# plai-group/latent-flexible-video-diffusion-modeling

Measured on AMD Instinct MI355X. Metric: denoising steps/sec on 20-frame 4x16x16 latents (sampling; training reported alongside), higher is better.
Workload: dtype f32

## Files before the change

### include/lfvdm_hip.h

```cpp
#ifndef LFVDM_HIP_H
#define LFVDM_HIP_H

#include <stdint.h>

#ifdef __cplusplus
extern "C" {
#endif

#define LFVDM_OK 0
#define LFVDM_E_SHAPE 1
#define LFVDM_E_LAUNCH 2
#define LFVDM_E_UNSUPPORTED 3

#define LFVDM_ACT_NONE 0
#define LFVDM_ACT_SILU 1

#define LFVDM_OUT_ROWS 0
#define LFVDM_OUT_NCHW 1

int lfvdm_abi_version(void);

typedef struct lfvdm_conv_args {
    const float* src0;
    const float* src1;
// ... 186 lines not shown
} lfvdm_rpe_job;

int lfvdm_rpe_nets(const lfvdm_rpe_job* jobs_dev, int njobs, int total_tiles, const int64_t* frame_indices_i64,
                   int B, int T, void* stream);
int lfvdm_rpe_nets_maxc(const lfvdm_rpe_job* jobs_dev, int njobs, int total_tiles, const int64_t* frame_indices_i64,
                        int B, int T, int max_channels, void* stream);

typedef struct lfvdm_rpe_bwd_job {
    const float* tproj;
    const float* Wd;
    const float* bd;
    const float* Wout_t;
    const float* dR;
    float* dtproj;
    float* dWd;
    float* dbd;
    int32_t C;
    int32_t tile0;
    int32_t tproj_ld;
    int32_t dtproj_ld;
} lfvdm_rpe_bwd_job;

int lfvdm_rpe_nets_bwd(const lfvdm_rpe_bwd_job* jobs_dev, int njobs, int total_tiles, const int64_t* frame_indices_i64,
                       int B, int T, void* stream);
int lfvdm_rpe_nets_bwd_det(const lfvdm_rpe_bwd_job* jobs_dev, int njobs, int total_tiles, const int64_t* frame_indices_i64,
                           int B, int T, float* det_ws, int64_t det_ws_floats, void* stream);

int lfvdm_rpe_front(const float* tproj, int tproj_ld, const float* feats, const float* Wd, const float* bd, float* act, int B,
                    int rows_per_b, int C, void* stream);
int lfvdm_rpe_front_bwd(const float* tproj, int tproj_ld, const float* feats, const float* Wd, const float* bd,
                        const float* d_act, float* dtproj, int dtproj_ld, float* dWd, float* dbd, int B, int rows_per_b,
                        int C, void* stream);

int lfvdm_attn_spatial(const float* qkv, float* o, float* attn_out, float* lse_out, int N, int P, int C, int heads,
                       void* stream);

int lfvdm_attn_spatial_fused_ok(int N, int P, int C, int heads);
int lfvdm_attn_spatial_fused(const float* xn, const float* Wqkv, const float* bqkv, float* o, int N, int P, int C, int heads,
                             void* stream);

int lfvdm_attn_spatial_bwd(const float* qkv, const float* o, const float* d_o, const float* lse, float* delta_ws,
                           float* dqkv, int N, int P, int C, int heads, void* stream);

int lfvdm_attn_temporal(const float* qkv, const float* Rq, const float* Rk, const float* Rv,
                        const float* mask , float* o, float* attn_out,
                        int B, int T, int P, int C, int heads, void* stream);
int lfvdm_attn_temporal_sel(const float* qkv, const float* Rq, const float* Rk, const float* Rv, const float* mask,
                            float* o, float* attn_out, int B, int T, int P, int C, int heads, const int64_t* rsel,
                            void* stream);
int lfvdm_attn_temporal_ring(const float* qkv, const float* Rq, const float* Rk, const float* Rv, const float* mask,
                             float* o, float* attn_out, int B, int T, int P, int C, int heads, const int64_t* rsel,
                             int ring, void* stream);

int lfvdm_attn_temporal_bwd(const float* qkv, const float* d_o, const float* Rq, const float* Rk, const float* Rv,
                            const float* mask, float* ws_p, float* ws_ds, float* dqkv, float* dRq, float* dRk,
                            float* dRv, int B, int T, int P, int C, int heads, void* stream);

int lfvdm_q_sample(const float* x0, const float* noise, const int64_t* t, const float* sqrt_acp,
                   const float* sqrt_1macp, float* out, int B, int inner, void* stream);
#define LFVDM_RULE_ANCESTRAL 0
#define LFVDM_RULE_DDIM 1
#define LFVDM_MEAN_EPS 0
#define LFVDM_MEAN_X0 1
int lfvdm_update_x0(const float* x, const float* model_out, const float* noise, const int64_t* t, const float* sqrt_recip_acp,
                    const float* sqrt_recipm1_acp, const float* c1, const float* c2, const float* sg, int rule, int mean_type,
                    int clip, float* sample, float* pred_xstart, float* mean_out, int B, int inner, void* stream);
int lfvdm_update_rng_x0(const float* x, const float* model_out, float* noise_out, const int64_t* t, const float* sqrt_recip_acp,
                        const float* sqrt_recipm1_acp, const float* c1, const float* c2, const float* sg, int rule,
                        int mean_type, int clip, float* sample, float* pred_xstart, float* mean_out, int B, int inner,
                        const int64_t* seed, void* stream);
int lfvdm_conv_out_psample_ok(int N, int H, int W, int C, int Cout);
int lfvdm_conv_out_update_x0(const float* act, const float* Wp, const float* bias, float* out, const float* x,
                             const float* noise_in, float* noise_out, const int64_t* t, const float* sqrt_recip_acp,
                             const float* sqrt_recipm1_acp, const float* c1, const float* c2, const float* sg, int rule,
                             int mean_type, int clip, float* sample, float* pred_xstart, float* mean_out, int B, int T, int H,
                             int W, int C, int Cout, const int64_t* seed, void* stream);
int lfvdm_update_ms_x0(const float* x, const float* model_out, const float* hist, const int64_t* t, const float* sqrt_recip_acp,
                       const float* sqrt_recipm1_acp, const float* k1, const float* k2, const float* k3, int mean_type, int clip,
                       float* sample, float* pred_xstart, int B, int inner, void* stream);
int lfvdm_conv_out_update_ms_x0(const float* act, const float* Wp, const float* bias, float* out, const float* x,
                                const float* hist, const int64_t* t, const float* sqrt_recip_acp, const float* sqrt_recipm1_acp,
                                const float* k1, const float* k2, const float* k3, int mean_type, int clip, float* sample,
                                float* pred_xstart, int B, int T, int H, int W, int C, int Cout, void* stream);
int lfvdm_known_blend(float* x, const float* known, const float* mask, const float* eps, float* noise_out, const int64_t* t,
                      const float* sqrt_acp_prev, const float* sqrt_1macp_prev, const int64_t* seed, int B, int T, int C,
                      int HW, void* stream);
int lfvdm_renoise(float* x, float* noise_out, const int64_t* t, const float* sqrt_1mbeta, const float* sqrt_beta,
                  const int64_t* seed, int B, int inner, void* stream);
int lfvdm_sampler_tick(int64_t* t, const float* model_timestep_table, float* model_t, int B, void* stream);
int lfvdm_sampler_tick_fetch(int64_t* t, const float* model_timestep_table, float* model_t, int B, const float* rows_all,
                             int rows_ld, float* rows, int row_floats, void* stream);
int lfvdm_masked_mse(const float* a, const float* b, const float* mask, float* out, int B, int T,
                     int frame_inner, void* stream);
int lfvdm_masked_mse_bwd(const float* target, const float* pred, const float* mask, const float* g, float* dpred, int B, int T,
                         int frame_inner, void* stream);

int lfvdm_train_loss(const float* target, const float* pred, const float* mask, const float* eval_mask, const int64_t* t,
                     const float* wtab, int n_t, float* mse, float* eval_mse, float* loss, int B, int T, int frame_inner,
                     void* stream);
int lfvdm_train_loss_bwd(const float* target, const float* pred, const float* mask, const int64_t* t, const float* wtab, int n_t,
                         const float* g, float* dpred, int B, int T, int frame_inner, void* stream);

int lfvdm_vb_terms(const float* x_start, const float* x_t, const float* model_out, const float* noise, const int64_t* t,
                   const float* sqrt_recip_acp, const float* sqrt_recipm1_acp, const float* c1, const float* c2,
                   const float* post_log_var, const float* model_log_var, const float* mask, int mean_type, int clip, float* vb,
                   float* xstart_mse, float* eps_mse, float* pred_xstart, int B, int T, int frame_inner, int out_ld,
                   int col_base, void* stream);
int lfvdm_vb_terms_bwd(const float* x_start, const float* x_t, const float* model_out, const int64_t* t,
                       const float* sqrt_recip_acp, const float* sqrt_recipm1_acp, const float* c1, const float* c2,
                       const float* model_log_var, const float* mask, const float* g, int mean_type, int clip, float* d_out,
                       int B, int T, int frame_inner, void* stream);

typedef struct lfvdm_adamw_args {
    float* p;
    const float* g;
    float* m;
    float* v;
    float* ema[4];
    float ema_rate[4];
    int32_t n_ema;
    int64_t n;
    float lr, beta1, beta2, eps, weight_decay;
    float bias_corr1, bias_corr2_sqrt;
    float grad_scale;
    float* grad_sqsum;
    const int32_t* skip_flag;
    const int32_t* skip_flag2;
} lfvdm_adamw_args;

int lfvdm_adamw_ema(const lfvdm_adamw_args* a, void* stream);

#define LFVDM_GRAD_NORM_MAX_PARTS 512
int lfvdm_grad_norm_nparts(int64_t n);
int lfvdm_grad_norm_partials(const float* g, int64_t n, float grad_scale, float* partials, int nparts, void* stream);
int lfvdm_grad_norm_finalize(const float* partials, int nparts, float max_norm, float* stat, void* stream);
int lfvdm_adamw_ema_clip(const lfvdm_adamw_args* a, const float* stat, void* stream);

int lfvdm_prepare_batch(const float* pool, const int32_t* table, float* batch, int64_t* frame_indices, float* obs_mask,
                        float* latent_mask, int B, int F, int Tp, int frame_elems, void* stream);

#define LFVDM_SLOT_PAD 0
#define LFVDM_SLOT_OBS 1
#define LFVDM_SLOT_LATENT 2
int lfvdm_search_assemble(const float* pool, const int32_t* table, const int32_t* role, float* x0, float* x_start,
                          float* obs_mask, float* latent_mask, float* mask, int64_t* frame_indices, int W, int K, int V, int Tv,
                          int frame_elems, void* stream);
int lfvdm_search_noise_qsample(const float* x_start, const int32_t* table, const int64_t* t_list, int32_t* ctl,
                               const int64_t* key, const float* sqrt_acp, const float* sqrt_1macp, float* noise, float* x_t,
                               int64_t* t_buf, int W, int K, int V, int frame_elems, void* stream);
int lfvdm_search_noise_fill(const int32_t* table, uint64_t seed, int step, int j, float* noise, int W, int K, int V,
                            int frame_elems, void* stream);
int lfvdm_search_scores(const float* terms, const int64_t* t_list, float* scores, int G, int V, int n_t, int ld, int col_base,
                        void* stream);

int lfvdm_compose_rows(const float* x, const float* x0, const float* obs, float* rows, int N, int Cx, int H, int W, int ld,
                       void* stream);

#define LFVDM_CHAIN_CONV 0
#define LFVDM_CHAIN_GN 1
#define LFVDM_CHAIN_LOCAL 2
#define LFVDM_CHAIN_MAX_DEPS 64
#define LFVDM_CHAIN_CTL_EPOCH 0
#define LFVDM_CHAIN_CTL_EXIT 32
#define LFVDM_CHAIN_CTL_ABORT 64
#define LFVDM_CHAIN_CTL_INTS 96

// ... 56 lines not shown
```

### latent-flexible-video-diffusion-modeling_amd/csrc/diffusion_ops.hip

```cpp
#include "common_hip.h"
#include "philox_normal.h"

namespace {

__global__ __launch_bounds__(256) void q_sample_kernel(const float* __restrict__ x0, const float* __restrict__ noise,
                                                       const int64_t* __restrict__ t, const float* __restrict__ sa,
                                                       const float* __restrict__ sb, float* __restrict__ out, int inner) {
    const int b = blockIdx.y;
    const float ca = sa[t[b]], cb = sb[t[b]];
    const size_t base = (size_t)b * inner;
    for (int i = (blockIdx.x * blockDim.x + threadIdx.x) * 4; i < inner; i += gridDim.x * blockDim.x * 4) {
        if (i + 3 < inner) {
            st4(out + base + i, ca * ld4(x0 + base + i) + cb * ld4(noise + base + i));
        } else {
            for (int j = i; j < inner; ++j) out[base + j] = ca * x0[base + j] + cb * noise[base + j];
        }
    }
}

enum { RULE_ANCESTRAL = 0, RULE_DDIM = 1, RULE_DDIM_DET = 2, RULE_DPMPP2M = 3 };
constexpr bool rule_draws(int rule) { return rule == RULE_ANCESTRAL || rule == RULE_DDIM; }

enum { MEAN_EPS = 0, MEAN_X0 = 1 };

template <int MEAN>
__device__ __forceinline__ float mean_x0hat(float r, float rm1, float xv, float out) {
    return MEAN == MEAN_X0 ? out : r * xv - rm1 * out;
}

template <int RULE>
__device__ __forceinline__ float rule_sigma(const float* __restrict__ t_logvar, int64_t tb) {
    if (RULE == RULE_ANCESTRAL) return tb != 0 ? expf(0.5f * t_logvar[tb]) : 0.f;
    if (RULE == RULE_DDIM) return tb != 0 ? t_logvar[tb] : 0.f;
    return 0.f;
}

struct StepCoef { float r, rm1, c1, c2, sigma; };

template <int RULE, int MEAN>
__device__ __forceinline__ StepCoef step_coef(int64_t tb, const float* t_recip, const float* t_recipm1, const float* t_c1,
                                              const float* t_c2, const float* t_logvar) {
    return {MEAN == MEAN_EPS ? t_recip[tb] : 0.f, MEAN == MEAN_EPS ? t_recipm1[tb] : 0.f, t_c1[tb], t_c2[tb],
            rule_sigma<RULE>(t_logvar, tb)};
}

template <int MEAN>
__device__ __forceinline__ float step_mean(const StepCoef& k, float xv, float out, int clip, float& p0) {
    p0 = mean_x0hat<MEAN>(k.r, k.rm1, xv, out);
    if (clip) p0 = fminf(fmaxf(p0, -1.f), 1.f);
    return k.c1 * p0 + k.c2 * xv;
}

template <int MEAN>
__device__ __forceinline__ float multistep_mean(const StepCoef& k, float k3, float xv, float out, int clip, const float* hist,
                                                size_t at, float& p0) {
    p0 = MEAN == MEAN_X0 ? out : __fmaf_rn(k.r, xv, -__fmul_rn(k.rm1, out));
    if (clip) p0 = fminf(fmaxf(p0, -1.f), 1.f);
    float mean = __fmaf_rn(k.c2, xv, __fmul_rn(k.c1, p0));
    if (k3 != 0.f) mean = __fmaf_rn(k3, __fsub_rn(p0, hist[at]), mean);
    return mean;
}

template <int RULE> struct PredOut { typedef float* __restrict__ ptr; };
template <> struct PredOut<RULE_DPMPP2M> { typedef float* ptr; };

template <int RULE, int MEAN>
__global__ __launch_bounds__(256) void p_sample_kernel(const float* x, const float* __restrict__ eps,
                                                       const float* __restrict__ noise, const int64_t* __restrict__ t,
                                                       const float* __restrict__ t_recip, const float* __restrict__ t_recipm1,
                                                       const float* __restrict__ t_c1, const float* __restrict__ t_c2,
                                                       const float* __restrict__ t_logvar, int clip,
                                                       float* sample, typename PredOut<RULE>::ptr pred,
                                                       float* __restrict__ mean_out, int inner, const float* hist,
                                                       const float* __restrict__ t_k3) {
    const int b = blockIdx.y;
    const int64_t tb = t[b];
    const StepCoef k = step_coef<RULE, MEAN>(tb, t_recip, t_recipm1, t_c1, t_c2, t_logvar);
    const float k3 = RULE == RULE_DPMPP2M ? t_k3[tb] : 0.f;
    const size_t base = (size_t)b * inner;
    for (int i = blockIdx.x * blockDim.x + threadIdx.x; i < inner; i += gridDim.x * blockDim.x) {
        float p0;
        const float mean = RULE == RULE_DPMPP2M ? multistep_mean<MEAN>(k, k3, x[base + i], eps[base + i], clip, hist, base + i, p0)
                                                : step_mean<MEAN>(k, x[base + i], eps[base + i], clip, p0);
        float sv = mean;
        if (rule_draws(RULE) && tb != 0) sv += k.sigma * noise[base + i];
        sample[base + i] = sv;
        if (pred) pred[base + i] = p0;
        if (mean_out) mean_out[base + i] = mean;
    }
}

template <int RULE, int MEAN>
__global__ __launch_bounds__(256) void p_sample_rng_kernel(const float* x, const float* __restrict__ eps,
                                                           float* __restrict__ noise_out, const int64_t* __restrict__ t,
                                                           const float* __restrict__ t_recip, const float* __restrict__ t_recipm1,
                                                           const float* __restrict__ t_c1, const float* __restrict__ t_c2,
                                                           const float* __restrict__ t_logvar, int clip, float* sample,
                                                           float* __restrict__ pred, float* __restrict__ mean_out, int inner,
                                                           const int64_t* __restrict__ seed) {
    const int b = blockIdx.y;
    const int64_t tb = t[b];
    const StepCoef k = step_coef<RULE, MEAN>(tb, t_recip, t_recipm1, t_c1, t_c2, t_logvar);
    const unsigned long long key = RULE != RULE_DDIM_DET ? (unsigned long long)seed[0] : 0ull;
    const unsigned k0 = (unsigned)key, k1 = (unsigned)(key >> 32);
    const size_t base = (size_t)b * inner;
    const int nq = (inner + 3) >> 2;
    for (int qd = blockIdx.x * blockDim.x + threadIdx.x; qd < nq; qd += gridDim.x * blockDim.x) {
        f32x4 z = (f32x4){0.f, 0.f, 0.f, 0.f};
        if (RULE != RULE_DDIM_DET) z = normal4((unsigned)qd, (unsigned)b, (unsigned)tb, k0, k1);
#pragma unroll
        for (int e = 0; e < 4; ++e) {
            const int i = 4 * qd + e;
            if (i < inner) {
                float p0;
                const float mean = step_mean<MEAN>(k, x[base + i], eps[base + i], clip, p0);
                sample[base + i] = RULE != RULE_DDIM_DET ? mean + k.sigma * z[e] : mean;
                if (RULE != RULE_DDIM_DET && noise_out) noise_out[base + i] = z[e];
                if (pred) pred[base + i] = p0;
                if (mean_out) mean_out[base + i] = mean;
            }
        }
    }
}

struct HeadUpdate {
    const float *act, *Wp, *bias, *x, *noise_in;
    float *eps_out, *noise_out, *sample, *pred, *mean_out;
    const int64_t *t, *seed;
    const float *t_recip, *t_recipm1, *t_c1, *t_c2, *t_logvar;
    int N, T, H, W, C, clip;
    const float *hist, *t_k3;
};

template <int CO, int CPL, int RULE, int MEAN>
__global__ __launch_bounds__(256) void conv_out_psample_kernel(const HeadUpdate p) {
    extern __shared__ __attribute__((aligned(16))) float wl[];
    const int tid = threadIdx.x;
    const int C = p.C;
    {
        constexpr int NW4 = CO * 9 * 16 * CPL, NIT = (NW4 + 255) / 256;
        f32x4 wv[NIT];
#pragma unroll
        for (int u = 0; u < NIT; ++u) {
            const int i = tid + 256 * u;
            wv[u] = i < NW4 ? ld4(p.Wp + 4 * (size_t)i) : (f32x4){0.f, 0.f, 0.f, 0.f};
        }
#pragma unroll
        for (int u = 0; u < NIT; ++u) {
            const int i = tid + 256 * u;
            if (i < NW4) st4(wl + 4 * i, wv[u]);
        }
    }
    __syncthreads();
    const int lane = tid & 63, wave = tid >> 6;
    const int WQ = p.W >> 2;
    const long quad = (long)blockIdx.x * 4 + wave;
    if (quad >= (long)p.N * p.H * WQ) return;
    const int n = (int)(quad / (p.H * WQ));
    const int rem = (int)(quad - (long)n * p.H * WQ);
    const int y = rem / WQ, xq = rem - y * WQ;
    const int j = lane >> 4, cl = lane & 15;
    const int x = 4 * xq + j;
    float acc[CO];
#pragma unroll
    for (int co = 0; co < CO; ++co) acc[co] = 0.f;
#pragma unroll
    for (int tap = 0; tap < 9; ++tap) {
        const int iy = y + tap / 3 - 1, ix = x + tap % 3 - 1;
        const bool inb = iy >= 0 && iy < p.H && ix >= 0 && ix < p.W;
        const float* a = p.act + ((size_t)(n * p.H + (inb ? iy : y)) * p.W + (inb ? ix : x)) * C;
#pragma unroll
        for (int u = 0; u < CPL; ++u) {
            const int c = (cl + 16 * u) * 4;
            f32x4 a4 = ld4(a + c);
            if (!inb) a4 = (f32x4){0.f, 0.f, 0.f, 0.f};
#pragma unroll
            for (int co = 0; co < CO; ++co) {
                const f32x4 w4 = ld4(wl + (co * 9 + tap) * C + c);
                acc[co] += (a4.x * w4.x + a4.y * w4.y) + (a4.z * w4.z + a4.w * w4.w);
            }
        }
    }
#pragma unroll
    for (int co = 0; co < CO; ++co)
#pragma unroll
        for (int o = 1; o < 16; o <<= 1) acc[co] += __shfl_xor(acc[co], o, 64);
    if (cl >= CO) return;
    float e = acc[0];
#pragma unroll
    for (int co = 1; co < CO; ++co) e = cl == co ? acc[co] : e;
    const int co = cl;
    e += p.bias[co];
    const int b = n / p.T, tt = n - b * p.T;
    const int inner = p.T * CO * p.H * p.W;
    const int i = ((tt * CO + co) * p.H + y) * p.W + x;
    const size_t at = (size_t)b * inner + i;
    const int64_t tb = p.t[b];
    const StepCoef k = step_coef<RULE, MEAN>(tb, p.t_recip, p.t_recipm1, p.t_c1, p.t_c2, p.t_logvar);
    float z = 0.f;
    if (!rule_draws(RULE)) {
    } else if (p.noise_in) {
        z = p.noise_in[at];
    } else {
        const unsigned long long key = (unsigned long long)p.seed[0];
        const f32x4 z4 = normal4((unsigned)(i >> 2), (unsigned)b, (unsigned)tb, (unsigned)key, (unsigned)(key >> 32));
        z = j == 0 ? z4.x : j == 1 ? z4.y : j == 2 ? z4.z : z4.w;
    }
    float p0;
    const float mean = RULE == RULE_DPMPP2M ? multistep_mean<MEAN>(k, p.t_k3[tb], p.x[at], e, p.clip, p.hist, at, p0)
                                            : step_mean<MEAN>(k, p.x[at], e, p.clip, p0);
    p.sample[at] = rule_draws(RULE) ? mean + k.sigma * z : mean;
    if (p.eps_out) p.eps_out[at] = e;
    if (rule_draws(RULE) && p.noise_out) p.noise_out[at] = z;
    if (p.pred) p.pred[at] = p0;
    if (p.mean_out) p.mean_out[at] = mean;
}

__global__ __launch_bounds__(1024) void masked_mse_kernel(const float* __restrict__ a, const float* __restrict__ bb,
                                                          const float* __restrict__ mask, float* __restrict__ out, int T,
                                                          int frame_inner) {
    const int b = blockIdx.x;
    const size_t base = (size_t)b * T * frame_inner;
    float acc = 0.f;
    if ((frame_inner & 3) == 0) {
        const int q = frame_inner >> 2, total = T * q;
        for (int e = threadIdx.x; e < total; e += 1024) {
            const int t = e / q;
            const float mk = mask ? mask[b * T + t] : 1.f;
            const f32x4 d = ld4(a + base + (size_t)e * 4) - ld4(bb + base + (size_t)e * 4);
            acc += ((d.x * d.x + d.y * d.y) + (d.z * d.z + d.w * d.w)) * mk;
        }
    } else {
        for (int t = 0; t < T; ++t) {
            const float mk = mask ? mask[b * T + t] : 1.f;
            for (int i = threadIdx.x; i < frame_inner; i += 1024) {
                const float d = a[base + (size_t)t * frame_inner + i] - bb[base + (size_t)t * frame_inner + i];
                acc += d * d * mk;
            }
        }
    }
    __shared__ float red[16];
    acc = wave_sum(acc);
    if ((threadIdx.x & 63) == 0) red[threadIdx.x >> 6] = acc;
    __syncthreads();
    if (threadIdx.x == 0) {
        float t = 0.f;
        for (int w = 0; w < 16; ++w) t += red[w];
        out[b] = t / (float)((size_t)T * frame_inner);
    }
}

__global__ __launch_bounds__(256) void masked_mse_bwd_kernel(const float* __restrict__ target, const float* __restrict__ pred,
                                                             const float* __restrict__ mask, const float* __restrict__ g,
                                                             float* __restrict__ dpred, int T, int frame_inner) {
    const int b = blockIdx.y;
    const size_t base = (size_t)b * T * frame_inner;
    const float sc = -2.0f * g[b] / (float)((size_t)T * frame_inner);
    const long total = (long)T * frame_inner;
    for (long i = (long)blockIdx.x * 256 + threadIdx.x; i < total; i += (long)gridDim.x * 256) {
        const float mk = mask ? mask[b * T + (int)(i / frame_inner)] : 1.f;
        dpred[base + i] = (target[base + i] - pred[base + i]) * (sc * mk);
    }
}

}

extern "C" int lfvdm_masked_mse_bwd(const float* target, const float* pred, const float* mask, const float* g, float* dpred,
                                    int B, int T, int frame_inner, void* stream) {
    if (B <= 0 || T <= 0 || frame_inner <= 0 || !target || !pred || !g || !dpred) return LFVDM_E_SHAPE;
    long gx = ((long)T * frame_inner + 255) / 256;
    if (gx > 1024) gx = 1024;
    hipLaunchKernelGGL(masked_mse_bwd_kernel, dim3((unsigned)gx, B), dim3(256), 0, (hipStream_t)stream, target, pred, mask, g, dpred,
                       T, frame_inner);
    LFVDM_CHECK_LAUNCH();
    return LFVDM_OK;
}

extern "C" int lfvdm_q_sample(const float* x0, const float* noise, const int64_t* t, const float* sqrt_acp,
                              const float* sqrt_1macp, float* out, int B, int inner, void* stream) {
    if (B <= 0 || inner <= 0) return LFVDM_E_SHAPE;
    int gx = (inner / 4 + 255) / 256;
    if (gx > 1024) gx = 1024;
    if (gx < 1) gx = 1;
    hipLaunchKernelGGL(q_sample_kernel, dim3(gx, B), dim3(256), 0, (hipStream_t)stream, x0, noise, t, sqrt_acp, sqrt_1macp, out, inner);
    LFVDM_CHECK_LAUNCH();
    return LFVDM_OK;
}

namespace {
__global__ void sampler_tick_kernel(int64_t* __restrict__ t, const float* __restrict__ table, float* __restrict__ model_t, int B) {
    const int b = blockIdx.x * blockDim.x + threadIdx.x;
    if (b >= B) return;
    int64_t v = t[b] - 1;
    v = v < 0 ? 0 : v;
    t[b] = v;
    model_t[b] = table[v];
}

// ... 124 lines not shown
                               const float* sqrt_recip_acp, const float* sqrt_recipm1_acp, const float* c1, const float* c2,
                               const float* sg, int rule, int mean_type, int clip, float* sample, float* pred_xstart,
                               float* mean_out, int B, int inner, void* stream) {
    const int R = update_cell(rule, mean_type, x, model_out, t, sqrt_recip_acp, sqrt_recipm1_acp, c1, c2, sg, sample, B, inner,
                              noise != nullptr);
    if (R < 0) return LFVDM_E_SHAPE;
    return on_grid(R, mean_type, [&](auto r, auto m) {
        return launch_update<decltype(r)::value, decltype(m)::value>(
            x, model_out, decltype(r)::value == RULE_DDIM_DET ? nullptr : noise, t, sqrt_recip_acp, sqrt_recipm1_acp, c1, c2, sg,
            clip, sample, pred_xstart, mean_out, B, inner, stream);
    });
}

extern "C" int lfvdm_update_rng_x0(const float* x, const float* model_out, float* noise_out, const int64_t* t,
                                   const float* sqrt_recip_acp, const float* sqrt_recipm1_acp, const float* c1, const float* c2,
                                   const float* sg, int rule, int mean_type, int clip, float* sample, float* pred_xstart,
                                   float* mean_out, int B, int inner, const int64_t* seed, void* stream) {
    const int R = update_cell(rule, mean_type, x, model_out, t, sqrt_recip_acp, sqrt_recipm1_acp, c1, c2, sg, sample, B, inner,
                              seed != nullptr);
    if (R < 0) return LFVDM_E_SHAPE;
    return on_grid(R, mean_type, [&](auto r, auto m) {
        constexpr bool det = decltype(r)::value == RULE_DDIM_DET;
        return launch_update_rng<decltype(r)::value, decltype(m)::value>(
            x, model_out, det ? nullptr : noise_out, t, sqrt_recip_acp, sqrt_recipm1_acp, c1, c2, sg, clip, sample, pred_xstart,
            mean_out, B, inner, det ? nullptr : seed, stream);
    });
}

extern "C" int lfvdm_conv_out_update_x0(const float* act, const float* Wp, const float* bias, float* out, const float* x,
                                        const float* noise_in, float* noise_out, const int64_t* t, const float* sqrt_recip_acp,
                                        const float* sqrt_recipm1_acp, const float* c1, const float* c2, const float* sg,
                                        int rule, int mean_type, int clip, float* sample, float* pred_xstart, float* mean_out,
                                        int B, int T, int H, int W, int C, int Cout, const int64_t* seed, void* stream) {
    const int R = update_cell(rule, mean_type, x, act, t, sqrt_recip_acp, sqrt_recipm1_acp, c1, c2, sg, sample, B, T,
                              noise_in || seed);
    if (R < 0 || !Wp || !bias) return LFVDM_E_SHAPE;
    const bool det = R == RULE_DDIM_DET;
    const HeadUpdate p = {act, Wp, bias, x, det ? nullptr : noise_in, out, det ? nullptr : noise_out, sample, pred_xstart, mean_out,
                          t, det ? nullptr : seed, sqrt_recip_acp, sqrt_recipm1_acp, c1, c2, sg, B * T, T, H, W, C, clip,
                          nullptr, nullptr};
    return on_grid(R, mean_type, [&](auto r, auto m) { return launch_head<decltype(r)::value, decltype(m)::value>(p, Cout, stream); });
}

namespace {
bool multistep_ok(int mean_type, const float* x, const float* model_out, const int64_t* t, const float* recip,
                  const float* recipm1, const float* k1, const float* k2, const float* k3, const float* sample, int B, int inner) {
    if (!mean_ok(mean_type, recip, recipm1)) return false;
    return B > 0 && inner > 0 && x && model_out && t && k1 && k2 && k3 && sample;
}
template <class F>
int on_multistep(bool have_hist, int mean_type, F f) {
    const bool x0 = mean_type == LFVDM_MEAN_X0;
    if (have_hist) return x0 ? f(Const<RULE_DPMPP2M>(), Const<MEAN_X0>()) : f(Const<RULE_DPMPP2M>(), Const<MEAN_EPS>());
    return x0 ? f(Const<RULE_DDIM_DET>(), Const<MEAN_X0>()) : f(Const<RULE_DDIM_DET>(), Const<MEAN_EPS>());
}
}

extern "C" int lfvdm_update_ms_x0(const float* x, const float* model_out, const float* hist, const int64_t* t,
                                  const float* sqrt_recip_acp, const float* sqrt_recipm1_acp, const float* k1, const float* k2,
                                  const float* k3, int mean_type, int clip, float* sample, float* pred_xstart, int B, int inner,
                                  void* stream) {
    if (!multistep_ok(mean_type, x, model_out, t, sqrt_recip_acp, sqrt_recipm1_acp, k1, k2, k3, sample, B, inner))
        return LFVDM_E_SHAPE;
    return on_multistep(hist != nullptr, mean_type, [&](auto r, auto m) {
        return launch_update<decltype(r)::value, decltype(m)::value>(x, model_out, nullptr, t, sqrt_recip_acp, sqrt_recipm1_acp, k1,
                                                                     k2, nullptr, clip, sample, pred_xstart, nullptr, B, inner,
                                                                     stream, hist, k3);
    });
}

extern "C" int lfvdm_conv_out_update_ms_x0(const float* act, const float* Wp, const float* bias, float* out, const float* x,
                                           const float* hist, const int64_t* t, const float* sqrt_recip_acp,
                                           const float* sqrt_recipm1_acp, const float* k1, const float* k2, const float* k3,
                                           int mean_type, int clip, float* sample, float* pred_xstart, int B, int T, int H, int W,
                                           int C, int Cout, void* stream) {
    if (!multistep_ok(mean_type, x, act, t, sqrt_recip_acp, sqrt_recipm1_acp, k1, k2, k3, sample, B, T) || !Wp || !bias)
        return LFVDM_E_SHAPE;
    const HeadUpdate p = {act, Wp, bias, x, nullptr, out, nullptr, sample, pred_xstart, nullptr, t, nullptr, sqrt_recip_acp,
                          sqrt_recipm1_acp, k1, k2, nullptr, B * T, T, H, W, C, clip, hist, k3};
    return on_multistep(hist != nullptr, mean_type,
                        [&](auto r, auto m) { return launch_head<decltype(r)::value, decltype(m)::value>(p, Cout, stream); });
}

extern "C" int lfvdm_masked_mse(const float* a, const float* b, const float* mask, float* out, int B, int T,
                                int frame_inner, void* stream) {
    if (B <= 0 || T <= 0 || frame_inner <= 0) return LFVDM_E_SHAPE;
    hipLaunchKernelGGL(masked_mse_kernel, dim3(B), dim3(1024), 0, (hipStream_t)stream, a, b, mask, out, T, frame_inner);
    LFVDM_CHECK_LAUNCH();
    return LFVDM_OK;
}
```

### latent-flexible-video-diffusion-modeling_amd/csrc/norm_embed.hip

```cpp
#include "common_hip.h"
#include "gn_wave_body.h"

namespace {

constexpr int GN_GPW = 8;
constexpr int GN_THREADS = 256;
constexpr int GN_MAXCW = 256;


template <int KEEP>
__global__ __launch_bounds__(GN_THREADS) void gn_coef_kernel(
    const float* __restrict__ s0, const float* __restrict__ s1, int C0, int C1, int P,
    const float* __restrict__ gamma, const float* __restrict__ beta, const float* __restrict__ film, int film_div,
    int film_ld, float eps, float* __restrict__ coefA, float* __restrict__ coefB, float* __restrict__ stats,
    float* __restrict__ act_out, int act_mode) {
    const int C = C0 + C1;
    const int cg = C / 32;
    const float rcg = __builtin_amdgcn_rcpf((float)cg);
    const int CW = GN_GPW * cg;
    const int Q = CW / 4;
    const int n = blockIdx.x;
    const int cbase = blockIdx.y * CW;
    const int PL = GN_THREADS / Q;
    const int tid = threadIdx.x;
    const bool active = tid < PL * Q;
    const int q = active ? tid % Q : 0;
    const int pl = active ? tid / Q : 0;
    const int c = cbase + q * 4;

    __shared__ float part[GN_THREADS * 4];
    __shared__ float chs[GN_MAXCW];
    __shared__ float gmean[GN_GPW], grstd[GN_GPW];
    __shared__ __attribute__((aligned(16))) float shA[GN_MAXCW], shB[GN_MAXCW];

    const size_t pos0 = (size_t)n * P;
    const bool pow2q = (Q & (Q - 1)) == 0 && Q <= 64;
    const bool cached = P <= KEEP * PL;
    f32x4 keep[KEEP];
    for (int pass = 0; pass < 2; ++pass) {
        f32x4 s = {0.f, 0.f, 0.f, 0.f};
        if (active) {
            f32x4 mu = {0.f, 0.f, 0.f, 0.f};
            if (pass) {
                mu.x = gmean[fdiv_small(q * 4 + 0, cg, rcg)]; mu.y = gmean[fdiv_small(q * 4 + 1, cg, rcg)];
                mu.z = gmean[fdiv_small(q * 4 + 2, cg, rcg)]; mu.w = gmean[fdiv_small(q * 4 + 3, cg, rcg)];
            }
            if (cached) {
#pragma unroll
                for (int i = 0; i < KEEP; ++i) {
                    const int p = pl + i * PL;
                    if (pass == 0) {
                        keep[i] = (p < P) ? ld_cat(s0, s1, C0, C1, pos0 + p, c) : (f32x4){0.f, 0.f, 0.f, 0.f};
                        s += keep[i];
                    } else if (p < P) {
                        const f32x4 v = keep[i] - mu;
                        s += v * v;
                    }
                }
            } else {
                for (int p = pl; p < P; p += PL) {
                    f32x4 v = ld_cat(s0, s1, C0, C1, pos0 + p, c);
                    if (pass) { v = v - mu; s += v * v; } else { s += v; }
                }
            }
            if (pow2q) {
                for (int off = Q; off < 64; off <<= 1) {
                    s.x += __shfl_xor(s.x, off, 64); s.y += __shfl_xor(s.y, off, 64);
                    s.z += __shfl_xor(s.z, off, 64); s.w += __shfl_xor(s.w, off, 64);
                }
                if ((tid & 63) < Q) st4(part + ((tid >> 6) * Q + q) * 4, s);
            } else {
                st4(part + (pl * Q + q) * 4, s);
            }
        }
        __syncthreads();
        const int rows = pow2q ? GN_THREADS / 64 : PL;
        for (int cc = tid; cc < CW; cc += GN_THREADS) {
            float t = 0.f;
            for (int i = 0; i < rows; ++i) t += part[i * CW + cc];
            chs[cc] = t;
        }
        __syncthreads();
        if (tid < GN_GPW) {
            float t = 0.f;
            for (int i = 0; i < cg; ++i) t += chs[tid * cg + i];
            const float inv = 1.0f / (float)(cg * P);
            if (pass == 0) gmean[tid] = t * inv;
            else grstd[tid] = 1.0f / sqrtf(t * inv + eps);
        }
        __syncthreads();
    }
    if (stats && tid < GN_GPW) {
        stats[((size_t)n * 32 + blockIdx.y * GN_GPW + tid) * 2 + 0] = gmean[tid];
        stats[((size_t)n * 32 + blockIdx.y * GN_GPW + tid) * 2 + 1] = grstd[tid];
    }
    for (int cc = tid; cc < CW; cc += GN_THREADS) {
        const int ch = cbase + cc;
        const int g = fdiv_small(cc, cg, rcg);
        float A = grstd[g] * gamma[ch];
        float B = beta[ch] - gmean[g] * A;
        if (film) {
            const float* f = film + (size_t)(n / film_div) * film_ld;
            const float sc = 1.0f + f[ch];
            A *= sc;
            B = B * sc + f[C + ch];
        }
        if (coefA) {
            coefA[(size_t)n * C + ch] = A;
            coefB[(size_t)n * C + ch] = B;
        }
        shA[cc] = A;
        shB[cc] = B;
    }
    if (act_out == nullptr) return;
    __syncthreads();
    if (active) {
        const f32x4 a4 = ld4(shA + q * 4), b4 = ld4(shB + q * 4);
        if (cached) {
#pragma unroll
            for (int i = 0; i < KEEP; ++i) {
                const int p = pl + i * PL;
                if (p < P) {
                    f32x4 v = keep[i] * a4 + b4;
                    if (act_mode == LFVDM_ACT_SILU) { v.x = silu_f(v.x); v.y = silu_f(v.y); v.z = silu_f(v.z); v.w = silu_f(v.w); }
                    st4(act_out + (pos0 + p) * C + c, v);
                }
            }
        } else {
            for (int p = pl; p < P; p += PL) {
                f32x4 v = ld_cat(s0, s1, C0, C1, pos0 + p, c) * a4 + b4;
                if (act_mode == LFVDM_ACT_SILU) { v.x = silu_f(v.x); v.y = silu_f(v.y); v.z = silu_f(v.z); v.w = silu_f(v.w); }
                st4(act_out + (pos0 + p) * C + c, v);
            }
        }
    }
}

template <int CG>
__global__ __launch_bounds__(64) void gn_wave_kernel(
    const float* __restrict__ s0, const float* __restrict__ s1, int C0, int C1, int P,
    const float* __restrict__ gamma, const float* __restrict__ beta, const float* __restrict__ film, int film_div,
    int film_ld, float eps, float* __restrict__ coefA, float* __restrict__ coefB, float* __restrict__ stats,
    float* __restrict__ act_out, int act_mode, int ldo) {
    gn_wave_body<CG, false>(blockIdx.x, blockIdx.y, threadIdx.x, s0, s1, C0, C1, P, gamma, beta, film, film_div, film_ld, eps, coefA,
                            coefB, stats, act_out, act_mode, ldo);
}

template <int CG>
__global__ __launch_bounds__(256) void gn_wave4_kernel(
    const float* __restrict__ s0, const float* __restrict__ s1, int C0, int C1, int P,
    const float* __restrict__ gamma, const float* __restrict__ beta, const float* __restrict__ film, int film_div,
    int film_ld, float eps, float* __restrict__ coefA, float* __restrict__ coefB, float* __restrict__ stats,
    float* __restrict__ act_out, int act_mode, int ldo) {
    gn_wave_body<CG, false, 4>(blockIdx.x, blockIdx.y, threadIdx.x & 63, s0, s1, C0, C1, P, gamma, beta, film, film_div, film_ld, eps,
                               coefA, coefB, stats, act_out, act_mode, ldo, __builtin_amdgcn_readfirstlane(threadIdx.x >> 6));
}

inline bool gn_wave_launch(const float* src0, const float* src1, int C0, int C1, int N, int P, const float* gamma,
                           const float* beta, const float* film, int film_div, int film_ld, float eps, float* coefA,
                           float* coefB, float* stats, float* out, int act, hipStream_t s) {
    static const bool off = getenv("LFVDM_GN_NO_WAVE") != nullptr;
    const int C = C0 + C1, cg = C / 32;
    if (off || P > 256 || C0 % 16 || (cg != 2 && cg != 4 && cg != 8 && cg != 16) || N > 65535) return false;
    const dim3 grid(N, C / 16);
    static const int minp4 = getenv("LFVDM_GN_WAVE4_MINP") ? atoi(getenv("LFVDM_GN_WAVE4_MINP")) : 128;
    if (minp4 > 0 && P >= minp4 && P % 64 == 0) {
#define LFVDM_GNW4(G)                                                                                                   \
    hipLaunchKernelGGL(gn_wave4_kernel<G>, grid, dim3(256), 0, s, src0, src1, C0, C1, P, gamma, beta, film, film_div, film_ld, \
                       eps, coefA, coefB, stats, out, act, 0)
        if (cg == 2) LFVDM_GNW4(2);
        else if (cg == 4) LFVDM_GNW4(4);
        else if (cg == 8) LFVDM_GNW4(8);
        else LFVDM_GNW4(16);
#undef LFVDM_GNW4
        return true;
    }
#define LFVDM_GNW(G)                                                                                                   \
    hipLaunchKernelGGL(gn_wave_kernel<G>, grid, dim3(64), 0, s, src0, src1, C0, C1, P, gamma, beta, film, film_div, film_ld, \
                       eps, coefA, coefB, stats, out, act, 0)
    if (cg == 2) LFVDM_GNW(2);
    else if (cg == 4) LFVDM_GNW(4);
    else if (cg == 8) LFVDM_GNW(8);
    else LFVDM_GNW(16);
#undef LFVDM_GNW
    return true;
}

constexpr int GN_KEEP = 8;

struct GnChunkGeom { int C0, C1, P, S, PL; };

__device__ __forceinline__ void gn_chunk_load(const float* s0, const float* s1, const GnChunkGeom& g, size_t pos0, int p_first,
                                              int pl, int c, f32x4 (&keep)[GN_KEEP]) {
#pragma unroll
    for (int i = 0; i < GN_KEEP; ++i) {
        const int p = p_first + pl + i * g.PL;
        keep[i] = ld_cat(s0, s1, g.C0, g.C1, pos0 + min(p, g.P - 1), c);
    }
}

__global__ __launch_bounds__(GN_THREADS) void gn_chunk_stats_kernel(const float* __restrict__ s0, const float* __restrict__ s1,
                                                                    GnChunkGeom g, float* __restrict__ part_out) {
    const int C = g.C0 + g.C1, cg = C / 32, CW = GN_GPW * cg, Q = CW / 4, PL = g.PL;
    const float rcg = __builtin_amdgcn_rcpf((float)cg);
    const int sidx = blockIdx.x, n = blockIdx.z, cbase = blockIdx.y * CW;
    const int tid = threadIdx.x;
    const bool active = tid < PL * Q;
    const int q = active ? tid % Q : 0, pl = active ? tid / Q : 0;
    const int c = cbase + q * 4;
    const int p_first = sidx * (GN_KEEP * PL);
    const int npos = min(GN_KEEP * PL, g.P - p_first);
    __shared__ float part[GN_THREADS * 4];
    __shared__ float chs[GN_MAXCW];
    __shared__ float gmean[GN_GPW];
    f32x4 keep[GN_KEEP];
    gn_chunk_load(s0, s1, g, (size_t)n * g.P, p_first, pl, c, keep);
    for (int pass = 0; pass < 2; ++pass) {
        f32x4 s = {0.f, 0.f, 0.f, 0.f};
        if (active) {
            f32x4 mu = {0.f, 0.f, 0.f, 0.f};
            if (pass) {
                mu.x = gmean[fdiv_small(q * 4 + 0, cg, rcg)]; mu.y = gmean[fdiv_small(q * 4 + 1, cg, rcg)];
                mu.z = gmean[fdiv_small(q * 4 + 2, cg, rcg)]; mu.w = gmean[fdiv_small(q * 4 + 3, cg, rcg)];
            }
#pragma unroll
            for (int i = 0; i < GN_KEEP; ++i) {
                if (pl + i * PL < npos) {
                    if (pass == 0) { s += keep[i]; } else { const f32x4 v = keep[i] - mu; s += v * v; }
                }
            }
            st4(part + (pl * Q + q) * 4, s);
        }
        __syncthreads();
        for (int cc = tid; cc < CW; cc += GN_THREADS) {
            float t = 0.f;
            for (int i = 0; i < PL; ++i) t += part[i * CW + cc];
            chs[cc] = t;
        }
        __syncthreads();
        if (tid < GN_GPW) {
            float t = 0.f;
            for (int i = 0; i < cg; ++i) t += chs[tid * cg + i];
            float* o = part_out + (((size_t)n * 32 + blockIdx.y * GN_GPW + tid) * g.S + sidx) * 2;
            if (pass == 0) { gmean[tid] = t / (float)(cg * npos); o[0] = gmean[tid]; }
            else o[1] = t;
        }
        __syncthreads();
    }
}
// ... 147 lines not shown
        const f32x4 ga = ld4(gamma + q * 4), be = ld4(beta + q * 4);
        f32x4 o;
        o.x = (v.x - gstat[fdiv_small(q * 4 + 0, cg, rcg)]) * gstat[32 + fdiv_small(q * 4 + 0, cg, rcg)] * ga.x + be.x;
        o.y = (v.y - gstat[fdiv_small(q * 4 + 1, cg, rcg)]) * gstat[32 + fdiv_small(q * 4 + 1, cg, rcg)] * ga.y + be.y;
        o.z = (v.z - gstat[fdiv_small(q * 4 + 2, cg, rcg)]) * gstat[32 + fdiv_small(q * 4 + 2, cg, rcg)] * ga.z + be.z;
        o.w = (v.w - gstat[fdiv_small(q * 4 + 3, cg, rcg)]) * gstat[32 + fdiv_small(q * 4 + 3, cg, rcg)] * ga.w + be.w;
        st4(y + base + t * tstride + q * 4, o);
    }
}

template <int TIT>
__global__ __launch_bounds__(256) void gn_temporal_reg_kernel(const float* __restrict__ x, const float* __restrict__ gamma,
                                                              const float* __restrict__ beta, float eps,
                                                              float* __restrict__ y, int B, int T, int P, int C) {
    __shared__ float chs_all[4][256];
    __shared__ float gstat_all[4][64];
    const int lane = threadIdx.x & 63;
    const int wave = threadIdx.x >> 6;
    const long sample = (long)blockIdx.x * 4 + wave;
    if (sample >= (long)B * P) return;
    float* chs = chs_all[wave];
    float* gstat = gstat_all[wave];
    const int b = (int)(sample / P), p = (int)(sample % P);
    const int cg = C / 32;
    const float rcg = __builtin_amdgcn_rcpf((float)cg);
    const int Q = C / 4;
    const size_t base = ((size_t)b * T * P + p) * C;
    const size_t tstride = (size_t)P * C;
    const int TL = 64 / Q;
    const int q = lane % Q, tl = lane / Q;
    f32x4 keep[TIT];
#pragma unroll
    for (int i = 0; i < TIT; ++i) {
        const int t = tl + i * TL;
        keep[i] = t < T ? ld4(x + base + t * tstride + q * 4) : (f32x4){0.f, 0.f, 0.f, 0.f};
    }
    f32x4 mu = {0.f, 0.f, 0.f, 0.f}, rs = {0.f, 0.f, 0.f, 0.f};
#pragma unroll
    for (int pass = 0; pass < 2; ++pass) {
        f32x4 s = {0.f, 0.f, 0.f, 0.f};
#pragma unroll
        for (int i = 0; i < TIT; ++i) {
            if (tl + i * TL < T) {
                if (pass) { const f32x4 v = keep[i] - mu; s += v * v; } else { s += keep[i]; }
            }
        }
        for (int o = Q; o < 64; o <<= 1) {
            s.x += __shfl_xor(s.x, o, 64); s.y += __shfl_xor(s.y, o, 64);
            s.z += __shfl_xor(s.z, o, 64); s.w += __shfl_xor(s.w, o, 64);
        }
        if (tl == 0) st4(chs + q * 4, s);
        wave_lds_fence();
        if (lane < 32) {
            float t = 0.f;
            for (int i = 0; i < cg; ++i) t += chs[lane * cg + i];
            const float inv = 1.0f / (float)(cg * T);
            if (pass == 0) gstat[lane] = t * inv;
            else gstat[32 + lane] = 1.0f / sqrtf(t * inv + eps);
        }
        wave_lds_fence();
        if (pass == 0) {
            mu.x = gstat[fdiv_small(q * 4 + 0, cg, rcg)]; mu.y = gstat[fdiv_small(q * 4 + 1, cg, rcg)];
            mu.z = gstat[fdiv_small(q * 4 + 2, cg, rcg)]; mu.w = gstat[fdiv_small(q * 4 + 3, cg, rcg)];
        } else {
            rs.x = gstat[32 + fdiv_small(q * 4 + 0, cg, rcg)]; rs.y = gstat[32 + fdiv_small(q * 4 + 1, cg, rcg)];
            rs.z = gstat[32 + fdiv_small(q * 4 + 2, cg, rcg)]; rs.w = gstat[32 + fdiv_small(q * 4 + 3, cg, rcg)];
        }
    }
    const f32x4 ga = ld4(gamma + q * 4), be = ld4(beta + q * 4);
#pragma unroll
    for (int i = 0; i < TIT; ++i) {
        const int t = tl + i * TL;
        if (t < T) {
            f32x4 o;
            o.x = (keep[i].x - mu.x) * rs.x * ga.x + be.x;
            o.y = (keep[i].y - mu.y) * rs.y * ga.y + be.y;
            o.z = (keep[i].z - mu.z) * rs.z * ga.z + be.z;
            o.w = (keep[i].w - mu.w) * rs.w * ga.w + be.w;
            st4(y + base + t * tstride + q * 4, o);
        }
    }
}

struct ConvInTick {
    int64_t* t;
    const float* table;
    float* model_t;
    const float* rows_all;
    float* rows;
    int B, rows_ld, row_floats;
};

__device__ __forceinline__ void conv_in_clock(const ConvInTick& tk, int64_t* tnew) {
    if ((int)threadIdx.x < tk.B) {
        int64_t v = tk.t[threadIdx.x] - 1;
        v = v < 0 ? 0 : v;
        tk.t[threadIdx.x] = v;
        tnew[threadIdx.x] = v;
    }
    __syncthreads();
    if ((int)threadIdx.x < tk.B) tk.model_t[threadIdx.x] = tk.table[tnew[threadIdx.x]];
    const int q4 = tk.row_floats >> 2;
    for (int b = 0; b < tk.B; ++b) {
        const float* src = tk.rows_all + ((size_t)tnew[b] * tk.B + b) * tk.rows_ld;
        float* dst = tk.rows + (size_t)b * tk.rows_ld;
        for (int i0 = threadIdx.x; i0 < q4; i0 += 256 * 8) {
            f32x4 v[8];
#pragma unroll
            for (int u = 0; u < 8; ++u) {
                const int i = i0 + 256 * u;
                v[u] = i < q4 ? ld4(src + 4 * i) : (f32x4){0.f, 0.f, 0.f, 0.f};
            }
#pragma unroll
            for (int u = 0; u < 8; ++u) {
                const int i = i0 + 256 * u;
                if (i < q4) st4(dst + 4 * i, v[u]);
            }
        }
    }
}

template <int QW, int CIT>
__global__ __launch_bounds__(256) void conv_in_kernel(const float* __restrict__ x, const float* __restrict__ x0,
                                                      const float* __restrict__ obs, const float* __restrict__ w,
                                                      const float* __restrict__ bias, float* __restrict__ out, int N,
                                                      int C, int H, int W, ConvInTick tk) {
    constexpr int Cout = 16 * QW;
    extern __shared__ __attribute__((aligned(16))) float wl[];
    if (tk.t != nullptr && blockIdx.x == gridDim.x - 1) {
        conv_in_clock(tk, reinterpret_cast<int64_t*>(wl));
        return;
    }
    const int Ci = CIT ? CIT : C + 1;
    const int K = Ci * 9;
    constexpr int CP = Cout + 4;
    {
        const float rK = __builtin_amdgcn_rcpf((float)K);
        const int total4 = (K * Cout) >> 2;
        for (int i0 = threadIdx.x; i0 < total4; i0 += 256 * 4) {
            f32x4 v[4];
#pragma unroll
            for (int u = 0; u < 4; ++u) {
                const int i4 = i0 + 256 * u;
                v[u] = i4 < total4 ? ld4(w + 4 * (size_t)i4) : (f32x4){0.f, 0.f, 0.f, 0.f};
            }
#pragma unroll
            for (int u = 0; u < 4; ++u) {
                const int i4 = i0 + 256 * u;
                if (i4 < total4) {
#pragma unroll
                    for (int e = 0; e < 4; ++e) {
                        const int i = 4 * i4 + e;
                        int co = (int)((float)i * rK);
                        int k = i - co * K;
                        if (k < 0) { k += K; co -= 1; }
                        if (k >= K) { k -= K; co += 1; }
                        wl[k * CP + co] = v[u][e];
                    }
                }
            }
        }
    }
    __syncthreads();
    const int lane = threadIdx.x & 63;
    const int grp = __builtin_amdgcn_readfirstlane(threadIdx.x >> 6);
    const int HW = H * W;
    const long total = (long)N * HW;
    const long pix = (long)blockIdx.x * 64 + lane;
    const bool live = pix < total;
    const long pp = live ? pix : total - 1;
    const int n = (int)(pp / HW);
    const int p = (int)(pp - (long)n * HW);
    const int oy = p / W, ox = p - oy * W;
    const float ob = obs[n];
    f32x4 acc[QW];
#pragma unroll
    for (int q = 0; q < QW; ++q) acc[q] = ld4(bias + (grp * QW + q) * 4);
    const float* xn = x + (size_t)n * C * HW;
    const float* x0n = x0 + (size_t)n * C * HW;
    const float* wg = wl + grp * QW * 4;
    if constexpr (CIT > 0) {
        float v[9][CIT];
#pragma unroll
        for (int tap = 0; tap < 9; ++tap) {
            const int iy = oy + tap / 3 - 1, ix = ox + tap % 3 - 1;
            const bool inb = iy >= 0 && iy < H && ix >= 0 && ix < W;
            const int ip = inb ? iy * W + ix : p;
#pragma unroll
            for (int ci = 0; ci < CIT; ++ci) {
                float t = ob;
                if (ci < CIT - 1) t = xn[ci * HW + ip] * (1.0f - ob) + x0n[ci * HW + ip] * ob;
                v[tap][ci] = inb ? t : 0.f;
            }
        }
#pragma unroll
        for (int tap = 0; tap < 9; ++tap)
#pragma unroll
            for (int ci = 0; ci < CIT; ++ci) {
                const float* wk = wg + (ci * 9 + tap) * CP;
#pragma unroll
                for (int q = 0; q < QW; ++q) acc[q] += v[tap][ci] * ld4(wk + q * 4);
            }
    } else {
#pragma unroll
        for (int tap = 0; tap < 9; ++tap) {
            const int iy = oy + tap / 3 - 1, ix = ox + tap % 3 - 1;
            const bool inb = iy >= 0 && iy < H && ix >= 0 && ix < W;
            const int ip = inb ? iy * W + ix : p;
            for (int ci = 0; ci < Ci; ++ci) {
                float v = ob;
                if (ci < C) v = xn[ci * HW + ip] * (1.0f - ob) + x0n[ci * HW + ip] * ob;
                v = inb ? v : 0.f;
                const float* wk = wg + (ci * 9 + tap) * CP;
#pragma unroll
                for (int q = 0; q < QW; ++q) acc[q] += v * ld4(wk + q * 4);
            }
        }
    }
    if (live) {
        float* o = out + (size_t)pix * Cout + grp * QW * 4;
#pragma unroll
        for (int q = 0; q < QW; ++q) st4(o + q * 4, acc[q]);
    }
}

template <int NCT, int CI>
__global__ __launch_bounds__(256) void conv_in_mfma_kernel(const float* __restrict__ x, const float* __restrict__ x0,
                                                           const float* __restrict__ obs, const float* __restrict__ w,
                                                           const float* __restrict__ bias, float* __restrict__ out, int N,
                                                           int H, int W, ConvInTick tk) {
    constexpr int Cout = 16 * NCT, C = CI - 1, K = 9 * CI, KP = (K + 3) & ~3, KS = KP + 1;
    constexpr int NKI = KP / 4;
    extern __shared__ __attribute__((aligned(16))) float wl[];
    if (tk.t != nullptr && blockIdx.x == gridDim.x - 1) {
        conv_in_clock(tk, reinterpret_cast<int64_t*>(wl));
        return;
    }
    float* As = wl;
    float* Ws = wl + 64 * KS;
    const int tid = threadIdx.x, lane = tid & 63, wave = __builtin_amdgcn_readfirstlane(tid >> 6);
    float wv[Cout / 4];
#pragma unroll
    for (int i = 0; i < Cout / 4; ++i) wv[i] = lane < K ? w[(size_t)(wave + 4 * i) * K + lane] : 0.f;
    const int HW = H * W;
    const long total = (long)N * HW;
    const long pix = (long)blockIdx.x * 64 + lane;
    const bool live = pix < total;
    const long pp = live ? pix : total - 1;
    const int n = (int)(pp / HW);
    const int pq = (int)(pp - (long)n * HW);
    const int oy = pq / W, ox = pq - oy * W;
    const float ob = obs[n];
    const float* xn = x + (size_t)n * C * HW;
    const float* x0n = x0 + (size_t)n * C * HW;
    float xa[NKI], xb[NKI];
    bool inb[NKI];
#pragma unroll
    for (int i = 0; i < NKI; ++i) {
        const int k = wave + 4 * i;
        const int ci = k / 9, tap = k - ci * 9;
        const int iy = oy + tap / 3 - 1, ix = ox + tap % 3 - 1;
        inb[i] = live && k < K && iy >= 0 && iy < H && ix >= 0 && ix < W;
        const int ip = inb[i] ? iy * W + ix : pq;
        const int cc = ci < C ? ci : 0;
        xa[i] = xn[cc * HW + ip];
        xb[i] = x0n[cc * HW + ip];
    }
#pragma unroll
    for (int i = 0; i < Cout / 4; ++i)
        if (lane < KP) Ws[(wave + 4 * i) * KS + lane] = wv[i];
#pragma unroll
    for (int i = 0; i < NKI; ++i) {
        const int k = wave + 4 * i;
        const int ci = k / 9;
        float v = ci < C ? xa[i] * (1.0f - ob) + xb[i] * ob : ob;
        As[lane * KS + k] = inb[i] ? v : 0.f;
    }
    __syncthreads();
    const int r16 = lane & 15, kq = lane >> 4;
    f32x4 acc[NCT];
#pragma unroll
    for (int c = 0; c < NCT; ++c) {
        const float b = bias[16 * c + r16];
        acc[c] = (f32x4){b, b, b, b};
    }
    const float* ar = As + (16 * wave + r16) * KS + kq;
    const float* wr = Ws + r16 * KS + kq;
#pragma unroll
    for (int s4 = 0; s4 < KP; s4 += 4) {
        const float a = ar[s4];
#pragma unroll
        for (int c = 0; c < NCT; ++c) acc[c] = __builtin_amdgcn_mfma_f32_16x16x4f32(a, wr[16 * c * KS + s4], acc[c], 0, 0, 0);
    }
    const long p0 = (long)blockIdx.x * 64 + 16 * wave + 4 * kq;
#pragma unroll
    for (int r = 0; r < 4; ++r) {
        if (p0 + r < total) {
            float* o = out + (size_t)(p0 + r) * Cout + r16;
#pragma unroll
            for (int c = 0; c < NCT; ++c) o[16 * c] = acc[c][r];
        }
    }
}

__global__ __launch_bounds__(256) void rowdot_kernel(const lfvdm_rowdot_job* __restrict__ jobs, int njobs, int total_rows) {
    const int lane = threadIdx.x & 63;
    const int row = blockIdx.x * 4 + (threadIdx.x >> 6);
    if (row >= total_rows) return;
    int j = 0;
    while (j + 1 < njobs && jobs[j + 1].row0 <= row) ++j;
    const lfvdm_rowdot_job J = jobs[j];
    const int o = row - J.row0;
    const float* wrow = J.W + (size_t)o * J.K;
    const float bo = J.b ? J.b[o] : 0.f;
    for (int m0 = 0; m0 < J.M; m0 += 8) {
        float acc[8];
#pragma unroll
        for (int i = 0; i < 8; ++i) acc[i] = 0.f;
        for (int k = lane * 4; k < J.K; k += 256) {
            const f32x4 wv = ld4(wrow + k);
#pragma unroll
            for (int i = 0; i < 8; ++i) {
                if (m0 + i >= J.M) break;
                f32x4 v;
                if (J.in_mode == 2) {
                    const float t = J.in[m0 + i];
                    const float* fr = J.in + J.ldin;
                    const int half = J.K >> 1;
                    float e[4];
#pragma unroll
                    for (int u = 0; u < 4; ++u) {
                        const int kk = k + u;
                        e[u] = kk < half ? cosf(t * fr[kk]) : sinf(t * fr[kk - half]);
                    }
                    v.x = e[0]; v.y = e[1]; v.z = e[2]; v.w = e[3];
                } else {
                    v = ld4(J.in + (size_t)(m0 + i) * J.ldin + k);
                    if (J.in_mode == 1) { v.x = silu_f(v.x); v.y = silu_f(v.y); v.z = silu_f(v.z); v.w = silu_f(v.w); }
                }
                acc[i] += v.x * wv.x + v.y * wv.y + v.z * wv.z + v.w * wv.w;
            }
        }
#pragma unroll
        for (int i = 0; i < 8; ++i) {
            if (m0 + i >= J.M) break;
            const float s = wave_sum(acc[i]);
            if (lane == 0) J.out[(size_t)(m0 + i) * J.ldout + o] = s + bo;
        }
    }
}

constexpr int RDB_ROWS = 8;
constexpr int RDB_TPW = 4;
constexpr int RDB_KIT = 4;
__global__ __launch_bounds__(256) void rowdot_bwd_kernel(const lfvdm_rowdot_bwd_job* __restrict__ jobs, int njobs, int total_tasks,
                                                         int tpw, const DetSlab ds) {
    __shared__ f32x4 red[3][4][RDB_KIT][64];
    const int lane = threadIdx.x & 63;
    const int wave = threadIdx.x >> 6;
    const int first = blockIdx.x * (4 * tpw);
    const int last = min(first + 4 * tpw, total_tasks) - 1;
    int jf = 0, jl = 0;
    while (jf + 1 < njobs && jobs[jf + 1].task0 <= first) ++jf;
    while (jl + 1 < njobs && jobs[jl + 1].task0 <= last) ++jl;
    const lfvdm_rowdot_bwd_job J0 = jobs[jf];
    const bool grouped = jf == jl && J0.din != nullptr && J0.M <= 4 && J0.K <= 256 * RDB_KIT && !ds.slab;
    f32x4 accG[4][RDB_KIT];
#pragma unroll
    for (int i = 0; i < 4; ++i)
#pragma unroll
        for (int it = 0; it < RDB_KIT; ++it) accG[i][it] = (f32x4){0.f, 0.f, 0.f, 0.f};
    for (int r = 0; r < tpw; ++r) {
        const int task = first + wave + 4 * r;
        if (task >= total_tasks) break;
        int j = jf;
        while (j + 1 < njobs && jobs[j + 1].task0 <= task) ++j;
        const lfvdm_rowdot_bwd_job J = jobs[j];
        const int o0 = (task - J.task0) * RDB_ROWS;
        const int o1 = min(o0 + RDB_ROWS, J.O);
        for (int m0 = 0; m0 < J.M; m0 += 4) {
            const int mc = min(4, J.M - m0);
            int it = 0;
            for (int k = lane * 4; k < J.K; k += 256, ++it) {
                f32x4 inv[4], accD[4];
#pragma unroll
// ... 176 lines not shown
    else LFVDM_GNP(16);
#undef LFVDM_GNP
    LFVDM_CHECK_LAUNCH();
    return LFVDM_OK;
}

extern "C" long lfvdm_gn_apply_ws_floats(int C, int N, int P) {
    if (C <= 0 || C % 32 || C > 1024 || N <= 0 || P <= 0) return 0;
    const int S = gn_chunks(C, P, nullptr);
    return (long)N * 32 * S * 2;
}

extern "C" int lfvdm_gn_apply_ws(const float* src0, const float* src1, int C0, int C1, int N, int P, const float* gamma,
                                 const float* beta, const float* film, int film_div, int film_ld, float eps, int act,
                                 float* out, float* coefA, float* coefB, float* stats, float* ws, long ws_floats,
                                 void* stream) {
    const int C = C0 + C1;
    if (N <= 0 || P <= 0 || C <= 0 || C % 32 || C0 % 4 || C > 1024 || !out) return LFVDM_E_SHAPE;
    if (C1 > 0 && !src1) return LFVDM_E_SHAPE;
    if (film && film_div <= 0) return LFVDM_E_SHAPE;
    if ((coefA == nullptr) != (coefB == nullptr)) return LFVDM_E_SHAPE;
    int PL = 0;
    const int S = gn_chunks(C, P, &PL);
    if (S == 0)
        return lfvdm_gn_apply(src0, src1, C0, C1, N, P, gamma, beta, film, film_div, film_ld, eps, act, out, coefA, coefB, stats,
                              stream);
    if (!ws || ws_floats < (long)N * 32 * S * 2 || N > 65535) return LFVDM_E_SHAPE;
    const GnChunkGeom g = {C0, C1, P, S, PL};
    const dim3 grid(S, 32 / GN_GPW, N);
    hipLaunchKernelGGL(gn_chunk_stats_kernel, grid, dim3(GN_THREADS), 0, (hipStream_t)stream, src0, src1, g, ws);
    LFVDM_CHECK_LAUNCH();
    hipLaunchKernelGGL(gn_chunk_apply_kernel, grid, dim3(GN_THREADS), 0, (hipStream_t)stream, src0, src1, g, (const float*)ws,
                       gamma, beta, film, film_div, film_ld, eps, coefA, coefB, stats, out, act);
    LFVDM_CHECK_LAUNCH();
    return LFVDM_OK;
}

extern "C" int lfvdm_gn_coef(const float* src0, const float* src1, int C0, int C1, int N, int P, const float* gamma,
                             const float* beta, const float* film, int film_div, int film_ld, float eps, float* coefA,
                             float* coefB, void* stream) {
    return lfvdm_gn_coef_stats(src0, src1, C0, C1, N, P, gamma, beta, film, film_div, film_ld, eps, coefA, coefB, nullptr,
                               stream);
}

extern "C" int lfvdm_gn_temporal(const float* x, const float* gamma, const float* beta, float eps, float* y, int B, int T,
                                 int P, int C, void* stream) {
    if (B <= 0 || T <= 0 || P <= 0 || C <= 0 || C % 32 || C > GT_MAXC) return LFVDM_E_SHAPE;
    const long samples = (long)B * P;
    const dim3 grid((unsigned)((samples + 3) / 4));
    const int Q = C / 4;
    if (Q <= 64 && 64 % Q == 0) {
        const int per_lane = (T + 64 / Q - 1) / (64 / Q);
        hipStream_t s = (hipStream_t)stream;
        if (per_lane <= 8) {
            hipLaunchKernelGGL(gn_temporal_reg_kernel<8>, grid, dim3(256), 0, s, x, gamma, beta, eps, y, B, T, P, C);
            LFVDM_CHECK_LAUNCH();
            return LFVDM_OK;
        }
        if (per_lane <= 16) {
            hipLaunchKernelGGL(gn_temporal_reg_kernel<16>, grid, dim3(256), 0, s, x, gamma, beta, eps, y, B, T, P, C);
            LFVDM_CHECK_LAUNCH();
            return LFVDM_OK;
        }
        if (per_lane <= 32) {
            hipLaunchKernelGGL(gn_temporal_reg_kernel<32>, grid, dim3(256), 0, s, x, gamma, beta, eps, y, B, T, P, C);
            LFVDM_CHECK_LAUNCH();
            return LFVDM_OK;
        }
    }
    hipLaunchKernelGGL(gn_temporal_kernel, grid, dim3(256), 0, (hipStream_t)stream, x, gamma, beta, eps, y, B, T, P, C);
    LFVDM_CHECK_LAUNCH();
    return LFVDM_OK;
}

static int conv_in_launch(const float* x, const float* x0, const float* obs, const float* w, const float* bias, float* out,
                          int N, int C, int H, int W, int Cout, const ConvInTick& tk, hipStream_t s) {
    if (N <= 0 || C <= 0 || Cout % 16 || Cout > 256 || H <= 0 || W <= 0) return LFVDM_E_SHAPE;
    size_t lds = (size_t)(C + 1) * 9 * (Cout + 4) * sizeof(float);
    if (lds > 64 * 1024) return LFVDM_E_UNSUPPORTED;
    if (lds < 64 * sizeof(int64_t)) lds = 64 * sizeof(int64_t);
    const long total = (long)N * H * W;
    const dim3 grid((unsigned)((total + 63) / 64) + (tk.t ? 1u : 0u));
    {
        static const bool off = getenv("LFVDM_CONV_IN_SCALAR") != nullptr;
        if (!off && (C == 4 || C == 3) && (Cout == 64 || Cout == 128)) {
            const int KP = (9 * (C + 1) + 3) & ~3;
            size_t l2 = (size_t)(64 + Cout) * (KP + 1) * sizeof(float);
            if (l2 < 64 * sizeof(int64_t)) l2 = 64 * sizeof(int64_t);
#define LFVDM_CIM(NCT, CI) hipLaunchKernelGGL((conv_in_mfma_kernel<NCT, CI>), grid, dim3(256), l2, s, x, x0, obs, w, bias, out, N, H, W, tk)
            if (C == 4) { if (Cout == 64) LFVDM_CIM(4, 5); else LFVDM_CIM(8, 5); }
            else { if (Cout == 64) LFVDM_CIM(4, 4); else LFVDM_CIM(8, 4); }
#undef LFVDM_CIM
            LFVDM_CHECK_LAUNCH();
            return LFVDM_OK;
        }
    }
#define LFVDM_CONV_IN(Q)                                                                                              \
    case Q:                                                                                                           \
        if (C == 4) hipLaunchKernelGGL((conv_in_kernel<Q, 5>), grid, dim3(256), lds, s, x, x0, obs, w, bias, out, N, C, H, W, tk);      \
        else if (C == 3) hipLaunchKernelGGL((conv_in_kernel<Q, 4>), grid, dim3(256), lds, s, x, x0, obs, w, bias, out, N, C, H, W, tk); \
        else hipLaunchKernelGGL((conv_in_kernel<Q, 0>), grid, dim3(256), lds, s, x, x0, obs, w, bias, out, N, C, H, W, tk);             \
        break;
    switch (Cout / 16) {
        LFVDM_CONV_IN(1) LFVDM_CONV_IN(2) LFVDM_CONV_IN(3) LFVDM_CONV_IN(4) LFVDM_CONV_IN(5) LFVDM_CONV_IN(6) LFVDM_CONV_IN(7)
        LFVDM_CONV_IN(8) LFVDM_CONV_IN(9) LFVDM_CONV_IN(10) LFVDM_CONV_IN(11) LFVDM_CONV_IN(12) LFVDM_CONV_IN(13)
        LFVDM_CONV_IN(14) LFVDM_CONV_IN(15) LFVDM_CONV_IN(16)
        default: return LFVDM_E_SHAPE;
    }
#undef LFVDM_CONV_IN
    LFVDM_CHECK_LAUNCH();
    return LFVDM_OK;
}

extern "C" int lfvdm_conv_in(const float* x, const float* x0, const float* obs, const float* w, const float* bias,
                             float* out, int N, int C, int H, int W, int Cout, void* stream) {
    const ConvInTick none = {nullptr, nullptr, nullptr, nullptr, nullptr, 0, 0, 0};
    return conv_in_launch(x, x0, obs, w, bias, out, N, C, H, W, Cout, none, (hipStream_t)stream);
}

extern "C" int lfvdm_conv_in_tick(const float* x, const float* x0, const float* obs, const float* w, const float* bias,
                                  float* out, int N, int C, int H, int W, int Cout, int64_t* t,
                                  const float* model_timestep_table, float* model_t, int B, const float* rows_all, int rows_ld,
                                  float* rows, int row_floats, void* stream) {
    if (B <= 0 || B > 64 || !t || !model_timestep_table || !model_t || !rows_all || !rows) return LFVDM_E_SHAPE;
    if (row_floats <= 0 || (row_floats & 3) || (rows_ld & 3) || rows_ld < row_floats) return LFVDM_E_SHAPE;
    const ConvInTick tk = {t, model_timestep_table, model_t, rows_all, rows, B, rows_ld, row_floats};
    return conv_in_launch(x, x0, obs, w, bias, out, N, C, H, W, Cout, tk, (hipStream_t)stream);
}

namespace {
__global__ __launch_bounds__(256) void silu_kernel(const float* __restrict__ in, float* __restrict__ out, long n4) {
    for (long i = (long)blockIdx.x * 256 + threadIdx.x; i < n4; i += (long)gridDim.x * 256) {
        f32x4 v = ld4(in + 4 * i);
        v.x = silu_f(v.x); v.y = silu_f(v.y); v.z = silu_f(v.z); v.w = silu_f(v.w);
        st4(out + 4 * i, v);
    }
}
}

extern "C" int lfvdm_silu(const float* in, float* out, int64_t n, void* stream) {
    if (!in || !out || n <= 0 || (n & 3)) return LFVDM_E_SHAPE;
    long blocks = (n / 4 + 255) / 256;
    if (blocks > 4096) blocks = 4096;
    hipLaunchKernelGGL(silu_kernel, dim3((unsigned)blocks), dim3(256), 0, (hipStream_t)stream, in, out, (long)(n / 4));
    LFVDM_CHECK_LAUNCH();
    return LFVDM_OK;
}

extern "C" int lfvdm_rowdot(const lfvdm_rowdot_job* jobs_dev, int njobs, int total_rows, void* stream) {
    if (njobs <= 0 || total_rows <= 0) return LFVDM_E_SHAPE;
    hipLaunchKernelGGL(rowdot_kernel, dim3((total_rows + 3) / 4), dim3(256), 0, (hipStream_t)stream, jobs_dev, njobs,
                       total_rows);
    LFVDM_CHECK_LAUNCH();
    return LFVDM_OK;
}
```

### latent-flexible-video-diffusion-modeling_amd/improved_diffusion/_engine.py

```python
import ctypes as C
import json
import os
import sys
import weakref

import torch as th
import torch.nn as nn

from . import _native as nat
from .nn import timestep_freqs


def _p(t):
    return t.data_ptr()


def update_args(tables, ddim=None, predict_xstart=False):
    if ddim is not None and "k3" in ddim:
        c1, c2, sg, rule = ddim["k1"], ddim["k2"], ddim["k3"], nat.RULE_DPMPP2M
    elif ddim is not None:
        c1, c2, sg, rule = ddim["k1"], ddim["k2"], ddim["sigma"], nat.RULE_DDIM
    else:
        c1, c2, sg = tables["posterior_mean_coef1"], tables["posterior_mean_coef2"], tables["model_log_variance"]
        rule = nat.RULE_ANCESTRAL
    if predict_xstart:
        return None, None, c1, c2, sg, rule, nat.MEAN_X0
    return tables["sqrt_recip_alphas_cumprod"], tables["sqrt_recipm1_alphas_cumprod"], c1, c2, sg, rule, nat.MEAN_EPS


SPATIAL_FUSED = os.environ.get("LFVDM_SPATIAL_FUSED", "1") != "0"
PROJ_GN = os.environ.get("LFVDM_PROJ_GN", "1") != "0"
TEMPORAL_QKV = os.environ.get("LFVDM_TEMPORAL_QKV", "1") != "0"
GN_EPILOGUE = os.environ.get("LFVDM_GN_EPILOGUE", "1") != "0"
NEXT_GN_EPILOGUE = os.environ.get("LFVDM_NEXT_GN_EPILOGUE", "1") != "0"
def level_chain_enabled():
    return os.environ.get("LFVDM_LEVEL_CHAIN", "1") != "0"


def chain_local_enabled():
    return os.environ.get("LFVDM_CHAIN_LOCAL", "1") != "0"


CHAIN_MAX_M = int(os.environ.get("LFVDM_CHAIN_MAX_M", "640"))
MAX_FRAMES = 64
CHAIN_TIMEOUT_S = float(os.environ.get("LFVDM_CHAIN_TIMEOUT_S", "2.0"))


class _TableBudget:

    def __init__(self):
        self._held = {}
        self._logged = set()

    def limit(self):
        return float(os.environ.get("LFVDM_TIME_TABLE_GB", "12")) * 2 ** 30

    def used(self):
        return sum(self._held.values())

    def remaining(self):
        return max(0.0, self.limit() - self.used())

    def reserve(self, plan, nbytes):
        if nbytes > self.remaining():
            import gc
            gc.collect()
        if nbytes > self.remaining():
            return False
        key = id(plan)
        self._held[key] = nbytes
        weakref.finalize(plan, self._held.pop, key, None)
        return True

    def log(self, msg):
        if os.environ.get("LFVDM_QUIET", "0") != "1" and msg not in self._logged:
            self._logged.add(msg)
            print("[lfvdm] " + msg, file=sys.stderr, flush=True)


_table_budget = _TableBudget()


class Plan:

    def __init__(self, engine, B, T, H, W, want_attn, time_steps=None):
        self.time_steps = int(time_steps) if time_steps else 0
        self.engine = engine
        self.model = engine.model
        self.B, self.T, self.H, self.W = B, T, H, W
        self.want_attn = want_attn
        self.dev = next(self.model.parameters()).device
        self.keep = []
        self.steps = []
        self.packs = []
        self.attn_t, self.attn_s = [], []
        self.chains = []
        self._build()

    def buf(self, *shape, dtype=th.float32):
        t = th.empty(*shape, device=self.dev, dtype=dtype)
        self.keep.append(t)
        return t

    def scratch(self, key, rows, cols):
        if level_chain_enabled() and rows <= CHAIN_MAX_M:
            return self.buf(rows * cols).view(rows, cols)
        pool = self.__dict__.setdefault("_scratch", {})
        t = pool.get(key)
        if t is None or t.numel() < rows * cols:
            t = pool[key] = self.buf(rows * cols)
        return t[:rows * cols].view(rows, cols)

    def gn_apply(self, a, b, C0, C1, N, P, gn, film, act, key):
        out = self.scratch(key, N * P, C0 + C1)
        L = nat.lib()
        args = (_p(a), _p(b) if b is not None else None, C0, C1, N, P, _p(gn.weight), _p(gn.bias),
                _p(film) if film is not None else None, self.T if film is not None else 1,
                self.rows_ld if film is not None else 0, gn.eps, act, _p(out), None, None, None)
        need = int(L.lfvdm_gn_apply_ws_floats(C0 + C1, N, P))
        if need:
            ws = self.scratch("gn_ws", 1, need)
            self.add(L.lfvdm_gn_apply_ws, *args, _p(ws), need)
        else:
# ... 481 lines not shown
        if nact is not None:
            res["act1"] = nact
        if getattr(self, "_cat_done", None) is not None:
            res["act1cat"], self._cat_done = self._cat_done, None
        return res

    def build_time_tables(self, ts_table):
        L, m = nat.lib(), self.model
        n_t, B = self.time_steps, self.B
        assert ts_table.numel() == n_t
        Bv, ch = n_t * B, m.model_channels
        ted, half = 4 * ch, ch // 2
        Bvp = (Bv + 3) // 4 * 4
        tin = th.zeros(Bvp + half, device=self.dev, dtype=th.float32)
        tin[:Bv] = ts_table.to(self.dev, th.float32).repeat_interleave(B)
        tin[Bvp:] = timestep_freqs(ch).to(self.dev)
        e0, emb = th.empty(Bv, ted, device=self.dev), th.empty(Bv, ted, device=self.dev)
        se0, semb = th.empty_like(e0), th.empty_like(emb)
        (j0, j1, jg), n_g, rows_g = self._emb_jobs(Bv, tin, Bvp, e0, emb, self.rows_all, se0, semb)
        s = nat.stream()
        nat.check(L.lfvdm_rowdot(_p(j0), 1, ted, s), "lfvdm_rowdot")
        nat.check(L.lfvdm_silu(_p(e0), _p(se0), e0.numel(), s), "lfvdm_silu")
        nat.check(L.lfvdm_rowdot(_p(j1), 1, ted, s), "lfvdm_rowdot")
        nat.check(L.lfvdm_silu(_p(emb), _p(semb), emb.numel(), s), "lfvdm_silu")
        nat.check(L.lfvdm_rowdot(_p(jg), n_g, rows_g, s), "lfvdm_rowdot")
        th.cuda.current_stream().synchronize()
        self.tables_sig = (self.time_signature(), tuple(ts_table.tolist()))

    def build_R_tables(self, frame_indices):
        if not self.R:
            return
        n_t, B, T = self.time_steps, self.B, self.T
        steps = (self.time_ring // 2) if self.time_ring else n_t
        self._fi_rep = frame_indices.to(self.dev, th.int64).reshape(B, T).repeat(steps, 1).contiguous()
        self._loaded = {}
        if not self.time_ring:
            self._fill_R(0, n_t, 0)

    def _fill_R(self, t0, t1, slot0):
        B, T = self.B, self.T
        key = (t0, t1, slot0)
        ent = self._fill_jobs.get(key)
        if ent is None:
            views = {r: buf[slot0 * B:] for r, buf in self.R.items()}
            ent = self._rpe_jobs((t1 - t0) * B, self.rows_all[t0 * B:], views)
            self._fill_jobs[key] = ent
        jr, n_r, tiles_r = ent
        nat.check(nat.lib().lfvdm_rpe_nets_maxc(_p(jr), n_r, tiles_r, _p(self._fi_rep), (t1 - t0) * B, T,
                                                max(r.rpe_net.channels for r in self.R), nat.stream()), "lfvdm_rpe_nets")

    def ensure_R(self, t_hi, t_lo=None):
        if not self.time_ring or not self.R:
            return
        H = self.time_ring // 2
        t_hi = min(max(int(t_hi), 0), self.time_steps - 1)
        t_lo = t_hi if t_lo is None else min(max(int(t_lo), 0), t_hi)
        assert t_hi - t_lo < H, "a graph launch walks less than half a ring of timesteps"
        for blk in {t_hi // H, t_lo // H}:
            if self._loaded.get(blk % 2) != blk:
                self._fill_R(blk * H, min((blk + 1) * H, self.time_steps), (blk % 2) * H)
                self._loaded[blk % 2] = blk

    def fill_whole_chain(self):
        if not self.R:
            return
        if not self.time_ring:
            self._fill_R(0, self.time_steps, 0)
            return
        H = self.time_ring // 2
        for blk in range((self.time_steps + H - 1) // H):
            self._fill_R(blk * H, min((blk + 1) * H, self.time_steps), (blk % 2) * H)
        self._loaded = {}

    def fuse_head_update(self, t_buf, tables, clip, seed, noise, pred, inject_noise, ddim=None, predict_xstart=False):
        L = nat.lib()
        h = self.head
        if self.head_fused:
            return True
        if h["step"] != len(self.steps) - 1 or L.lfvdm_conv_out_psample_ok(self.B * self.T, self.H, self.W, h["C"], h["Cout"]) != 0:
            return False
        self.keep.append((t_buf, tables, seed, noise, pred, ddim))
        recip, recipm1, c1, c2, sg, rule, mean_type = update_args(tables, ddim, predict_xstart)
        det, x0 = sg is None, recip is None
        if rule == nat.RULE_DPMPP2M:
            args = (_p(h["act"]), _p(h["Wp"]), _p(h["bias"]), _p(self.out), _p(self.x_in), _p(pred), _p(t_buf),
                    None if x0 else _p(recip), None if x0 else _p(recipm1), _p(c1), _p(c2), _p(sg), mean_type, int(bool(clip)),
                    _p(self.x_in), _p(pred), self.B, self.T, self.H, self.W, h["C"], h["Cout"])
            self.steps[h["step"]] = (L.lfvdm_conv_out_update_ms_x0, args)
            self.head_fused = True
            return True
        args = (_p(h["act"]), _p(h["Wp"]), _p(h["bias"]), _p(self.out), _p(self.x_in),
                _p(noise) if inject_noise and not det else None, None if inject_noise or det else _p(noise), _p(t_buf),
                None if x0 else _p(recip), None if x0 else _p(recipm1), _p(c1), _p(c2), None if det else _p(sg), rule, mean_type,
                int(bool(clip)), _p(self.x_in), _p(pred), None, self.B, self.T, self.H, self.W, h["C"], h["Cout"],
                None if det else _p(seed))
        self.steps[h["step"]] = (L.lfvdm_conv_out_update_x0, args)
        self.head_fused = True
        return True

    def tick(self, t_buf, ts_table):
        L = nat.lib()
        if self.time_steps:
            nat.check(L.lfvdm_sampler_tick_fetch(_p(t_buf), _p(ts_table), _p(self.tin), self.B, _p(self.rows_all), self.rows_ld,
                                                 _p(self.rows), self.film_floats, nat.stream()), "lfvdm_sampler_tick_fetch")
        else:
            nat.check(L.lfvdm_sampler_tick(_p(t_buf), _p(ts_table), _p(self.tin), self.B, nat.stream()), "lfvdm_sampler_tick")

    def autotune(self, rounds=3, reps=6):
        L = nat.lib()
        cache = nat.tune_cache()
        tuned = 0
        for fn, args in self.steps:
            if fn is not L.lfvdm_conv_igemm:
                continue
            a = args[0]._obj
            key = nat.tune_key(a)
            if (level_chain_enabled() and a.N * a.Ho * a.Wo <= CHAIN_MAX_M and a.out_mode == nat.OUT_ROWS
                    and self._local_tiles(a) == 0):
                ckey = key + (nat.TUNE_CHAIN,)
                if ckey not in cache:
                    cache[ckey] = nat.autotune_launch(a, rounds, reps, chain_only=True)
                if cache[ckey]:
                    a.tune = cache[ckey]
                    tuned += 1
                    continue
            if key not in cache:
                cache[key] = nat.autotune_launch(a, rounds, reps)
            a.tune = cache[key]
            tuned += 1
        self.tuned = True
        nat.tune_cache_save()
        n_chains = self.build_chains()
        for fn, args in self.steps:
            if fn is L.lfvdm_conv_igemm:
                a = args[0]._obj
                key = nat.tune_key(a)
                if cache.get(key + (nat.TUNE_CHAIN,)) and a.tune == cache[key + (nat.TUNE_CHAIN,)]:
                    if key not in cache:
                        cache[key] = nat.autotune_launch(a, rounds, reps)
                    a.tune = cache[key]
        nat.tune_cache_save()
        if n_chains and os.environ.get("LFVDM_CHAIN_TUNE", "1") != "0":
            self.tune_chains()
        return tuned

    def _local_tiles(self, a):
        L = nat.lib()
        if not (chain_local_enabled() and level_chain_enabled()) or a.N * a.Ho * a.Wo > CHAIN_MAX_M or a.out_mode != nat.OUT_ROWS:
            return 0
        forced = int(os.environ.get("LFVDM_CHAIN_LOCAL_RT", "0")) or int(nat.tune_cache().get(nat.tune_key(a) + (nat.TUNE_LOCAL_RT,), 0))
        M, NS = a.N * a.Ho * a.Wo, a.Cout // 16
        order = (1, 2) if -(-M // 16) * NS <= 256 else (2, 1)
        for rt in ((forced,) if forced else order):
            if L.lfvdm_chain_local_ok(C.byref(a), rt) == 0:
                return rt
        return 0

    def _chain_stage(self, step):
        L = nat.lib()
        fn, args = step
        st = nat.ChainStage()
        if fn is L.lfvdm_conv_igemm:
            a = args[0]._obj
            rt = self._local_tiles(a)
            if rt:
                st.kind, st.cfg = nat.CHAIN_LOCAL, rt
                C.memmove(C.byref(st.conv), C.byref(a), C.sizeof(nat.ConvArgs))
                return st
            if a.N * a.Ho * a.Wo > CHAIN_MAX_M or L.lfvdm_chain_conv_ok(C.byref(a)) != 0:
                return None
            st.kind = nat.CHAIN_CONV
            C.memmove(C.byref(st.conv), C.byref(a), C.sizeof(nat.ConvArgs))
            return st
        if fn is L.lfvdm_gn_apply_part:
            (src, Cp, N, P, cg, gamma, beta, eps, act, out, ldo) = args
            if N * P > CHAIN_MAX_M or L.lfvdm_chain_gn_ok(Cp, 0, N, P) != 0:
                return None
            st.kind = nat.CHAIN_GN
            g = st.gn
            g.src0, g.src1, g.C0, g.C1, g.N, g.P = src, None, Cp, 0, N, P
# ... 198 lines not shown
            runs.append((self._step_pos[id(run[0][0])], run))
        if os.environ.get("LFVDM_SKIP_SIDE", "1") != "0":
            for step, _ in getattr(self, "skip_side", []):
                for _, r in runs:
                    for sp, st in r:
                        if sp is step and any(not x.side and x is not st for _, x in r):
                            st.side = 1
        out = []
        for pos, step in sorted([(p, ("run", r)) for p, r in runs if r] + [(p, ("step", sp)) for p, sp in lone], key=lambda e: e[0]):
            if step[0] == "step":
                out.append(step[1])
                continue
            r = step[1]
            single = len(r) == 1 and r[0][1].kind == nat.CHAIN_LOCAL and os.environ.get("LFVDM_CHAIN_SINGLE", "0") == "1"
            ch = self._make_chain(r) if len(r) >= 2 or single else None
            if ch is None:
                out.extend(sp for sp, _ in r)
            else:
                self.chains.append(ch)
                out.append(ch["step"])
        self.steps = out
        if head_last:
            self.head["step"] = len(self.steps) - 1
        return len(self.chains)

    def disable_chains(self):
        if not self.chains:
            self.chains_off = True
            return
        head_last = self.head["step"] == len(self.steps) - 1
        by_step = {id(ch["step"]): ch for ch in self.chains}
        out = []
        for step in self.steps:
            ch = by_step.get(id(step))
            out.extend(ch["steps"] if ch is not None else [step])
        self.steps, self.chains, self.chains_off = out, [], True
        if head_last:
            self.head["step"] = len(self.steps) - 1

    def split_chains(self):
        if not self.chains:
            return 0
        head_last = self.head["step"] == len(self.steps) - 1
        by_step = {id(ch["step"]): ch for ch in self.chains}
        out, n = [], 0
        for step in self.steps:
            ch = by_step.get(id(step))
            if ch is None:
                out.append(step)
                continue
            for sp, st in self._launch_order(ch["run"]):
                one = self._make_chain([(sp, st)])
                assert one is not None
                out.append(one["step"])
                n += 1
        self.steps, self.chains, self.chains_off = out, [], True
        if head_last:
            self.head["step"] = len(self.steps) - 1
        return n

    def chains_aborted(self):
        if not self.chains:
            return False
        return bool(th.stack([ch["ctl"][nat.CHAIN_CTL_ABORT] for ch in self.chains]).ne(0).any().item())

    def weight_signature(self):
        return (self.engine.epoch,) + tuple(e[0]._version for e in self.packs)

    def time_signature(self):
        return self.weight_signature() + tuple(t._version for t in self._time_params)

    def refresh_weights(self):
        s = nat.stream()
        L = nat.lib()
        for w, out, *part in self.packs:
            if part == ["up2x"]:
                nat.check(L.lfvdm_pack_conv_weight_up2x(_p(w), _p(out), w.shape[0], w.shape[1], s), "pack_up2x")
                continue
            if part:
                w = w.detach()[:, part[0]:part[1]].contiguous()
            nat.check(L.lfvdm_pack_conv_weight(_p(w), _p(out), w.shape[0], w.shape[1], w.shape[2], s), "pack")
        self._sig = self.weight_signature()

    def launch(self, tick=None):
        L = nat.lib()
        s = nat.stream()
        for fn, args in self.steps:
            if tick is not None and fn is L.lfvdm_conv_in:
                rc = L.lfvdm_conv_in_tick(*args, _p(tick[0]), _p(tick[1]), _p(self.tin), self.B, _p(self.rows_all),
                                          self.rows_ld, _p(self.rows), self.film_floats, s)
                tick = None
            else:
                rc = fn(*args, s)
            if rc:
                nat.check(rc, getattr(fn, "__name__", "kernel"))
        assert tick is None, "the plan has no lfvdm_conv_in launch to carry the clock"

    def set_inputs(self, x, x0, timesteps, frame_indices, obs_mask, latent_mask):
        B, T = self.B, self.T
        if x.data_ptr() != self.x_in.data_ptr():
            self.x_in.copy_(x)
        if x0.data_ptr() != self.x0_in.data_ptr():
            self.x0_in.copy_(x0)
        ob = obs_mask.reshape(B, T).to(th.float32)
        self.obs.copy_(ob.reshape(-1))
        th.clamp(ob + latent_mask.reshape(B, T).to(th.float32), max=1.0, out=self.mask)
        self.fi.copy_(frame_indices)
        self.tin[:B].copy_(timesteps)


class Engine:

    def __init__(self, model):
        nat.lib()
        self.model = model
        self.plans = {}
        self.epoch = 0
        for p in model.parameters():
            if p.dtype != th.float32:
                raise RuntimeError("the native path is fp32 (use_fp16 is off in the reference defaults)")

    def plan(self, B, T, H, W, want_attn=False):
        key = (B, T, H, W, bool(want_attn))
        pl = self.plans.get(key)
        if pl is None:
            pl = Plan(self, B, T, H, W, bool(want_attn))
            pl.refresh_weights()
            self.plans[key] = pl
        elif pl._sig != pl.weight_signature():
            pl.refresh_weights()
        return pl

    def invalidate(self):
        self.epoch += 1
        nat.param_epoch[0] += 1

    def forward(self, x, x0, timesteps, frame_indices, obs_mask, latent_mask, return_attn_weights=False):
        B, T, Cx, H, W = x.shape
        grad_needed = th.is_grad_enabled() and (x.requires_grad or any(p.requires_grad for p in self.model.parameters()))
        if grad_needed or (self.model.training and self.model.dropout > 0):
            from ._autograd import unet_apply
            return unet_apply(self, x, x0, timesteps, frame_indices, obs_mask, latent_mask, return_attn_weights)
        pl = self.plan(B, T, H, W, return_attn_weights)
        pl.set_inputs(x.detach(), x0.detach(), timesteps, frame_indices, obs_mask, latent_mask)
        pl.launch()
        out = pl.out.clone()
        attns = None
        if return_attn_weights:
            attns = {"spatial": [a.mean(dim=1).abs() for a in pl.attn_s],
                     "temporal": [a.mean(dim=1).abs() for a in pl.attn_t], "mixed": []}
        return out, attns
```

### latent-flexible-video-diffusion-modeling_amd/improved_diffusion/_native.py

```python
import atexit
import ctypes as C
import json
import os

import torch

_HERE = os.path.dirname(os.path.abspath(__file__))
LIB_PATH = os.environ.get("LFVDM_LIB_PATH") or os.path.join(os.path.dirname(_HERE), "lib", "liblfvdm_hip.so")

ACT_NONE, ACT_SILU = 0, 1
OUT_ROWS, OUT_NCHW = 0, 1

_lib = None

c_fp = C.c_void_p
c_i = C.c_int


class ConvArgs(C.Structure):
    _fields_ = [
        ("src0", c_fp), ("src1", c_fp), ("C0", C.c_int32), ("C1", C.c_int32), ("N", C.c_int32),
        ("Hs", C.c_int32), ("Ws", C.c_int32), ("up", C.c_int32), ("stride", C.c_int32), ("ksize", C.c_int32),
        ("Ho", C.c_int32), ("Wo", C.c_int32), ("coefA", c_fp), ("coefB", c_fp), ("act", C.c_int32),
        ("W", c_fp), ("bias", c_fp), ("Cout", C.c_int32),
        ("s2src0", c_fp), ("s2src1", c_fp), ("s2C0", C.c_int32), ("s2C1", C.c_int32), ("W2", c_fp), ("bias2", c_fp),
        ("res", c_fp), ("ldr", C.c_int32), ("resA", c_fp), ("resB", c_fp),
        ("out", c_fp), ("ldo", C.c_int32), ("out_mode", C.c_int32), ("tune", C.c_int32),
        ("splitk_ws", c_fp), ("splitk_cnt", c_fp), ("splitk_ws_floats", C.c_int64), ("splitk_cnt_ints", C.c_int64),
        ("gn_gamma", c_fp), ("gn_beta", c_fp), ("gn_film", c_fp), ("gn_out", c_fp), ("gn_film_ld", C.c_int32),
        ("gn_film_div", C.c_int32), ("gn_act", C.c_int32), ("gn_skip_raw", C.c_int32), ("gn_eps", C.c_float),
        ("gn_general", C.c_int32), ("gn_gw", C.c_int32), ("gn_ld", C.c_int32),
    ]


class GnArgs(C.Structure):
    _fields_ = [("src0", c_fp), ("src1", c_fp), ("C0", C.c_int32), ("C1", C.c_int32), ("N", C.c_int32), ("P", C.c_int32),
                ("gamma", c_fp), ("beta", c_fp), ("film", c_fp), ("film_div", C.c_int32), ("film_ld", C.c_int32),
                ("eps", C.c_float), ("act", C.c_int32), ("out", c_fp), ("cg", C.c_int32), ("ldo", C.c_int32), ("out_base", c_fp),
                ("out_col", C.c_int32), ("pad_", C.c_int32)]


class ChainStage(C.Structure):
    _fields_ = [("kind", C.c_int32), ("n_items", C.c_int32), ("flag_base", C.c_int32), ("n_flags", C.c_int32),
                ("dep_base", C.c_int32), ("dep_stride", C.c_int32), ("cfg", C.c_int32), ("kz", C.c_int32), ("nt2", C.c_int32),
                ("wg_off", C.c_int32), ("side", C.c_int32), ("wg_lo", C.c_int32), ("wg_count", C.c_int32), ("ws_off", C.c_int64), ("cnt_off", C.c_int64), ("conv", ConvArgs), ("gn", GnArgs)]


CHAIN_CONV, CHAIN_GN, CHAIN_LOCAL = 0, 1, 2
CHAIN_CTL_EPOCH, CHAIN_CTL_EXIT, CHAIN_CTL_ABORT, CHAIN_CTL_INTS = 0, 32, 64, 96


class AdamWArgs(C.Structure):
    _fields_ = [("p", c_fp), ("g", c_fp), ("m", c_fp), ("v", c_fp), ("ema", c_fp * 4), ("ema_rate", C.c_float * 4),
                ("n_ema", C.c_int32), ("n", C.c_int64), ("lr", C.c_float), ("beta1", C.c_float), ("beta2", C.c_float),
                ("eps", C.c_float), ("weight_decay", C.c_float), ("bias_corr1", C.c_float), ("bias_corr2_sqrt", C.c_float),
                ("grad_scale", C.c_float), ("grad_sqsum", c_fp), ("skip_flag", c_fp), ("skip_flag2", c_fp)]


class RowdotJob(C.Structure):
    _fields_ = [("W", c_fp), ("b", c_fp), ("inp", c_fp), ("out", c_fp), ("K", C.c_int32), ("O", C.c_int32),
                ("M", C.c_int32), ("ldin", C.c_int32), ("ldout", C.c_int32), ("in_mode", C.c_int32),
                ("row0", C.c_int32), ("pad_", C.c_int32)]


class RowdotBwdJob(C.Structure):
    _fields_ = [("W", c_fp), ("inp", c_fp), ("dout", c_fp), ("dW", c_fp), ("db", c_fp), ("din", c_fp), ("K", C.c_int32),
                ("O", C.c_int32), ("M", C.c_int32), ("ldin", C.c_int32), ("lddout", C.c_int32), ("lddin", C.c_int32),
                ("in_mode", C.c_int32), ("task0", C.c_int32)]


class PackJob(C.Structure):
    _fields_ = [("src", c_fp), ("dst", c_fp), ("Cout", C.c_int32), ("Cin", C.c_int32), ("taps", C.c_int32),
                ("transposed", C.c_int32), ("blk0", C.c_int32), ("ld", C.c_int32)]


param_epoch = [0]


class UnpackJob(C.Structure):
    _fields_ = [("gp", c_fp), ("g", c_fp), ("Cout", C.c_int32), ("Cin", C.c_int32), ("taps", C.c_int32), ("row0", C.c_int32),
                ("ldp", C.c_int32), ("pad_", C.c_int32)]


class RpeJob(C.Structure):
    _fields_ = [("tproj", c_fp), ("Wd", c_fp), ("bd", c_fp), ("Wout", c_fp), ("bout", c_fp), ("R", c_fp),
                ("C", C.c_int32), ("tile0", C.c_int32), ("tproj_ld", C.c_int32), ("pad_", C.c_int32), ("act", c_fp)]


class RpeBwdJob(C.Structure):
    _fields_ = [("tproj", c_fp), ("Wd", c_fp), ("bd", c_fp), ("Wout_t", c_fp), ("dR", c_fp), ("dtproj", c_fp),
                ("dWd", c_fp), ("dbd", c_fp), ("C", C.c_int32), ("tile0", C.c_int32), ("tproj_ld", C.c_int32),
                ("dtproj_ld", C.c_int32)]


class WgradJob(C.Structure):
    _fields_ = [("a", ConvArgs), ("msplit", C.c_int32), ("task0", C.c_int32)]


_SIGS = {
    "lfvdm_abi_version": ([], c_i),
    "lfvdm_conv_igemm": ([C.POINTER(ConvArgs), c_fp], c_i),
    "lfvdm_conv_igemm_config": ([C.POINTER(ConvArgs), C.POINTER(c_i), C.POINTER(c_i)], c_i),
    "lfvdm_conv_igemm_candidates": ([C.POINTER(ConvArgs), C.POINTER(c_i), c_i], c_i),
    "lfvdm_pack_conv_weight": ([c_fp, c_fp, c_i, c_i, c_i, c_fp], c_i),
    "lfvdm_pack_conv_weight_up2x": ([c_fp, c_fp, c_i, c_i, c_fp], c_i),
    "lfvdm_conv_wgrad": ([C.POINTER(ConvArgs), c_fp], c_i),
    "lfvdm_pack_conv_weight_t": ([c_fp, c_fp, c_i, c_i, c_i, c_fp], c_i),
    "lfvdm_unpack_conv_grad": ([c_fp, c_fp, c_i, c_i, c_i, c_i, c_fp], c_i),
    "lfvdm_unpack_conv_grads": ([c_fp, c_i, c_i, c_i, c_fp], c_i),
    "lfvdm_pack_conv_weights": ([c_fp, c_i, c_i, c_fp], c_i),
    "lfvdm_conv_in": ([c_fp] * 6 + [c_i] * 5 + [c_fp], c_i),
    "lfvdm_gn_coef": ([c_fp, c_fp, c_i, c_i, c_i, c_i, c_fp, c_fp, c_fp, c_i, c_i, C.c_float, c_fp, c_fp, c_fp], c_i),
    "lfvdm_gn_coef_stats": ([c_fp, c_fp, c_i, c_i, c_i, c_i, c_fp, c_fp, c_fp, c_i, c_i, C.c_float, c_fp, c_fp, c_fp, c_fp], c_i),
    "lfvdm_gn_apply": ([c_fp, c_fp, c_i, c_i, c_i, c_i, c_fp, c_fp, c_fp, c_i, c_i, C.c_float, c_i, c_fp, c_fp, c_fp, c_fp, c_fp], c_i),
    "lfvdm_gn_apply_part": ([c_fp, c_i, c_i, c_i, c_i, c_fp, c_fp, C.c_float, c_i, c_fp, c_i, c_fp], c_i),
    "lfvdm_gn_apply_ws_floats": ([c_i, c_i, c_i], C.c_long),
    "lfvdm_gn_apply_ws": ([c_fp, c_fp, c_i, c_i, c_i, c_i, c_fp, c_fp, c_fp, c_i, c_i, C.c_float, c_i, c_fp, c_fp, c_fp, c_fp, c_fp,
                           C.c_long, c_fp], c_i),
    "lfvdm_compose_rows": ([c_fp, c_fp, c_fp, c_fp, c_i, c_i, c_i, c_i, c_i, c_fp], c_i),
    "lfvdm_conv_in_tick": ([c_fp, c_fp, c_fp, c_fp, c_fp, c_fp, c_i, c_i, c_i, c_i, c_i, c_fp, c_fp, c_fp, c_i, c_fp, c_i, c_fp, c_i,
                            c_fp], c_i),
    "lfvdm_conv_out_psample_ok": ([c_i] * 5, c_i),
    "lfvdm_update_x0": ([c_fp] * 9 + [c_i, c_i, c_i] + [c_fp] * 3 + [c_i, c_i, c_fp], c_i),
    "lfvdm_update_rng_x0": ([c_fp] * 9 + [c_i, c_i, c_i] + [c_fp] * 3 + [c_i, c_i, c_fp, c_fp], c_i),
    "lfvdm_conv_out_update_x0": ([c_fp] * 13 + [c_i, c_i, c_i] + [c_fp] * 3 + [c_i] * 6 + [c_fp, c_fp], c_i),
    "lfvdm_update_ms_x0": ([c_fp] * 9 + [c_i, c_i] + [c_fp] * 2 + [c_i, c_i, c_fp], c_i),
    "lfvdm_conv_out_update_ms_x0": ([c_fp] * 12 + [c_i, c_i] + [c_fp] * 2 + [c_i] * 6 + [c_fp], c_i),
    "lfvdm_known_blend": ([c_fp] * 9 + [c_i] * 4 + [c_fp], c_i),
    "lfvdm_renoise": ([c_fp] * 6 + [c_i, c_i, c_fp], c_i),
    "lfvdm_masked_mse_bwd": ([c_fp, c_fp, c_fp, c_fp, c_fp, c_i, c_i, c_i, c_fp], c_i),
    "lfvdm_vb_terms": ([c_fp] * 12 + [c_i, c_i] + [c_fp] * 4 + [c_i] * 5 + [c_fp], c_i),
    "lfvdm_vb_terms_bwd": ([c_fp] * 11 + [c_i, c_i, c_fp, c_i, c_i, c_i, c_fp], c_i),
    "lfvdm_gn_bwd_stats": ([c_fp, c_fp, c_fp, c_i, c_i, c_i, c_i, c_fp, c_fp, c_fp, c_i, c_fp, c_fp], c_i),
    "lfvdm_gn_bwd_apply": ([c_fp, c_fp, c_fp, c_i, c_i, c_i, c_i, c_fp, c_fp, c_fp, c_fp, c_i, c_fp, c_fp, c_i, c_i, c_fp], c_i),
    "lfvdm_gn_bwd_apply_params": ([c_fp, c_fp, c_fp, c_i, c_i, c_i, c_i, c_fp, c_fp, c_fp, c_fp, c_i, c_fp, c_fp, c_i, c_i,
                                   c_fp, c_fp, c_fp, c_i, c_i, c_fp, c_fp, c_fp, c_i, c_fp, c_i, c_fp], c_i),
    "lfvdm_gn_bwd_fused_sums": ([c_fp, c_fp, c_fp, c_i, c_i, c_i, c_i, c_fp, c_fp, c_fp, c_i, c_fp, c_fp, c_fp, c_i, c_fp, c_i,
                                 c_fp, c_fp], c_i),
    "lfvdm_gn_bwd_ws_floats": ([c_i, c_i, c_i], C.c_long),
    "lfvdm_gn_bwd_ws": ([c_fp, c_fp, c_fp, c_i, c_i, c_i, c_i, c_fp, c_fp, c_fp, c_i, c_fp, c_fp, c_fp, c_fp, c_fp, c_i, c_i,
                         c_fp, c_fp, c_fp, c_i, c_fp, c_i, c_fp, c_i, c_fp, c_fp, C.c_long, c_fp], c_i),
    "lfvdm_gn_bwd_fused": ([c_fp, c_fp, c_fp, c_i, c_i, c_i, c_i, c_fp, c_fp, c_fp, c_i, c_fp, c_fp, c_fp, c_fp, c_fp, c_i, c_i,
                            c_fp, c_fp, c_fp, c_i, c_fp, c_i, c_fp, c_i, c_fp], c_i),
    "lfvdm_gn_param_grads": ([c_fp, c_fp, c_fp, c_fp, c_i, c_i, c_fp, c_fp, c_fp, c_i, c_i, c_i, c_fp], c_i),
    "lfvdm_rowdot_bwd": ([c_fp, c_i, c_i, c_fp], c_i),
    "lfvdm_gn_temporal_bwd": ([c_fp, c_fp, c_fp, C.c_float, c_fp, c_fp, c_fp, c_i, c_i, c_i, c_i, c_i, c_fp], c_i),
    "lfvdm_gn_temporal": ([c_fp, c_fp, c_fp, C.c_float, c_fp, c_i, c_i, c_i, c_i, c_fp], c_i),
    "lfvdm_gn_temporal_qkv_ok": ([c_i, c_i, c_i, c_i], c_i),
    "lfvdm_proj_gn_ok": ([c_i, c_i, c_i], c_i),
    "lfvdm_proj_gn": ([c_fp, c_fp, c_fp, c_fp, c_fp, c_fp, C.c_float, c_i, c_fp, c_fp, c_i, c_i, c_i, c_fp], c_i),
    "lfvdm_gn_temporal_qkv": ([c_fp, c_fp, c_fp, C.c_float, c_fp, c_fp, c_fp, c_fp, c_i, c_i, c_i, c_i, c_fp], c_i),
    "lfvdm_rowdot": ([c_fp, c_i, c_i, c_fp], c_i),
    "lfvdm_silu": ([c_fp, c_fp, C.c_int64, c_fp], c_i),
    "lfvdm_rpe_nets": ([c_fp, c_i, c_i, c_fp, c_i, c_i, c_fp], c_i),
    "lfvdm_rpe_nets_maxc": ([c_fp, c_i, c_i, c_fp, c_i, c_i, c_i, c_fp], c_i),
    "lfvdm_rpe_nets_bwd": ([c_fp, c_i, c_i, c_fp, c_i, c_i, c_fp], c_i),
    "lfvdm_conv_wgrad_grouped": ([c_fp, c_i, c_i, c_fp], c_i),
    "lfvdm_attn_spatial": ([c_fp, c_fp, c_fp, c_fp, c_i, c_i, c_i, c_i, c_fp], c_i),
    "lfvdm_attn_spatial_fused_ok": ([c_i, c_i, c_i, c_i], c_i),
    "lfvdm_attn_spatial_fused": ([c_fp, c_fp, c_fp, c_fp, c_i, c_i, c_i, c_i, c_fp], c_i),
    "lfvdm_det_reduce": ([c_fp, c_fp, C.c_long, C.c_long, c_fp], c_i),
    "lfvdm_gn_temporal_bwd_det": ([c_fp, c_fp, c_fp, C.c_float, c_fp, c_fp, c_fp, c_i, c_i, c_i, c_i, c_i, c_fp, C.c_int64, c_fp], c_i),
    "lfvdm_rowdot_bwd_det": ([c_fp, c_i, c_i, c_fp, C.c_int64, c_fp, C.c_int64, c_fp], c_i),
    "lfvdm_rpe_nets_bwd_det": ([c_fp, c_i, c_i, c_fp, c_i, c_i, c_fp, C.c_int64, c_fp], c_i),
    "lfvdm_rpe_front": ([c_fp, c_i, c_fp, c_fp, c_fp, c_fp, c_i, c_i, c_i, c_fp], c_i),
    "lfvdm_rpe_front_bwd": ([c_fp, c_i, c_fp, c_fp, c_fp, c_fp, c_fp, c_i, c_fp, c_fp, c_i, c_i, c_i, c_fp], c_i),
    "lfvdm_sampler_tick": ([c_fp, c_fp, c_fp, c_i, c_fp], c_i),
    "lfvdm_sampler_tick_fetch": ([c_fp, c_fp, c_fp, c_i, c_fp, c_i, c_fp, c_i, c_fp], c_i),
    "lfvdm_attn_temporal_sel": ([c_fp] * 7 + [c_i] * 5 + [c_fp, c_fp], c_i),
    "lfvdm_attn_temporal_ring": ([c_fp] * 7 + [c_i] * 5 + [c_fp, c_i, c_fp], c_i),
    "lfvdm_attn_temporal_bwd": ([c_fp] * 12 + [c_i] * 5 + [c_fp], c_i),
    "lfvdm_attn_spatial_bwd": ([c_fp] * 6 + [c_i, c_i, c_i, c_i, c_fp], c_i),
    "lfvdm_attn_temporal": ([c_fp] * 7 + [c_i] * 5 + [c_fp], c_i),
    "lfvdm_adamw_ema": ([C.POINTER(AdamWArgs), c_fp], c_i),
    "lfvdm_grad_norm_nparts": ([C.c_int64], c_i),
    "lfvdm_grad_norm_partials": ([c_fp, C.c_int64, C.c_float, c_fp, c_i, c_fp], c_i),
    "lfvdm_grad_norm_finalize": ([c_fp, c_i, C.c_float, c_fp, c_fp], c_i),
    "lfvdm_adamw_ema_clip": ([C.POINTER(AdamWArgs), c_fp, c_fp], c_i),
    "lfvdm_q_sample": ([c_fp] * 6 + [c_i, c_i, c_fp], c_i),
    "lfvdm_masked_mse": ([c_fp] * 4 + [c_i, c_i, c_i, c_fp], c_i),
    "lfvdm_train_loss": ([c_fp] * 6 + [c_i] + [c_fp] * 3 + [c_i, c_i, c_i, c_fp], c_i),
    "lfvdm_train_loss_bwd": ([c_fp] * 5 + [c_i, c_fp, c_fp, c_i, c_i, c_i, c_fp], c_i),
    "lfvdm_prepare_batch": ([c_fp] * 6 + [c_i] * 4 + [c_fp], c_i),
    "lfvdm_search_assemble": ([c_fp] * 9 + [c_i] * 5 + [c_fp], c_i),
    "lfvdm_search_noise_qsample": ([c_fp] * 10 + [c_i] * 4 + [c_fp], c_i),
    "lfvdm_search_noise_fill": ([c_fp, C.c_uint64, c_i, c_i, c_fp] + [c_i] * 4 + [c_fp], c_i),
    "lfvdm_search_scores": ([c_fp, c_fp, c_fp] + [c_i] * 5 + [c_fp], c_i),
    "lfvdm_chain_plan": ([C.POINTER(ChainStage), c_i, C.POINTER(C.c_int32), C.c_int64, C.POINTER(C.c_int64), C.POINTER(C.c_int32),
                          C.POINTER(C.c_int64), C.POINTER(C.c_int64), C.POINTER(C.c_int32), C.POINTER(C.c_int32)], c_i),
    "lfvdm_chain_conv_ok": ([C.POINTER(ConvArgs)], c_i),
    "lfvdm_chain_gn_ok": ([c_i, c_i, c_i, c_i], c_i),
    "lfvdm_chain_local_ok": ([C.POINTER(ConvArgs), c_i], c_i),
    "lfvdm_chain_capacity": ([c_i], c_i),
    "lfvdm_level_chain": ([c_fp, c_i, c_fp, c_fp, c_fp, c_i, c_i, C.c_double, c_fp], c_i),
    "lfvdm_flag_add": ([c_fp, c_fp], c_i),
    "lfvdm_flag_wait": ([c_fp, c_i, C.c_double, c_fp, c_fp], c_i),
    "lfvdm_flag_wait2": ([c_fp, c_i, C.c_double, c_fp, c_fp, c_fp], c_i),
}

EXPORTS = tuple(_SIGS)


def lib():
    global _lib
    if _lib is None:
        if not os.path.exists(LIB_PATH):
            raise RuntimeError(
                f"native library {LIB_PATH} is missing - build it with "
                "`python latent-flexible-video-diffusion-modeling_amd/build.py` (there is no fallback path)")
        L = C.CDLL(LIB_PATH)
# ... 358 lines not shown


def rowdot(jobs_dev, njobs, total_rows):
    check(lib().lfvdm_rowdot(ptr(jobs_dev, torch.uint8), njobs, total_rows, stream()), "lfvdm_rowdot")


def rpe_nets(jobs_dev, njobs, total_tiles, frame_indices, B, T):
    check(lib().lfvdm_rpe_nets(ptr(jobs_dev, torch.uint8), njobs, total_tiles, ptr(frame_indices, torch.int64), B, T,
                               stream()), "lfvdm_rpe_nets")


def attn_spatial(qkv, o, attn_out, N, P, Cc, heads, lse=None):
    check(lib().lfvdm_attn_spatial(ptr(qkv), ptr(o), ptr(attn_out), ptr(lse), N, P, Cc, heads, stream()),
          "lfvdm_attn_spatial")


def attn_spatial_bwd(qkv, o, d_o, lse, delta_ws, dqkv, N, P, Cc, heads):
    check(lib().lfvdm_attn_spatial_bwd(ptr(qkv), ptr(o), ptr(d_o), ptr(lse), ptr(delta_ws), ptr(dqkv), N, P, Cc, heads,
                                       stream()), "lfvdm_attn_spatial_bwd")


def attn_temporal(qkv, Rq, Rk, Rv, mask, o, attn_out, B, T, P, Cc, heads):
    check(lib().lfvdm_attn_temporal(ptr(qkv), ptr(Rq), ptr(Rk), ptr(Rv), ptr(mask), ptr(o), ptr(attn_out), B, T, P, Cc,
                                    heads, stream()), "lfvdm_attn_temporal")


def attn_temporal_bwd(qkv, d_o, Rq, Rk, Rv, mask, ws_p, ws_ds, dqkv, dRq, dRk, dRv, B, T, P, Cc, heads):
    check(lib().lfvdm_attn_temporal_bwd(ptr(qkv), ptr(d_o), ptr(Rq), ptr(Rk), ptr(Rv), ptr(mask), ptr(ws_p), ptr(ws_ds),
                                        ptr(dqkv), ptr(dRq), ptr(dRk), ptr(dRv), B, T, P, Cc, heads, stream()),
          "lfvdm_attn_temporal_bwd")


def q_sample(x0, noise, t, sa, sb, out):
    B = x0.shape[0]
    check(lib().lfvdm_q_sample(ptr(x0), ptr(noise), ptr(t, torch.int64), ptr(sa), ptr(sb), ptr(out), B,
                               x0.numel() // B, stream()), "lfvdm_q_sample")


RULE_ANCESTRAL, RULE_DDIM = 0, 1
MEAN_EPS, MEAN_X0 = 0, 1
RULE_DPMPP2M = "dpmpp2m"


def update_x0(x, out, noise, t, recip, recipm1, c1, c2, sg, rule, mean_type, clip, sample, pred=None, mean=None):
    B = x.shape[0]
    check(lib().lfvdm_update_x0(ptr(x), ptr(out), ptr(noise), ptr(t, torch.int64), ptr(recip), ptr(recipm1), ptr(c1), ptr(c2),
                                ptr(sg), int(rule), int(mean_type), int(bool(clip)), ptr(sample), ptr(pred), ptr(mean), B,
                                x.numel() // B, stream()), "lfvdm_update_x0")


def update_rng_x0(x, out, noise_out, t, recip, recipm1, c1, c2, sg, rule, mean_type, clip, sample, seed, pred=None, mean=None):
    B = x.shape[0]
    check(lib().lfvdm_update_rng_x0(ptr(x), ptr(out), ptr(noise_out), ptr(t, torch.int64), ptr(recip), ptr(recipm1), ptr(c1),
                                    ptr(c2), ptr(sg), int(rule), int(mean_type), int(bool(clip)), ptr(sample), ptr(pred),
                                    ptr(mean), B, x.numel() // B, ptr(seed, torch.int64) if seed is not None else None, stream()),
          "lfvdm_update_rng_x0")


def conv_out_update_x0(act, wp, bias, out, x, noise_in, noise_out, t, recip, recipm1, c1, c2, sg, rule, mean_type, clip, sample,
                       seed, pred=None, mean=None):
    B, T, Cout, H, W = x.shape
    check(lib().lfvdm_conv_out_update_x0(ptr(act), ptr(wp), ptr(bias), ptr(out), ptr(x), ptr(noise_in), ptr(noise_out),
                                         ptr(t, torch.int64), ptr(recip), ptr(recipm1), ptr(c1), ptr(c2), ptr(sg), int(rule),
                                         int(mean_type), int(bool(clip)), ptr(sample), ptr(pred), ptr(mean), B, T, H, W,
                                         act.shape[-1], Cout, ptr(seed, torch.int64) if seed is not None else None, stream()),
          "lfvdm_conv_out_update_x0")


def update_ms_x0(x, out, hist, t, recip, recipm1, k1, k2, k3, mean_type, clip, sample, pred=None):
    B = x.shape[0]
    check(lib().lfvdm_update_ms_x0(ptr(x), ptr(out), ptr(hist), ptr(t, torch.int64), ptr(recip), ptr(recipm1), ptr(k1), ptr(k2),
                                   ptr(k3), int(mean_type), int(bool(clip)), ptr(sample), ptr(pred), B, x.numel() // B, stream()),
          "lfvdm_update_ms_x0")


def conv_out_update_ms_x0(act, wp, bias, out, x, hist, t, recip, recipm1, k1, k2, k3, mean_type, clip, sample, pred=None):
    B, T, Cout, H, W = x.shape
    check(lib().lfvdm_conv_out_update_ms_x0(ptr(act), ptr(wp), ptr(bias), ptr(out), ptr(x), ptr(hist), ptr(t, torch.int64),
                                            ptr(recip), ptr(recipm1), ptr(k1), ptr(k2), ptr(k3), int(mean_type), int(bool(clip)),
                                            ptr(sample), ptr(pred), B, T, H, W, act.shape[-1], Cout, stream()),
          "lfvdm_conv_out_update_ms_x0")


def known_blend(x, known, mask, t, a, s, eps=None, seed=None, noise_out=None):
    B, T, Cx, H, W = x.shape
    if known.shape != x.shape or tuple(mask.shape) != (B, T, H, W) or (eps is not None and eps.shape != x.shape):
        raise RuntimeError("known_blend: known / eps are shaped like x (B, T, C, H, W) and mask is (B, T, H, W)")
    check(lib().lfvdm_known_blend(ptr(x), ptr(known), ptr(mask), ptr(eps), ptr(noise_out), ptr(t, torch.int64), ptr(a), ptr(s),
                                  ptr(seed, torch.int64) if seed is not None else None, B, T, Cx, H * W, stream()),
          "lfvdm_known_blend")


def renoise(x, t, c, d, seed, noise_out=None):
    B = x.shape[0]
    check(lib().lfvdm_renoise(ptr(x), ptr(noise_out), ptr(t, torch.int64), ptr(c), ptr(d), ptr(seed, torch.int64), B,
                              x.numel() // B, stream()), "lfvdm_renoise")


def vb_terms(x_start, x_t, out, noise, t, recip, recipm1, c1, c2, post_logvar, model_logvar, mask, mean_type, clip, vb,
             xstart_mse=None, eps_mse=None, pred=None, col_base=-1):
    B, T = x_t.shape[0], x_t.shape[1]
    ld = vb.shape[1] if vb.dim() == 2 else 1
    check(lib().lfvdm_vb_terms(ptr(x_start), ptr(x_t), ptr(out), ptr(noise), ptr(t, torch.int64), ptr(recip), ptr(recipm1), ptr(c1),
                               ptr(c2), ptr(post_logvar), ptr(model_logvar), ptr(mask), int(mean_type), int(bool(clip)), ptr(vb),
                               ptr(xstart_mse), ptr(eps_mse), ptr(pred), B, T, x_t.numel() // (B * T), ld, int(col_base),
                               stream()), "lfvdm_vb_terms")


def vb_terms_bwd(x_start, x_t, out, t, recip, recipm1, c1, c2, model_logvar, mask, g, mean_type, clip, d_out):
    B, T = x_t.shape[0], x_t.shape[1]
    check(lib().lfvdm_vb_terms_bwd(ptr(x_start), ptr(x_t), ptr(out), ptr(t, torch.int64), ptr(recip), ptr(recipm1), ptr(c1), ptr(c2),
                                   ptr(model_logvar), ptr(mask), ptr(g), int(mean_type), int(bool(clip)), ptr(d_out), B, T,
                                   x_t.numel() // (B * T), stream()), "lfvdm_vb_terms_bwd")


def prepare_batch(pool, table, batch, frame_indices, obs_mask, latent_mask):
    B, Tp = pool.shape[:2]
    F = table.shape[1]
    check(lib().lfvdm_prepare_batch(ptr(pool), ptr(table, torch.int32), ptr(batch), ptr(frame_indices, torch.int64), ptr(obs_mask),
                                    ptr(latent_mask), B, F, Tp, pool[0, 0].numel(), stream()), "lfvdm_prepare_batch")


def masked_mse(a, b, mask, out, B, T, frame_inner):
    check(lib().lfvdm_masked_mse(ptr(a), ptr(b), ptr(mask), ptr(out), B, T, frame_inner, stream()), "lfvdm_masked_mse")


def train_loss(target, pred, mask, eval_mask, t, wtab, mse, eval_mse, loss):
    B, T = pred.shape[0], pred.shape[1]
    check(lib().lfvdm_train_loss(ptr(target), ptr(pred), ptr(mask), ptr(eval_mask), ptr(t, torch.int64), ptr(wtab), wtab.numel(),
                                 ptr(mse), ptr(eval_mse), ptr(loss), B, T, pred.numel() // (B * T), stream()), "lfvdm_train_loss")


def train_loss_bwd(target, pred, mask, t, wtab, g, dpred):
    B, T = pred.shape[0], pred.shape[1]
    check(lib().lfvdm_train_loss_bwd(ptr(target), ptr(pred), ptr(mask), ptr(t, torch.int64), ptr(wtab), wtab.numel(), ptr(g),
                                     ptr(dpred), B, T, pred.numel() // (B * T), stream()), "lfvdm_train_loss_bwd")


def grad_norm_nparts(n):
    return int(lib().lfvdm_grad_norm_nparts(int(n)))


def grad_clip_stat(g, grad_scale, max_norm, partials, stat):
    n = g.numel()
    if partials.numel() != grad_norm_nparts(n) or stat.numel() != 4:
        raise RuntimeError("grad_clip_stat: partials must hold grad_norm_nparts(n) floats and stat four")
    check(lib().lfvdm_grad_norm_partials(ptr(g), n, float(grad_scale), ptr(partials), partials.numel(), stream()),
          "lfvdm_grad_norm_partials")
    check(lib().lfvdm_grad_norm_finalize(ptr(partials), partials.numel(), float(max_norm), ptr(stat), stream()),
          "lfvdm_grad_norm_finalize")


def adamw_ema_clip(a, stat):
    check(lib().lfvdm_adamw_ema_clip(C.byref(a), ptr(stat), stream()), "lfvdm_adamw_ema_clip")


class StreamFlags:

    def __init__(self, n, device):
        self.buf = torch.zeros(n + 1, 32, device=device, dtype=torch.int32)
        self.n = n

    def add(self, k):
        check(lib().lfvdm_flag_add(self.buf[k].data_ptr(), stream()), "lfvdm_flag_add")

    def wait(self, k, target, torch_stream, timeout_s=20.0, also_f32=None):
# ... 48 lines not shown
```

### latent-flexible-video-diffusion-modeling_amd/improved_diffusion/_replay.py

```python
import torch as th

from . import _native as nat


class ReplayedStep:

    def __init__(self, diffusion, unet, shape, clip_denoised, inject_noise, time_tables=True):
        self.diffusion, self.unet, self.shape = diffusion, unet, tuple(shape)
        self.clip = bool(clip_denoised)
        self.inject_noise = bool(inject_noise)
        diffusion._check_native_modes()
        self.x0_mode = diffusion.predicts_xstart
        B, T, Cx, H, W = self.shape
        from ._engine import Plan
        self.engine = unet.native_engine()
        self.plan = Plan(self.engine, B, T, H, W, False, time_steps=diffusion.num_timesteps if time_tables else None)
        self.plan.refresh_weights()
        dev = self.plan.dev
        self.tb = diffusion.tables(dev)
        self.ts_table = diffusion.model_timestep_table(dev)
        self.t_buf = self.plan.t_sel if self.plan.time_steps else th.zeros(B, dtype=th.int64, device=dev)
        self._table_events = None
        self._ts_key = tuple(self.ts_table.tolist())
        self.graph = None
# ... 2 lines not shown
        self.chain_timeouts = 0

    @property
    def table_build_ms(self):
        if self._table_events is None:
            return 0.0
        e0, e1 = self._table_events
        e1.synchronize()
        return e0.elapsed_time(e1)

    def _build_chain_tables(self, frame_indices):
        pl, n = self.plan, self.diffusion.num_timesteps
        if not pl.time_steps:
            return
        e0, e1 = th.cuda.Event(enable_timing=True), th.cuda.Event(enable_timing=True)
        e0.record()
        if pl.tables_sig != (pl.time_signature(), self._ts_key):
            pl.build_time_tables(self.ts_table)
        pl.build_R_tables(frame_indices)
        pl.ensure_R(n - 1)
        e1.record()
        self._table_events = (e0, e1)
        self.t_buf.fill_(n)
        pl.tick(self.t_buf, self.ts_table)

    def _capture_step(self):
        import os
        pl = self.plan
        rng_state = th.cuda.get_rng_state(pl.dev)
        if os.environ.get("LFVDM_AUTOTUNE", "1") != "0" and not getattr(pl, "tuned", False):
            saved0 = pl.x_in.clone()
            pl.launch()
            pl.autotune()
            pl.x_in.copy_(saved0)
        saved = pl.x_in.clone()
        self.t_buf.fill_(self.diffusion.num_timesteps)
        s = th.cuda.Stream()
        s.wait_stream(th.cuda.current_stream())
        with th.cuda.stream(s):
            self._step_body()
        th.cuda.current_stream().wait_stream(s)
        g = th.cuda.CUDAGraph()
        with th.cuda.graph(g, capture_error_mode="thread_local"):
            self._step_body()
        self.graph = g
        pl.x_in.copy_(saved)
        th.cuda.synchronize()
        th.cuda.set_rng_state(rng_state, pl.dev)

    def _begin_chain(self, x, model_kwargs):
        pl = self.plan
        if pl._sig != pl.weight_signature():
            pl.refresh_weights()
        with th.no_grad():
            pl.set_inputs(x, model_kwargs["x0"], th.zeros(pl.B, device=pl.dev), model_kwargs["frame_indices"],
                          model_kwargs["obs_mask"], model_kwargs["latent_mask"])
            self._build_chain_tables(model_kwargs["frame_indices"])
            if self.graph is None:
                self._capture_step()
            self.t_buf.fill_(self.diffusion.num_timesteps)
        self.expected_t = self.diffusion.num_timesteps - 1

    def chain_timed_out(self):
        self._abort_unchecked = False
        return bool(self.plan.chains) and self.plan.chains_aborted()

    def fall_back(self):
        import sys
        print("[lfvdm] ERROR: a persistent level chain timed out (lfvdm_level_chain); falling back to the per-launch plan",
              file=sys.stderr, flush=True)
        self.plan.disable_chains()
        self.graph = None
        self.chain_timeouts += 1

    def step(self, i):
        if i != self.expected_t:
            self.t_buf.fill_(i + 1)
        self.plan.ensure_R(i)
        self.graph.replay()
        self._abort_unchecked = True
        self.expected_t = max(i - 1, 0)


class GraphSampler(ReplayedStep):

    def __init__(self, diffusion, unet, shape, clip_denoised, inject_noise=False, rule=("ancestral",)):
        self.rule = tuple(rule)
        if self.rule[0] not in ("ancestral", "ddim", "dpmpp2m") or len(self.rule) != (2 if self.rule[0] == "ddim" else 1):
            raise ValueError(f"unknown update rule {rule!r}")
        super().__init__(diffusion, unet, shape, clip_denoised, inject_noise)
        dev = self.plan.dev
        self.multistep = self.rule[0] == "dpmpp2m"
        if self.multistep:
            self.ddim = diffusion.dpm_solver_tables(dev)
        else:
            self.ddim = diffusion.ddim_tables(dev, self.rule[1]) if self.rule[0] == "ddim" else None
        self.update = diffusion._update_args(dev, self.rule)
        self.noise = th.empty(self.shape, device=dev)
        self.pred = th.empty(self.shape, device=dev)
        self.seed = th.zeros(1, dtype=th.int64, device=dev)
        import os
        self.K = max(1, int(os.environ.get("LFVDM_STEPS_PER_GRAPH", "8")))
        if self.plan.time_steps and self.plan.time_ring:
            self.K = min(self.K, self.plan.time_ring // 2)
        self.graph_k = None
        self.known = self.known_mask = self.known_eps = self.known_noise = self.known_tb = None

    def enable_known_region(self, fixed_noise, record_noise=False):
        if self.graph is not None or self.graph_k is not None:
            raise RuntimeError("enable_known_region comes before the sampler's first chain: its graphs are captured already")
        B, T, _, H, W = self.shape
        dev = self.plan.dev
        self.known_tb = self.diffusion.known_region_tables(dev)
        self.known = th.zeros(self.shape, device=dev)
        self.known_mask = th.zeros(B, T, H, W, device=dev)
        self.known_eps = th.zeros(self.shape, device=dev) if fixed_noise else None
        self.known_noise = th.zeros(self.shape, device=dev) if record_noise and not fixed_noise else None

    def _step_body(self):
        self._denoise_body()
        if self.known is not None:
            nat.known_blend(self.plan.x_in, self.known, self.known_mask, self.t_buf, self.known_tb["a"], self.known_tb["s"],
                            eps=self.known_eps, seed=self.seed, noise_out=self.known_noise)
            self.extra_launches += 1

    def renoise(self):
        tb = self.known_tb
        nat.renoise(self.plan.x_in, self.t_buf, tb["sqrt_1mbeta"], tb["sqrt_beta"], self.seed)

    def _denoise_body(self):
        import os
        pl = self.plan
        recip, recipm1, c1, c2, sg, rule, mean_type = self.update
        det = sg is None or self.multistep
        in_kernel = det or (not self.inject_noise and os.environ.get("LFVDM_SAMPLER_NOISE", "kernel") != "torch")
        fused = (os.environ.get("LFVDM_FUSED_HEAD", "1") != "0" and (in_kernel or self.inject_noise)
                 and pl.fuse_head_update(self.t_buf, self.tb, self.clip, self.seed, self.noise, self.pred, self.inject_noise,
                                         ddim=self.ddim, predict_xstart=self.x0_mode))
        tick_in_conv = bool(pl.time_steps) and os.environ.get("LFVDM_TICK_IN_CONV", "1") != "0"
        if tick_in_conv:
            pl.launch(tick=(self.t_buf, self.ts_table))
        else:
            pl.tick(self.t_buf, self.ts_table)
            pl.launch()
        draw = not (fused or in_kernel or self.inject_noise)
        self.extra_launches = int(not tick_in_conv) + int(not fused) + int(draw)
        if fused:
            return
        if self.multistep:
            nat.update_ms_x0(pl.x_in, pl.out, self.pred, self.t_buf, recip, recipm1, c1, c2, sg, mean_type, self.clip, pl.x_in,
                             self.pred)
            return
        if in_kernel:
            nat.update_rng_x0(pl.x_in, pl.out, None if det else self.noise, self.t_buf, recip, recipm1, c1, c2, sg, rule,
                              mean_type, self.clip, pl.x_in, None if det else self.seed, self.pred)
            return
        if draw:
            self.noise.normal_()
        nat.update_x0(pl.x_in, pl.out, self.noise, self.t_buf, recip, recipm1, c1, c2, sg, rule, mean_type, self.clip, pl.x_in,
                      self.pred)

    def begin(self, img, model_kwargs, known=None, known_mask=None, known_eps=None):
        if self._abort_unchecked and self.chain_timed_out():
            self.fall_back()
        if (self.known is None) != (known is None) or (self.known_eps is None) != (known_eps is None):
            raise ValueError("known / known_mask (and known_eps under a fixed-noise rule) go to a sampler made with "
                             "enable_known_region, and to no other")
        if known is not None:
            self.known.copy_(known)
            self.known_mask.copy_(known_mask)
            if known_eps is not None:
                self.known_eps.copy_(known_eps)
        self._begin_chain(img, model_kwargs)
        self.seed.random_()
        if self.multistep:
            self.pred.zero_()

    def fall_back(self):
        super().fall_back()
        self.graph_k = None

    def chain_table_ms(self):
        pl = self.plan
        if not pl.time_steps:
            return 0.0
        e0, e1 = th.cuda.Event(enable_timing=True), th.cuda.Event(enable_timing=True)
        th.cuda.synchronize()
        e0.record()
        pl.fill_whole_chain()
        e1.record()
        e1.synchronize()
        if self.expected_t is not None:
            pl.ensure_R(self.expected_t)
        return e0.elapsed_time(e1)

    def _state(self):
        return {"sample": self.plan.x_in, "pred_xstart": self.pred, "attn": None}

    def _check_order(self, i):
        if self.multistep and i != self.expected_t and i != self.diffusion.num_timesteps - 1:
            raise ValueError(f"the multistep rule {self.rule!r} walks consecutive timesteps: expected t = {self.expected_t} "
                             f"(or {self.diffusion.num_timesteps - 1}, a new chain), got {i}")

    def step(self, i):
        self._check_order(i)
        super().step(i)
        return self._state()

    def run(self, i, n):
        if self.inject_noise and n > 1:
            raise ValueError("inject_noise: the caller provides the noise of every step - use step()")
        self._check_order(i)
        if i != self.expected_t:
            self.t_buf.fill_(i + 1)
        left, t = int(n), int(i)
        if self.K > 1 and left >= self.K:
            if self.graph_k is None:
                g = th.cuda.CUDAGraph()
                th.cuda.synchronize()
                with th.no_grad(), th.cuda.graph(g, capture_error_mode="thread_local"):
                    for _ in range(self.K):
                        self._step_body()
                self.graph_k = g
            while left >= self.K:
                self.plan.ensure_R(t, t - self.K + 1)
                self.graph_k.replay()
                left -= self.K
                t = max(t - self.K, 0)
        for _ in range(left):
            self.plan.ensure_R(t)
            self.graph.replay()
            t = max(t - 1, 0)
        self._abort_unchecked = True
        self.expected_t = max(int(i) - int(n), 0)
        return self._state()


class BpdEvaluator(ReplayedStep):

    def __init__(self, diffusion, unet, shape, clip_denoised, inject_noise=False):
        super().__init__(diffusion, unet, shape, clip_denoised, inject_noise)
        assert self.plan.time_steps == diffusion.num_timesteps and self.plan.t_sel is not None
        B, T, n, dev = self.plan.B, self.plan.T, diffusion.num_timesteps, self.plan.dev
        self.x_start = th.empty(self.shape, device=dev)
        self.noise = th.empty(self.shape, device=dev)
        self.mask = th.ones(B, T, device=dev)
        self.vb, self.xstart_mse, self.mse = (th.zeros(B, n, device=dev) for _ in range(3))

    def _step_body(self):
        pl, tb, d = self.plan, self.tb, self.diffusion
        pl.tick(self.t_buf, self.ts_table)
        if not self.inject_noise:
            self.noise.normal_()
        nat.q_sample(self.x_start, self.noise, self.t_buf, tb["sqrt_alphas_cumprod"], tb["sqrt_one_minus_alphas_cumprod"], pl.x_in)
        pl.launch()
        recip, recipm1, c1, c2, post_lv, model_lv = d._vb_tables(pl.dev)
        nat.vb_terms(self.x_start, pl.x_in, pl.out, self.noise, self.t_buf, recip, recipm1, c1, c2, post_lv, model_lv, self.mask,
                     nat.MEAN_X0 if self.x0_mode else nat.MEAN_EPS, self.clip, self.vb, self.xstart_mse, self.mse, None,
                     col_base=d.num_timesteps - 1)

    def begin(self, x_start, model_kwargs, latent_mask=None):
        with th.no_grad():
            self.x_start.copy_(x_start)
            if latent_mask is None:
                self.mask.fill_(1.0)
            else:
                self.mask.copy_(latent_mask.reshape(self.mask.shape))
        self._begin_chain(self.x_start, model_kwargs)

    def evaluate(self, x_start, model_kwargs, latent_mask=None):
        n = self.diffusion.num_timesteps
        for attempt in range(2):
            self.begin(x_start, model_kwargs, latent_mask)
            for i in range(n - 1, -1, -1):
                self.step(i)
            if attempt == 0 and self.chain_timed_out():
                self.fall_back()
                continue
            break
        return self.vb.clone(), self.xstart_mse.clone(), self.mse.clone()
```

Before: 1264.

## Fuse step boundary: output head, sampler update, clock tick, next conv_in and GroupNorm

Adds a step_seam kernel that fuses the last stage of one denoising step (output conv head plus sampler update) with the first stages of the next step (timestep tick, row fetch, input conv via MFMA, first GroupNorm). A grid-wide atomic ticket lets the last block advance the clock. Inside the K-step CUDA graph, consecutive steps are joined at these seams to cut kernel launches and global round trips between steps. In exchange it adds a large LDS footprint, a ticket-counter synchronisation, and a warm-up call that saves and restores state.

```diff
diff --git a/include/lfvdm_hip.h b/include/lfvdm_hip.h
--- a/include/lfvdm_hip.h
+++ b/include/lfvdm_hip.h
@@ -292,6 +292,34 @@
                                 const float* hist, const int64_t* t, const float* sqrt_recip_acp, const float* sqrt_recipm1_acp,
                                 const float* k1, const float* k2, const float* k3, int mean_type, int clip, float* sample,
                                 float* pred_xstart, int B, int T, int H, int W, int C, int Cout, void* stream);
+typedef struct lfvdm_step_seam_args {
+    const float *act, *Wp, *bias_out;
+    float* out;
+    const float* x;
+    const float* noise_in;
+    float* noise_out;
+    int64_t* t;
+    const float *sqrt_recip_acp, *sqrt_recipm1_acp, *c1, *c2, *sg, *hist, *k3;
+    float *sample, *pred_xstart, *mean_out;
+    const int64_t* seed;
+    int32_t rule, mean_type, clip, multistep;
+    int32_t B, T, H, W, C, Cx;
+    const float *x0, *obs, *w_in, *bias_in;
+    float* h0;
+    const float *gamma, *beta;
+    float* gn_out;
+    float eps;
+    int32_t rows_ld, row_floats, pad_;
+    const float* clock_table;
+    float* model_t;
+    const float* rows_all;
+    float* rows;
+    int32_t* ticket;
+} lfvdm_step_seam_args;
+int lfvdm_step_seam_ok(int N, int H, int W, int C, int Cx);
+int lfvdm_step_seam_gn_ok(int N, int H, int W, int C, int Cx);
+int lfvdm_step_seam(const lfvdm_step_seam_args* a, void* stream);
+
 int lfvdm_known_blend(float* x, const float* known, const float* mask, const float* eps, float* noise_out, const int64_t* t,
                       const float* sqrt_acp_prev, const float* sqrt_1macp_prev, const int64_t* seed, int B, int T, int C,
                       int HW, void* stream);
diff --git a/latent-flexible-video-diffusion-modeling_amd/csrc/conv_in_body.h b/latent-flexible-video-diffusion-modeling_amd/csrc/conv_in_body.h
--- /dev/null
+++ b/latent-flexible-video-diffusion-modeling_amd/csrc/conv_in_body.h
@@ -0,0 +1,134 @@
+#pragma once
+#include <stdlib.h>
+
+#include "common_hip.h"
+
+namespace {
+
+struct ConvInTick {
+    int64_t* t;
+    const float* table;
+    float* model_t;
+    const float* rows_all;
+    float* rows;
+    int B, rows_ld, row_floats;
+};
+
+__device__ __forceinline__ void conv_in_clock(const ConvInTick& tk, int64_t* tnew) {
+    if ((int)threadIdx.x < tk.B) {
+        int64_t v = tk.t[threadIdx.x] - 1;
+        v = v < 0 ? 0 : v;
+        tk.t[threadIdx.x] = v;
+        tnew[threadIdx.x] = v;
+    }
+    __syncthreads();
+    if ((int)threadIdx.x < tk.B) tk.model_t[threadIdx.x] = tk.table[tnew[threadIdx.x]];
+    const int q4 = tk.row_floats >> 2;
+    for (int b = 0; b < tk.B; ++b) {
+        const float* src = tk.rows_all + ((size_t)tnew[b] * tk.B + b) * tk.rows_ld;
+        float* dst = tk.rows + (size_t)b * tk.rows_ld;
+        for (int i0 = threadIdx.x; i0 < q4; i0 += 256 * 8) {
+            f32x4 v[8];
+#pragma unroll
+            for (int u = 0; u < 8; ++u) {
+                const int i = i0 + 256 * u;
+                v[u] = i < q4 ? ld4(src + 4 * i) : (f32x4){0.f, 0.f, 0.f, 0.f};
+            }
+#pragma unroll
+            for (int u = 0; u < 8; ++u) {
+                const int i = i0 + 256 * u;
+                if (i < q4) st4(dst + 4 * i, v[u]);
+            }
+        }
+    }
+}
+
+template <int NCT, int CI>
+struct ConvInMfma {
+    static constexpr int Cout = 16 * NCT, C = CI - 1, K = 9 * CI, KP = (K + 3) & ~3, KS = KP + 1;
+    static constexpr int NKI = KP / 4;
+    static constexpr int A_FLOATS = 64 * KS, W_FLOATS = Cout * KS;
+
+    struct Filt { float v[Cout / 4]; };
+    struct Patch { float xa[NKI], xb[NKI]; bool inb[NKI]; };
+
+    static __device__ __forceinline__ Filt filt_load(const float* __restrict__ w, int wave, int lane) {
+        Filt f;
+#pragma unroll
+        for (int i = 0; i < Cout / 4; ++i) f.v[i] = lane < K ? w[(size_t)(wave + 4 * i) * K + lane] : 0.f;
+        return f;
+    }
+    static __device__ __forceinline__ void filt_store(const Filt& f, float* Ws, int wave, int lane) {
+#pragma unroll
+        for (int i = 0; i < Cout / 4; ++i)
+            if (lane < KP) Ws[(wave + 4 * i) * KS + lane] = f.v[i];
+    }
+    static __device__ __forceinline__ Patch patch_load(const float* xn, const float* x0n, int H, int W, int oy, int ox, int pq,
+                                                       bool live, int wave) {
+        Patch p;
+        const int HW = H * W;
+#pragma unroll
+        for (int i = 0; i < NKI; ++i) {
+            const int k = wave + 4 * i;
+            const int ci = k / 9, tap = k - ci * 9;
+            const int iy = oy + tap / 3 - 1, ix = ox + tap % 3 - 1;
+            p.inb[i] = live && k < K && iy >= 0 && iy < H && ix >= 0 && ix < W;
+            const int ip = p.inb[i] ? iy * W + ix : pq;
+            const int cc = ci < C ? ci : 0;
+            p.xa[i] = xn[cc * HW + ip];
+            p.xb[i] = x0n[cc * HW + ip];
+        }
+        return p;
+    }
+    static __device__ __forceinline__ void patch_store(const Patch& p, float ob, float* As, int wave, int lane) {
+#pragma unroll
+        for (int i = 0; i < NKI; ++i) {
+            const int k = wave + 4 * i;
+            const int ci = k / 9;
+            float v = ci < C ? p.xa[i] * (1.0f - ob) + p.xb[i] * ob : ob;
+            As[lane * KS + k] = p.inb[i] ? v : 0.f;
+        }
+    }
+    static __device__ __forceinline__ void mma(const float* As, const float* Ws, const float* __restrict__ bias, int wave, int lane,
+                                               f32x4 (&acc)[NCT]) {
+        const int r16 = lane & 15, kq = lane >> 4;
+#pragma unroll
+        for (int c = 0; c < NCT; ++c) {
+            const float b = bias[16 * c + r16];
+            acc[c] = (f32x4){b, b, b, b};
+        }
+        const float* ar = As + (16 * wave + r16) * KS + kq;
+        const float* wr = Ws + r16 * KS + kq;
+#pragma unroll
+        for (int s4 = 0; s4 < KP; s4 += 4) {
+            const float a = ar[s4];
+#pragma unroll
+            for (int c = 0; c < NCT; ++c) acc[c] = __builtin_amdgcn_mfma_f32_16x16x4f32(a, wr[16 * c * KS + s4], acc[c], 0, 0, 0);
+        }
+    }
+    static __device__ __forceinline__ void out_store(const f32x4 (&acc)[NCT], float* __restrict__ out, long p0, long total, int lane) {
+        const int r16 = lane & 15;
+#pragma unroll
+        for (int r = 0; r < 4; ++r) {
+            if (p0 + r < total) {
+                float* o = out + (size_t)(p0 + r) * Cout + r16;
+#pragma unroll
+                for (int c = 0; c < NCT; ++c) o[16 * c] = acc[c][r];
+            }
+        }
+    }
+};
+
+inline bool conv_in_takes_mfma(int C, int Cout) {
+    static const bool off = getenv("LFVDM_CONV_IN_SCALAR") != nullptr;
+    return !off && (C == 4 || C == 3) && (Cout == 64 || Cout == 128);
+}
+inline int gn_wave_width(int C0, int C1, int N, int P) {
+    static const bool off = getenv("LFVDM_GN_NO_WAVE") != nullptr;
+    static const int minp4 = getenv("LFVDM_GN_WAVE4_MINP") ? atoi(getenv("LFVDM_GN_WAVE4_MINP")) : 128;
+    const int C = C0 + C1, cg = C / 32;
+    if (off || P > 256 || C0 % 16 || (cg != 2 && cg != 4 && cg != 8 && cg != 16) || N > 65535) return 0;
+    return minp4 > 0 && P >= minp4 && P % 64 == 0 ? 4 : 1;
+}
+
+}
diff --git a/latent-flexible-video-diffusion-modeling_amd/csrc/diffusion_ops.hip b/latent-flexible-video-diffusion-modeling_amd/csrc/diffusion_ops.hip
--- a/latent-flexible-video-diffusion-modeling_amd/csrc/diffusion_ops.hip
+++ b/latent-flexible-video-diffusion-modeling_amd/csrc/diffusion_ops.hip
@@ -1,4 +1,7 @@
 #include "common_hip.h"
+#include "conv_in_body.h"
+#include "gn_wave_body.h"
+#include "head_update_body.h"
 #include "philox_normal.h"
 
 namespace {
@@ -16,49 +19,6 @@
             for (int j = i; j < inner; ++j) out[base + j] = ca * x0[base + j] + cb * noise[base + j];
         }
     }
-}
-
-enum { RULE_ANCESTRAL = 0, RULE_DDIM = 1, RULE_DDIM_DET = 2, RULE_DPMPP2M = 3 };
-constexpr bool rule_draws(int rule) { return rule == RULE_ANCESTRAL || rule == RULE_DDIM; }
-
-enum { MEAN_EPS = 0, MEAN_X0 = 1 };
-
-template <int MEAN>
-__device__ __forceinline__ float mean_x0hat(float r, float rm1, float xv, float out) {
-    return MEAN == MEAN_X0 ? out : r * xv - rm1 * out;
-}
-
-template <int RULE>
-__device__ __forceinline__ float rule_sigma(const float* __restrict__ t_logvar, int64_t tb) {
-    if (RULE == RULE_ANCESTRAL) return tb != 0 ? expf(0.5f * t_logvar[tb]) : 0.f;
-    if (RULE == RULE_DDIM) return tb != 0 ? t_logvar[tb] : 0.f;
-    return 0.f;
-}
-
-struct StepCoef { float r, rm1, c1, c2, sigma; };
-
-template <int RULE, int MEAN>
-__device__ __forceinline__ StepCoef step_coef(int64_t tb, const float* t_recip, const float* t_recipm1, const float* t_c1,
-                                              const float* t_c2, const float* t_logvar) {
-    return {MEAN == MEAN_EPS ? t_recip[tb] : 0.f, MEAN == MEAN_EPS ? t_recipm1[tb] : 0.f, t_c1[tb], t_c2[tb],
-            rule_sigma<RULE>(t_logvar, tb)};
-}
-
-template <int MEAN>
-__device__ __forceinline__ float step_mean(const StepCoef& k, float xv, float out, int clip, float& p0) {
-    p0 = mean_x0hat<MEAN>(k.r, k.rm1, xv, out);
-    if (clip) p0 = fminf(fmaxf(p0, -1.f), 1.f);
-    return k.c1 * p0 + k.c2 * xv;
-}
-
-template <int MEAN>
-__device__ __forceinline__ float multistep_mean(const StepCoef& k, float k3, float xv, float out, int clip, const float* hist,
-                                                size_t at, float& p0) {
-    p0 = MEAN == MEAN_X0 ? out : __fmaf_rn(k.r, xv, -__fmul_rn(k.rm1, out));
-    if (clip) p0 = fminf(fmaxf(p0, -1.f), 1.f);
-    float mean = __fmaf_rn(k.c2, xv, __fmul_rn(k.c1, p0));
-    if (k3 != 0.f) mean = __fmaf_rn(k3, __fsub_rn(p0, hist[at]), mean);
-    return mean;
 }
 
 template <int RULE> struct PredOut { typedef float* __restrict__ ptr; };
@@ -123,34 +83,12 @@
     }
 }
 
-struct HeadUpdate {
-    const float *act, *Wp, *bias, *x, *noise_in;
-    float *eps_out, *noise_out, *sample, *pred, *mean_out;
-    const int64_t *t, *seed;
-    const float *t_recip, *t_recipm1, *t_c1, *t_c2, *t_logvar;
-    int N, T, H, W, C, clip;
-    const float *hist, *t_k3;
-};
-
 template <int CO, int CPL, int RULE, int MEAN>
 __global__ __launch_bounds__(256) void conv_out_psample_kernel(const HeadUpdate p) {
     extern __shared__ __attribute__((aligned(16))) float wl[];
     const int tid = threadIdx.x;
     const int C = p.C;
-    {
-        constexpr int NW4 = CO * 9 * 16 * CPL, NIT = (NW4 + 255) / 256;
-        f32x4 wv[NIT];
-#pragma unroll
-        for (int u = 0; u < NIT; ++u) {
-            const int i = tid + 256 * u;
-            wv[u] = i < NW4 ? ld4(p.Wp + 4 * (size_t)i) : (f32x4){0.f, 0.f, 0.f, 0.f};
-        }
-#pragma unroll
-        for (int u = 0; u < NIT; ++u) {
-            const int i = tid + 256 * u;
-            if (i < NW4) st4(wl + 4 * i, wv[u]);
-        }
-    }
+    head_stage_filters<CO, CPL>(p.Wp, wl, tid);
     __syncthreads();
     const int lane = tid & 63, wave = tid >> 6;
     const int WQ = p.W >> 2;
@@ -161,59 +99,9 @@
     const int y = rem / WQ, xq = rem - y * WQ;
     const int j = lane >> 4, cl = lane & 15;
     const int x = 4 * xq + j;
-    float acc[CO];
-#pragma unroll
-    for (int co = 0; co < CO; ++co) acc[co] = 0.f;
-#pragma unroll
-    for (int tap = 0; tap < 9; ++tap) {
-        const int iy = y + tap / 3 - 1, ix = x + tap % 3 - 1;
-        const bool inb = iy >= 0 && iy < p.H && ix >= 0 && ix < p.W;
-        const float* a = p.act + ((size_t)(n * p.H + (inb ? iy : y)) * p.W + (inb ? ix : x)) * C;
-#pragma unroll
-        for (int u = 0; u < CPL; ++u) {
-            const int c = (cl + 16 * u) * 4;
-            f32x4 a4 = ld4(a + c);
-            if (!inb) a4 = (f32x4){0.f, 0.f, 0.f, 0.f};
-#pragma unroll
-            for (int co = 0; co < CO; ++co) {
-                const f32x4 w4 = ld4(wl + (co * 9 + tap) * C + c);
-                acc[co] += (a4.x * w4.x + a4.y * w4.y) + (a4.z * w4.z + a4.w * w4.w);
-            }
-        }
-    }
-#pragma unroll
-    for (int co = 0; co < CO; ++co)
-#pragma unroll
-        for (int o = 1; o < 16; o <<= 1) acc[co] += __shfl_xor(acc[co], o, 64);
+    const float e = head_conv_pixel<CO, CPL>(p.act + (size_t)n * p.H * p.W * C, wl, p.H, p.W, C, y, x, cl);
     if (cl >= CO) return;
-    float e = acc[0];
-#pragma unroll
-    for (int co = 1; co < CO; ++co) e = cl == co ? acc[co] : e;
-    const int co = cl;
-    e += p.bias[co];
-    const int b = n / p.T, tt = n - b * p.T;
-    const int inner = p.T * CO * p.H * p.W;
-    const int i = ((tt * CO + co) * p.H + y) * p.W + x;
-    const size_t at = (size_t)b * inner + i;
-    const int64_t tb = p.t[b];
-    const StepCoef k = step_coef<RULE, MEAN>(tb, p.t_recip, p.t_recipm1, p.t_c1, p.t_c2, p.t_logvar);
-    float z = 0.f;
-    if (!rule_draws(RULE)) {
-    } else if (p.noise_in) {
-        z = p.noise_in[at];
-    } else {
-        const unsigned long long key = (unsigned long long)p.seed[0];
-        const f32x4 z4 = normal4((unsigned)(i >> 2), (unsigned)b, (unsigned)tb, (unsigned)key, (unsigned)(key >> 32));
-        z = j == 0 ? z4.x : j == 1 ? z4.y : j == 2 ? z4.z : z4.w;
-    }
-    float p0;
-    const float mean = RULE == RULE_DPMPP2M ? multistep_mean<MEAN>(k, p.t_k3[tb], p.x[at], e, p.clip, p.hist, at, p0)
-                                            : step_mean<MEAN>(k, p.x[at], e, p.clip, p0);
-    p.sample[at] = rule_draws(RULE) ? mean + k.sigma * z : mean;
-    if (p.eps_out) p.eps_out[at] = e;
-    if (rule_draws(RULE) && p.noise_out) p.noise_out[at] = z;
-    if (p.pred) p.pred[at] = p0;
-    if (p.mean_out) p.mean_out[at] = mean;
+    head_update_elem<CO, RULE, MEAN>(p, e, n, y, x, j, cl, p.t[n / p.T]);
 }
 
 __global__ __launch_bounds__(1024) void masked_mse_kernel(const float* __restrict__ a, const float* __restrict__ bb,
@@ -504,6 +392,188 @@
                         [&](auto r, auto m) { return launch_head<decltype(r)::value, decltype(m)::value>(p, Cout, stream); });
 }
 
+namespace {
+struct SeamFront {
+    const float *x0, *obs, *w, *bias;
+    float* h0;
+    const float *gamma, *beta;
+    float* gn_out;
+    float eps;
+    ConvInTick tk;
+    int* ticket;
+    const float *gn_s1, *gn_film;
+    float *gn_coefA, *gn_coefB, *gn_stats;
+    int gn_C1, gn_film_div, gn_film_ld, gn_act, gn_ldo;
+};
+
+template <int CO>
+struct SeamLds {
+    typedef ConvInMfma<4, CO + 1> M;
+    static constexpr int C = 64;
+    static constexpr int WL = CO * 9 * C;
+    static size_t bytes(int P) { return sizeof(float) * ((size_t)WL + M::W_FLOATS + M::A_FLOATS + (size_t)CO * P + (size_t)P * C); }
+};
+
+__device__ __noinline__ void seam_gn(const float* __restrict__ s0, const float* __restrict__ s1, int C0, int C1, int P,
+                                     const float* __restrict__ gamma, const float* __restrict__ beta,
+                                     const float* __restrict__ film, int film_div, int film_ld, float eps,
+                                     float* __restrict__ coefA, float* __restrict__ coefB, float* __restrict__ stats,
+                                     float* __restrict__ act_out, int act_mode, int ldo, int n, int wave, int lane) {
+    gn_wave_body<2, false>(n, wave, lane, s0, s1, C0, C1, P, gamma, beta, film, film_div, film_ld, eps, coefA, coefB, stats, act_out,
+                           act_mode, ldo);
+}
+
+template <int CO, int RULE, int MEAN>
+__global__ __launch_bounds__(256) void step_seam_kernel(const HeadUpdate p, const SeamFront f) {
+    typedef SeamLds<CO> L;
+    typedef typename L::M M;
+    constexpr int C = L::C;
+    extern __shared__ __attribute__((aligned(16))) float sm[];
+    __shared__ int64_t s_t[64];
+    __shared__ int s_last;
+    const int P = p.H * p.W;
+    float* wl = sm;
+    float* Ws = wl + L::WL;
+    float* As = Ws + M::W_FLOATS;
+    float* xs = As + M::A_FLOATS;
+    float* af = xs + CO * P;
+    const int tid = threadIdx.x, lane = tid & 63, wave = __builtin_amdgcn_readfirstlane(tid >> 6);
+    const int n = blockIdx.x;
+    if (tid == 0) {
+        const int64_t tb = p.t[n / p.T];
+        s_t[0] = tb;
+        int last = 0;
+        if (f.tk.t != nullptr) {
+            __threadfence();
+            last = atomicAdd(f.ticket, 1) == (int)gridDim.x - 1;
+            if (last) *f.ticket = 0;
+        }
+        s_last = last;
+    }
+    const typename M::Filt wv = M::filt_load(f.w, wave, lane);
+    head_stage_filters<CO, 1>(p.Wp, wl, tid);
+    M::filt_store(wv, Ws, wave, lane);
+    {
+        const float* src = p.act + (size_t)n * P * C;
+        const int total4 = P * (C / 4);
+        for (int i0 = tid; i0 < total4; i0 += 256 * 8) {
+            f32x4 v[8];
+#pragma unroll
+            for (int u = 0; u < 8; ++u) {
+                const int i = i0 + 256 * u;
+                v[u] = i < total4 ? ld4(src + 4 * (size_t)i) : (f32x4){0.f, 0.f, 0.f, 0.f};
+            }
+#pragma unroll
+            for (int u = 0; u < 8; ++u) {
+                const int i = i0 + 256 * u;
+                if (i < total4) st4(af + 4 * i, v[u]);
+            }
+        }
+    }
+    __syncthreads();
+    const int64_t tb = s_t[0];
+    const bool clock = s_last != 0;
+    {
+        const int WQ = p.W >> 2, j = lane >> 4, cl = lane & 15;
+        for (int quad = wave; quad < p.H * WQ; quad += 4) {
+            const int y = quad / WQ, x = 4 * (quad - y * WQ) + j;
+            const float e = head_conv_pixel<CO, 1>(af, wl, p.H, p.W, C, y, x, cl);
+            if (cl < CO) xs[cl * P + y * p.W + x] = head_update_elem<CO, RULE, MEAN, true>(p, e, n, y, x, j, cl, tb);
+        }
+    }
+    __syncthreads();
+    if (clock) conv_in_clock(f.tk, s_t);
+    const float ob = f.obs[n];
+    const float* x0n = f.x0 + (size_t)n * CO * P;
+    for (int p0 = 0; p0 < P; p0 += 64) {
+        const int pix = p0 + lane;
+        const bool live = pix < P;
+        const int pq = live ? pix : P - 1;
+        const int oy = pq / p.W, ox = pq - oy * p.W;
+        const typename M::Patch pt = M::patch_load(xs, x0n, p.H, p.W, oy, ox, pq, live, wave);
+        if (p0) __syncthreads();
+        M::patch_store(pt, ob, As, wave, lane);
+        __syncthreads();
+        f32x4 acc[4];
+        M::mma(As, Ws, f.bias, wave, lane, acc);
+        M::out_store(acc, f.h0, (long)n * P + p0 + 16 * wave + 4 * (lane >> 4), (long)n * P + P, lane);
+    }
+    if (f.gn_out == nullptr) return;
+    __syncthreads();
+    seam_gn(f.h0, f.gn_s1, p.C, f.gn_C1, P, f.gamma, f.beta, f.gn_film, f.gn_film_div, f.gn_film_ld, f.eps, f.gn_coefA, f.gn_coefB,
+            f.gn_stats, f.gn_out, f.gn_act, f.gn_ldo, n, wave, lane);
+}
+
+template <int RULE, int MEAN>
+int launch_seam(const HeadUpdate& p, const SeamFront& f, int Cx, void* stream) {
+    const int P = p.H * p.W;
+    hipStream_t s = (hipStream_t)stream;
+#define LFVDM_SEAM(CO)                                                                                              \
+    do {                                                                                                            \
+        static DynLdsLimit limit;                                                                                   \
+        const size_t lds = SeamLds<CO>::bytes(P);                                                                   \
+        if (int rc = limit.ensure(reinterpret_cast<const void*>(&step_seam_kernel<CO, RULE, MEAN>), lds)) return rc; \
+        hipLaunchKernelGGL((step_seam_kernel<CO, RULE, MEAN>), dim3(p.N), dim3(256), lds, s, p, f);                 \
+    } while (0)
+    if (Cx == 4) LFVDM_SEAM(4); else LFVDM_SEAM(3);
+#undef LFVDM_SEAM
+    LFVDM_CHECK_LAUNCH();
+    return LFVDM_OK;
+}
+}
+
+extern "C" int lfvdm_step_seam_ok(int N, int H, int W, int C, int Cx) {
+    if (int rc = lfvdm_conv_out_psample_ok(N, H, W, C, Cx)) return rc;
+    if (C != 64 || N > 65535 || (long)H * W > 256) return LFVDM_E_UNSUPPORTED;
+    if (!conv_in_takes_mfma(Cx, C)) return LFVDM_E_UNSUPPORTED;
+    const int width = gn_wave_width(C, 0, N, H * W);
+    if (width != (H * W >= 128 && (H * W) % 64 == 0 ? 4 : 1)) return LFVDM_E_UNSUPPORTED;
+    const size_t lds = Cx == 4 ? SeamLds<4>::bytes(H * W) : SeamLds<3>::bytes(H * W);
+    return lds <= 160 * 1024 ? LFVDM_OK : LFVDM_E_UNSUPPORTED;
+}
+
+extern "C" int lfvdm_step_seam_gn_ok(int N, int H, int W, int C, int Cx) {
+    if (int rc = lfvdm_step_seam_ok(N, H, W, C, Cx)) return rc;
+    return gn_wave_width(C, 0, N, H * W) == 1 ? LFVDM_OK : LFVDM_E_UNSUPPORTED;
+}
+
+extern "C" int lfvdm_step_seam(const lfvdm_step_seam_args* a, void* stream) {
+    if (!a) return LFVDM_E_SHAPE;
+    if (a->B <= 0 || a->T <= 0 || !a->x0 || !a->obs || !a->w_in || !a->bias_in || !a->h0 || !a->Wp || !a->bias_out)
+        return LFVDM_E_SHAPE;
+    if (a->gn_out && (!a->gamma || !a->beta)) return LFVDM_E_SHAPE;
+    if (a->gn_out && lfvdm_step_seam_gn_ok(a->B * a->T, a->H, a->W, a->C, a->Cx) != LFVDM_OK) return LFVDM_E_UNSUPPORTED;
+    ConvInTick tk = {nullptr, nullptr, nullptr, nullptr, nullptr, 0, 0, 0};
+    if (a->clock_table) {
+        if (a->B > 64 || !a->model_t || !a->rows_all || !a->rows || !a->ticket) return LFVDM_E_SHAPE;
+        if (a->row_floats <= 0 || (a->row_floats & 3) || (a->rows_ld & 3) || a->rows_ld < a->row_floats) return LFVDM_E_SHAPE;
+        tk = {a->t, a->clock_table, a->model_t, a->rows_all, a->rows, a->B, a->rows_ld, a->row_floats};
+    }
+    const int N = a->B * a->T;
+    const SeamFront f = {a->x0, a->obs, a->w_in, a->bias_in, a->h0, a->gamma, a->beta, a->gn_out, a->eps, tk, a->ticket,
+                         nullptr, nullptr, nullptr, nullptr, nullptr, 0, 1, 0, LFVDM_ACT_SILU, 0};
+    if (a->multistep) {
+        if (!multistep_ok(a->mean_type, a->x, a->act, a->t, a->sqrt_recip_acp, a->sqrt_recipm1_acp, a->c1, a->c2, a->k3, a->sample,
+                          a->B, a->T))
+            return LFVDM_E_SHAPE;
+        if (int rc = lfvdm_step_seam_ok(N, a->H, a->W, a->C, a->Cx)) return rc;
+        const HeadUpdate p = {a->act, a->Wp, a->bias_out, a->x, nullptr, a->out, nullptr, a->sample, a->pred_xstart, nullptr, a->t,
+                              nullptr, a->sqrt_recip_acp, a->sqrt_recipm1_acp, a->c1, a->c2, nullptr, N, a->T, a->H, a->W, a->C,
+                              a->clip, a->hist, a->k3};
+        return on_multistep(a->hist != nullptr, a->mean_type,
+                            [&](auto r, auto m) { return launch_seam<decltype(r)::value, decltype(m)::value>(p, f, a->Cx, stream); });
+    }
+    const int R = update_cell(a->rule, a->mean_type, a->x, a->act, a->t, a->sqrt_recip_acp, a->sqrt_recipm1_acp, a->c1, a->c2, a->sg,
+                              a->sample, a->B, a->T, a->noise_in || a->seed);
+    if (R < 0) return LFVDM_E_SHAPE;
+    if (int rc = lfvdm_step_seam_ok(N, a->H, a->W, a->C, a->Cx)) return rc;
+    const bool det = R == RULE_DDIM_DET;
+    const HeadUpdate p = {a->act, a->Wp, a->bias_out, a->x, det ? nullptr : a->noise_in, a->out, det ? nullptr : a->noise_out,
+                          a->sample, a->pred_xstart, a->mean_out, a->t, det ? nullptr : a->seed, a->sqrt_recip_acp,
+                          a->sqrt_recipm1_acp, a->c1, a->c2, a->sg, N, a->T, a->H, a->W, a->C, a->clip, nullptr, nullptr};
+    return on_grid(R, a->mean_type, [&](auto r, auto m) { return launch_seam<decltype(r)::value, decltype(m)::value>(p, f, a->Cx, stream); });
+}
+
 extern "C" int lfvdm_masked_mse(const float* a, const float* b, const float* mask, float* out, int B, int T,
                                 int frame_inner, void* stream) {
     if (B <= 0 || T <= 0 || frame_inner <= 0) return LFVDM_E_SHAPE;
diff --git a/latent-flexible-video-diffusion-modeling_amd/csrc/head_update_body.h b/latent-flexible-video-diffusion-modeling_amd/csrc/head_update_body.h
--- /dev/null
+++ b/latent-flexible-video-diffusion-modeling_amd/csrc/head_update_body.h
@@ -0,0 +1,145 @@
+#pragma once
+#include "common_hip.h"
+#include "philox_normal.h"
+
+namespace {
+
+enum { RULE_ANCESTRAL = 0, RULE_DDIM = 1, RULE_DDIM_DET = 2, RULE_DPMPP2M = 3 };
+constexpr bool rule_draws(int rule) { return rule == RULE_ANCESTRAL || rule == RULE_DDIM; }
+
+enum { MEAN_EPS = 0, MEAN_X0 = 1 };
+
+template <int MEAN>
+__device__ __forceinline__ float mean_x0hat(float r, float rm1, float xv, float out) {
+    return MEAN == MEAN_X0 ? out : r * xv - rm1 * out;
+}
+
+template <int RULE>
+__device__ __forceinline__ float rule_sigma(const float* __restrict__ t_logvar, int64_t tb) {
+    if (RULE == RULE_ANCESTRAL) return tb != 0 ? expf(0.5f * t_logvar[tb]) : 0.f;
+    if (RULE == RULE_DDIM) return tb != 0 ? t_logvar[tb] : 0.f;
+    return 0.f;
+}
+
+struct StepCoef { float r, rm1, c1, c2, sigma; };
+
+template <int RULE, int MEAN>
+__device__ __forceinline__ StepCoef step_coef(int64_t tb, const float* t_recip, const float* t_recipm1, const float* t_c1,
+                                              const float* t_c2, const float* t_logvar) {
+    return {MEAN == MEAN_EPS ? t_recip[tb] : 0.f, MEAN == MEAN_EPS ? t_recipm1[tb] : 0.f, t_c1[tb], t_c2[tb],
+            rule_sigma<RULE>(t_logvar, tb)};
+}
+
+template <int MEAN>
+__device__ __forceinline__ float step_mean(const StepCoef& k, float xv, float out, int clip, float& p0) {
+    p0 = mean_x0hat<MEAN>(k.r, k.rm1, xv, out);
+    if (clip) p0 = fminf(fmaxf(p0, -1.f), 1.f);
+    return k.c1 * p0 + k.c2 * xv;
+}
+
+template <int MEAN>
+__device__ __forceinline__ float multistep_mean(const StepCoef& k, float k3, float xv, float out, int clip, const float* hist,
+                                                size_t at, float& p0) {
+    p0 = MEAN == MEAN_X0 ? out : __fmaf_rn(k.r, xv, -__fmul_rn(k.rm1, out));
+    if (clip) p0 = fminf(fmaxf(p0, -1.f), 1.f);
+    float mean = __fmaf_rn(k.c2, xv, __fmul_rn(k.c1, p0));
+    if (k3 != 0.f) mean = __fmaf_rn(k3, __fsub_rn(p0, hist[at]), mean);
+    return mean;
+}
+
+struct HeadUpdate {
+    const float *act, *Wp, *bias, *x, *noise_in;
+    float *eps_out, *noise_out, *sample, *pred, *mean_out;
+    const int64_t *t, *seed;
+    const float *t_recip, *t_recipm1, *t_c1, *t_c2, *t_logvar;
+    int N, T, H, W, C, clip;
+    const float *hist, *t_k3;
+};
+
+template <int CO, int CPL>
+__device__ __forceinline__ void head_stage_filters(const float* Wp, float* wl, int tid) {
+    constexpr int NW4 = CO * 9 * 16 * CPL, NIT = (NW4 + 255) / 256;
+    f32x4 wv[NIT];
+#pragma unroll
+    for (int u = 0; u < NIT; ++u) {
+        const int i = tid + 256 * u;
+        wv[u] = i < NW4 ? ld4(Wp + 4 * (size_t)i) : (f32x4){0.f, 0.f, 0.f, 0.f};
+    }
+#pragma unroll
+    for (int u = 0; u < NIT; ++u) {
+        const int i = tid + 256 * u;
+        if (i < NW4) st4(wl + 4 * i, wv[u]);
+    }
+}
+
+template <int CO, int CPL>
+__device__ __forceinline__ float head_conv_pixel(const float* fr, const float* wl, int H, int W, int C, int y, int x, int cl) {
+    float acc[CO];
+#pragma unroll
+    for (int co = 0; co < CO; ++co) acc[co] = 0.f;
+#pragma unroll
+    for (int tap = 0; tap < 9; ++tap) {
+        const int iy = y + tap / 3 - 1, ix = x + tap % 3 - 1;
+        const bool inb = iy >= 0 && iy < H && ix >= 0 && ix < W;
+        const float* a = fr + ((size_t)(inb ? iy : y) * W + (inb ? ix : x)) * C;
+#pragma unroll
+        for (int u = 0; u < CPL; ++u) {
+            const int c = (cl + 16 * u) * 4;
+            f32x4 a4 = ld4(a + c);
+            if (!inb) a4 = (f32x4){0.f, 0.f, 0.f, 0.f};
+#pragma unroll
+            for (int co = 0; co < CO; ++co) {
+                const f32x4 w4 = ld4(wl + (co * 9 + tap) * C + c);
+                acc[co] += (a4.x * w4.x + a4.y * w4.y) + (a4.z * w4.z + a4.w * w4.w);
+            }
+        }
+    }
+#pragma unroll
+    for (int co = 0; co < CO; ++co)
+#pragma unroll
+        for (int o = 1; o < 16; o <<= 1) acc[co] += __shfl_xor(acc[co], o, 64);
+    float e = acc[0];
+#pragma unroll
+    for (int co = 1; co < CO; ++co) e = cl == co ? acc[co] : e;
+    return e;
+}
+
+template <int MEAN>
+__device__ __forceinline__ float step_mean_unfused(const StepCoef& k, float xv, float out, int clip, float& p0) {
+#pragma clang fp contract(off)
+    p0 = MEAN == MEAN_X0 ? out : k.r * xv - k.rm1 * out;
+    if (clip) p0 = fminf(fmaxf(p0, -1.f), 1.f);
+    return k.c1 * p0 + k.c2 * xv;
+}
+
+template <int CO, int RULE, int MEAN, bool PINNED = false>
+__device__ __forceinline__ float head_update_elem(const HeadUpdate& p, float e, int n, int y, int x, int j, int co, int64_t tb) {
+    e += p.bias[co];
+    const int b = n / p.T, tt = n - b * p.T;
+    const int inner = p.T * CO * p.H * p.W;
+    const int i = ((tt * CO + co) * p.H + y) * p.W + x;
+    const size_t at = (size_t)b * inner + i;
+    const StepCoef k = step_coef<RULE, MEAN>(tb, p.t_recip, p.t_recipm1, p.t_c1, p.t_c2, p.t_logvar);
+    float z = 0.f;
+    if (!rule_draws(RULE)) {
+    } else if (p.noise_in) {
+        z = p.noise_in[at];
+    } else {
+        const unsigned long long key = (unsigned long long)p.seed[0];
+        const f32x4 z4 = normal4((unsigned)(i >> 2), (unsigned)b, (unsigned)tb, (unsigned)key, (unsigned)(key >> 32));
+        z = j == 0 ? z4.x : j == 1 ? z4.y : j == 2 ? z4.z : z4.w;
+    }
+    float p0;
+    const float mean = RULE == RULE_DPMPP2M ? multistep_mean<MEAN>(k, p.t_k3[tb], p.x[at], e, p.clip, p.hist, at, p0)
+                       : PINNED && rule_draws(RULE) ? step_mean_unfused<MEAN>(k, p.x[at], e, p.clip, p0)
+                                                    : step_mean<MEAN>(k, p.x[at], e, p.clip, p0);
+    const float sv = rule_draws(RULE) ? mean + k.sigma * z : mean;
+    p.sample[at] = sv;
+    if (p.eps_out) p.eps_out[at] = e;
+    if (rule_draws(RULE) && p.noise_out) p.noise_out[at] = z;
+    if (p.pred) p.pred[at] = p0;
+    if (p.mean_out) p.mean_out[at] = mean;
+    return sv;
+}
+
+}
diff --git a/latent-flexible-video-diffusion-modeling_amd/csrc/norm_embed.hip b/latent-flexible-video-diffusion-modeling_amd/csrc/norm_embed.hip
--- a/latent-flexible-video-diffusion-modeling_amd/csrc/norm_embed.hip
+++ b/latent-flexible-video-diffusion-modeling_amd/csrc/norm_embed.hip
@@ -1,4 +1,5 @@
 #include "common_hip.h"
+#include "conv_in_body.h"
 #include "gn_wave_body.h"
 
 namespace {
@@ -159,12 +160,11 @@
 inline bool gn_wave_launch(const float* src0, const float* src1, int C0, int C1, int N, int P, const float* gamma,
                            const float* beta, const float* film, int film_div, int film_ld, float eps, float* coefA,
                            float* coefB, float* stats, float* out, int act, hipStream_t s) {
-    static const bool off = getenv("LFVDM_GN_NO_WAVE") != nullptr;
     const int C = C0 + C1, cg = C / 32;
-    if (off || P > 256 || C0 % 16 || (cg != 2 && cg != 4 && cg != 8 && cg != 16) || N > 65535) return false;
+    const int width = gn_wave_width(C0, C1, N, P);
+    if (!width) return false;
     const dim3 grid(N, C / 16);
-    static const int minp4 = getenv("LFVDM_GN_WAVE4_MINP") ? atoi(getenv("LFVDM_GN_WAVE4_MINP")) : 128;
-    if (minp4 > 0 && P >= minp4 && P % 64 == 0) {
+    if (width == 4) {
 #define LFVDM_GNW4(G)                                                                                                   \
     hipLaunchKernelGGL(gn_wave4_kernel<G>, grid, dim3(256), 0, s, src0, src1, C0, C1, P, gamma, beta, film, film_div, film_ld, \
                        eps, coefA, coefB, stats, out, act, 0)
@@ -478,44 +478,6 @@
     }
 }
 
-struct ConvInTick {
-    int64_t* t;
-    const float* table;
-    float* model_t;
-    const float* rows_all;
-    float* rows;
-    int B, rows_ld, row_floats;
-};
-
-__device__ __forceinline__ void conv_in_clock(const ConvInTick& tk, int64_t* tnew) {
-    if ((int)threadIdx.x < tk.B) {
-        int64_t v = tk.t[threadIdx.x] - 1;
-        v = v < 0 ? 0 : v;
-        tk.t[threadIdx.x] = v;
-        tnew[threadIdx.x] = v;
-    }
-    __syncthreads();
-    if ((int)threadIdx.x < tk.B) tk.model_t[threadIdx.x] = tk.table[tnew[threadIdx.x]];
-    const int q4 = tk.row_floats >> 2;
-    for (int b = 0; b < tk.B; ++b) {
-        const float* src = tk.rows_all + ((size_t)tnew[b] * tk.B + b) * tk.rows_ld;
-        float* dst = tk.rows + (size_t)b * tk.rows_ld;
-        for (int i0 = threadIdx.x; i0 < q4; i0 += 256 * 8) {
-            f32x4 v[8];
-#pragma unroll
-            for (int u = 0; u < 8; ++u) {
-                const int i = i0 + 256 * u;
-                v[u] = i < q4 ? ld4(src + 4 * i) : (f32x4){0.f, 0.f, 0.f, 0.f};
-            }
-#pragma unroll
-            for (int u = 0; u < 8; ++u) {
-                const int i = i0 + 256 * u;
-                if (i < q4) st4(dst + 4 * i, v[u]);
-            }
-        }
-    }
-}
-
 template <int QW, int CIT>
 __global__ __launch_bounds__(256) void conv_in_kernel(const float* __restrict__ x, const float* __restrict__ x0,
                                                       const float* __restrict__ obs, const float* __restrict__ w,
@@ -625,19 +587,17 @@
                                                            const float* __restrict__ obs, const float* __restrict__ w,
                                                            const float* __restrict__ bias, float* __restrict__ out, int N,
                                                            int H, int W, ConvInTick tk) {
-    constexpr int Cout = 16 * NCT, C = CI - 1, K = 9 * CI, KP = (K + 3) & ~3, KS = KP + 1;
-    constexpr int NKI = KP / 4;
+    typedef ConvInMfma<NCT, CI> M;
+    constexpr int C = M::C;
     extern __shared__ __attribute__((aligned(16))) float wl[];
     if (tk.t != nullptr && blockIdx.x == gridDim.x - 1) {
         conv_in_clock(tk, reinterpret_cast<int64_t*>(wl));
         return;
     }
     float* As = wl;
-    float* Ws = wl + 64 * KS;
+    float* Ws = wl + M::A_FLOATS;
     const int tid = threadIdx.x, lane = tid & 63, wave = __builtin_amdgcn_readfirstlane(tid >> 6);
-    float wv[Cout / 4];
-#pragma unroll
-    for (int i = 0; i < Cout / 4; ++i) wv[i] = lane < K ? w[(size_t)(wave + 4 * i) * K + lane] : 0.f;
+    const typename M::Filt wv = M::filt_load(w, wave, lane);
     const int HW = H * W;
     const long total = (long)N * HW;
     const long pix = (long)blockIdx.x * 64 + lane;
@@ -647,56 +607,13 @@
     const int pq = (int)(pp - (long)n * HW);
     const int oy = pq / W, ox = pq - oy * W;
     const float ob = obs[n];
-    const float* xn = x + (size_t)n * C * HW;
-    const float* x0n = x0 + (size_t)n * C * HW;
-    float xa[NKI], xb[NKI];
-    bool inb[NKI];
-#pragma unroll
-    for (int i = 0; i < NKI; ++i) {
-        const int k = wave + 4 * i;
-        const int ci = k / 9, tap = k - ci * 9;
-        const int iy = oy + tap / 3 - 1, ix = ox + tap % 3 - 1;
-        inb[i] = live && k < K && iy >= 0 && iy < H && ix >= 0 && ix < W;
-        const int ip = inb[i] ? iy * W + ix : pq;
-        const int cc = ci < C ? ci : 0;
-        xa[i] = xn[cc * HW + ip];
-        xb[i] = x0n[cc * HW + ip];
-    }
-#pragma unroll
-    for (int i = 0; i < Cout / 4; ++i)
-        if (lane < KP) Ws[(wave + 4 * i) * KS + lane] = wv[i];
-#pragma unroll
-    for (int i = 0; i < NKI; ++i) {
-        const int k = wave + 4 * i;
-        const int ci = k / 9;
-        float v = ci < C ? xa[i] * (1.0f - ob) + xb[i] * ob : ob;
-        As[lane * KS + k] = inb[i] ? v : 0.f;
-    }
+    const typename M::Patch pt = M::patch_load(x + (size_t)n * C * HW, x0 + (size_t)n * C * HW, H, W, oy, ox, pq, live, wave);
+    M::filt_store(wv, Ws, wave, lane);
+    M::patch_store(pt, ob, As, wave, lane);
     __syncthreads();
-    const int r16 = lane & 15, kq = lane >> 4;
     f32x4 acc[NCT];
-#pragma unroll
-    for (int c = 0; c < NCT; ++c) {
-        const float b = bias[16 * c + r16];
-        acc[c] = (f32x4){b, b, b, b};
-    }
-    const float* ar = As + (16 * wave + r16) * KS + kq;
-    const float* wr = Ws + r16 * KS + kq;
-#pragma unroll
-    for (int s4 = 0; s4 < KP; s4 += 4) {
-        const float a = ar[s4];
-#pragma unroll
-        for (int c = 0; c < NCT; ++c) acc[c] = __builtin_amdgcn_mfma_f32_16x16x4f32(a, wr[16 * c * KS + s4], acc[c], 0, 0, 0);
-    }
-    const long p0 = (long)blockIdx.x * 64 + 16 * wave + 4 * kq;
-#pragma unroll
-    for (int r = 0; r < 4; ++r) {
-        if (p0 + r < total) {
-            float* o = out + (size_t)(p0 + r) * Cout + r16;
-#pragma unroll
-            for (int c = 0; c < NCT; ++c) o[16 * c] = acc[c][r];
-        }
-    }
+    M::mma(As, Ws, bias, wave, lane, acc);
+    M::out_store(acc, out, (long)blockIdx.x * 64 + 16 * wave + 4 * (lane >> 4), total, lane);
 }
 
 __global__ __launch_bounds__(256) void rowdot_kernel(const lfvdm_rowdot_job* __restrict__ jobs, int njobs, int total_rows) {
@@ -1039,8 +956,7 @@
     const long total = (long)N * H * W;
     const dim3 grid((unsigned)((total + 63) / 64) + (tk.t ? 1u : 0u));
     {
-        static const bool off = getenv("LFVDM_CONV_IN_SCALAR") != nullptr;
-        if (!off && (C == 4 || C == 3) && (Cout == 64 || Cout == 128)) {
+        if (conv_in_takes_mfma(C, Cout)) {
             const int KP = (9 * (C + 1) + 3) & ~3;
             size_t l2 = (size_t)(64 + Cout) * (KP + 1) * sizeof(float);
             if (l2 < 64 * sizeof(int64_t)) l2 = 64 * sizeof(int64_t);
diff --git a/latent-flexible-video-diffusion-modeling_amd/improved_diffusion/_engine.py b/latent-flexible-video-diffusion-modeling_amd/improved_diffusion/_engine.py
--- a/latent-flexible-video-diffusion-modeling_amd/improved_diffusion/_engine.py
+++ b/latent-flexible-video-diffusion-modeling_amd/improved_diffusion/_engine.py
@@ -39,6 +39,10 @@
 
 def chain_local_enabled():
     return os.environ.get("LFVDM_CHAIN_LOCAL", "1") != "0"
+
+
+def step_seam_enabled():
+    return os.environ.get("LFVDM_STEP_SEAM", "0") == "1"
 
 
 CHAIN_MAX_M = int(os.environ.get("LFVDM_CHAIN_MAX_M", "640"))
@@ -686,6 +690,11 @@
         self.keep.append((t_buf, tables, seed, noise, pred, ddim))
         recip, recipm1, c1, c2, sg, rule, mean_type = update_args(tables, ddim, predict_xstart)
         det, x0 = sg is None, recip is None
+        ms = rule == nat.RULE_DPMPP2M
+        h["update"] = dict(t=t_buf, recip=recip, recipm1=recipm1, c1=c1, c2=c2, sg=sg, rule=rule, mean_type=mean_type,
+                           clip=int(bool(clip)), pred=pred, hist=pred if ms else None,
+                           noise_in=noise if inject_noise and not det and not ms else None,
+                           noise_out=None if inject_noise or det or ms else noise, seed=None if det or ms else seed)
         if rule == nat.RULE_DPMPP2M:
             args = (_p(h["act"]), _p(h["Wp"]), _p(h["bias"]), _p(self.out), _p(self.x_in), _p(pred), _p(t_buf),
                     None if x0 else _p(recip), None if x0 else _p(recipm1), _p(c1), _p(c2), _p(sg), mean_type, int(bool(clip)),
@@ -700,6 +709,50 @@
                 None if det else _p(seed))
         self.steps[h["step"]] = (L.lfvdm_conv_out_update_x0, args)
         self.head_fused = True
+        return True
+
+    def seam_steps(self):
+        L = nat.lib()
+        for i, (fn, args) in enumerate(self.steps[:-1]):
+            if fn is L.lfvdm_conv_in:
+                gfn, g = self.steps[i + 1]
+                h0, ch = args[5], args[10]
+                if (gfn is L.lfvdm_gn_apply and g[0] == h0 and g[1] is None and (g[2], g[3]) == (ch, 0) and g[8] is None
+                        and g[12] == nat.ACT_SILU and g[14] is None and g[16] is None):
+                    return self.steps[i], self.steps[i + 1]
+                return None
+        return None
+
+    def fuse_step_seam(self, ts_table):
+        L, h = nat.lib(), self.head
+        if not step_seam_enabled() or not self.head_fused or not self.time_steps or h["step"] != len(self.steps) - 1:
+            return False
+        pair = self.seam_steps()
+        if pair is None or L.lfvdm_step_seam_ok(self.B * self.T, self.H, self.W, h["C"], h["Cout"]) != 0:
+            return False
+        seam = self.__dict__.get("seam")
+        if seam is not None and seam["first"] is pair[0] and seam["ts_table"] is ts_table:
+            return True
+        (_, ci), (_, g), u = pair[0], pair[1], h["update"]
+        if (ci[0], ci[7], ci[10]) != (_p(self.x_in), h["Cout"], h["C"]):
+            return False
+        gn_inside = L.lfvdm_step_seam_gn_ok(self.B * self.T, self.H, self.W, h["C"], h["Cout"]) == 0
+        if not gn_inside:
+            pair = pair[:1]
+        ms = u["rule"] == nat.RULE_DPMPP2M
+        op = lambda t: _p(t) if t is not None else None
+        if "seam_ticket" not in self.__dict__:
+            self.seam_ticket = self.buf(1, dtype=th.int32).zero_()
+        a = nat.StepSeamArgs(
+            act=_p(h["act"]), Wp=_p(h["Wp"]), bias_out=_p(h["bias"]), out=_p(self.out), x=_p(self.x_in), noise_in=op(u["noise_in"]),
+            noise_out=op(u["noise_out"]), t=_p(u["t"]), sqrt_recip_acp=op(u["recip"]), sqrt_recipm1_acp=op(u["recipm1"]),
+            c1=_p(u["c1"]), c2=_p(u["c2"]), sg=None if ms else op(u["sg"]), hist=op(u["hist"]), k3=_p(u["sg"]) if ms else None,
+            sample=_p(self.x_in), pred_xstart=_p(u["pred"]), mean_out=None, seed=op(u["seed"]), rule=0 if ms else int(u["rule"]),
+            mean_type=int(u["mean_type"]), clip=u["clip"], multistep=int(ms), B=self.B, T=self.T, H=self.H, W=self.W, C=h["C"],
+            Cx=h["Cout"], x0=ci[1], obs=ci[2], w_in=ci[3], bias_in=ci[4], h0=ci[5], gamma=g[6], beta=g[7], gn_out=g[13] if gn_inside else None,
+            eps=float(g[11]), rows_ld=self.rows_ld, row_floats=self.film_floats, clock_table=_p(ts_table), model_t=_p(self.tin),
+            rows_all=_p(self.rows_all), rows=_p(self.rows), ticket=_p(self.seam_ticket))
+        self.seam = dict(args=a, skip=pair, first=pair[0], ts_table=ts_table, gn_inside=gn_inside)
         return True
 
     def tick(self, t_buf, ts_table):
@@ -1064,11 +1117,19 @@
             nat.check(L.lfvdm_pack_conv_weight(_p(w), _p(out), w.shape[0], w.shape[1], w.shape[2], s), "pack")
         self._sig = self.weight_signature()
 
-    def launch(self, tick=None):
+    def launch(self, tick=None, seam_in=False, seam_out=False):
         L = nat.lib()
         s = nat.stream()
-        for fn, args in self.steps:
-            if tick is not None and fn is L.lfvdm_conv_in:
+        skip = self.seam["skip"] if seam_in else ()
+        last = self.steps[-1] if seam_out else None
+        assert not (seam_in and tick is not None), "the seam that did this forward's conv_in moved the clock as well"
+        for step in self.steps:
+            fn, args = step
+            if step is last:
+                rc = L.lfvdm_step_seam(C.byref(self.seam["args"]), s)
+            elif any(step is sk for sk in skip):
+                continue
+            elif tick is not None and fn is L.lfvdm_conv_in:
                 rc = L.lfvdm_conv_in_tick(*args, _p(tick[0]), _p(tick[1]), _p(self.tin), self.B, _p(self.rows_all),
                                           self.rows_ld, _p(self.rows), self.film_floats, s)
                 tick = None
diff --git a/latent-flexible-video-diffusion-modeling_amd/improved_diffusion/_native.py b/latent-flexible-video-diffusion-modeling_amd/improved_diffusion/_native.py
--- a/latent-flexible-video-diffusion-modeling_amd/improved_diffusion/_native.py
+++ b/latent-flexible-video-diffusion-modeling_amd/improved_diffusion/_native.py
@@ -91,6 +91,17 @@
     _fields_ = [("tproj", c_fp), ("Wd", c_fp), ("bd", c_fp), ("Wout_t", c_fp), ("dR", c_fp), ("dtproj", c_fp),
                 ("dWd", c_fp), ("dbd", c_fp), ("C", C.c_int32), ("tile0", C.c_int32), ("tproj_ld", C.c_int32),
                 ("dtproj_ld", C.c_int32)]
+
+
+class StepSeamArgs(C.Structure):
+    _fields_ = [("act", c_fp), ("Wp", c_fp), ("bias_out", c_fp), ("out", c_fp), ("x", c_fp), ("noise_in", c_fp),
+                ("noise_out", c_fp), ("t", c_fp), ("sqrt_recip_acp", c_fp), ("sqrt_recipm1_acp", c_fp), ("c1", c_fp), ("c2", c_fp),
+                ("sg", c_fp), ("hist", c_fp), ("k3", c_fp), ("sample", c_fp), ("pred_xstart", c_fp), ("mean_out", c_fp),
+                ("seed", c_fp), ("rule", C.c_int32), ("mean_type", C.c_int32), ("clip", C.c_int32), ("multistep", C.c_int32),
+                ("B", C.c_int32), ("T", C.c_int32), ("H", C.c_int32), ("W", C.c_int32), ("C", C.c_int32), ("Cx", C.c_int32),
+                ("x0", c_fp), ("obs", c_fp), ("w_in", c_fp), ("bias_in", c_fp), ("h0", c_fp), ("gamma", c_fp), ("beta", c_fp),
+                ("gn_out", c_fp), ("eps", C.c_float), ("rows_ld", C.c_int32), ("row_floats", C.c_int32), ("pad_", C.c_int32),
+                ("clock_table", c_fp), ("model_t", c_fp), ("rows_all", c_fp), ("rows", c_fp), ("ticket", c_fp)]
 
 
 class WgradJob(C.Structure):
@@ -126,6 +137,9 @@
     "lfvdm_conv_out_update_x0": ([c_fp] * 13 + [c_i, c_i, c_i] + [c_fp] * 3 + [c_i] * 6 + [c_fp, c_fp], c_i),
     "lfvdm_update_ms_x0": ([c_fp] * 9 + [c_i, c_i] + [c_fp] * 2 + [c_i, c_i, c_fp], c_i),
     "lfvdm_conv_out_update_ms_x0": ([c_fp] * 12 + [c_i, c_i] + [c_fp] * 2 + [c_i] * 6 + [c_fp], c_i),
+    "lfvdm_step_seam_ok": ([c_i] * 5, c_i),
+    "lfvdm_step_seam_gn_ok": ([c_i] * 5, c_i),
+    "lfvdm_step_seam": ([C.POINTER(StepSeamArgs), c_fp], c_i),
     "lfvdm_known_blend": ([c_fp] * 9 + [c_i] * 4 + [c_fp], c_i),
     "lfvdm_renoise": ([c_fp] * 6 + [c_i, c_i, c_fp], c_i),
     "lfvdm_masked_mse_bwd": ([c_fp, c_fp, c_fp, c_fp, c_fp, c_i, c_i, c_i, c_fp], c_i),
@@ -650,6 +664,28 @@
           "lfvdm_conv_out_update_ms_x0")
 
 
+def step_seam_args(act, wp, bias_out, out, x, noise_in, noise_out, t, recip, recipm1, c1, c2, sg, rule, mean_type, clip, sample, seed,
+                   pred, x0, obs, w_in, bias_in, h0, gamma, beta, eps, gn_out, mean=None, hist=None, clock=None):
+    B, T, Cx, H, W = x.shape
+    ms = rule == RULE_DPMPP2M
+    i64 = lambda v: ptr(v, torch.int64) if v is not None else None
+    a = StepSeamArgs(act=ptr(act), Wp=ptr(wp), bias_out=ptr(bias_out), out=ptr(out), x=ptr(x), noise_in=ptr(noise_in),
+                     noise_out=ptr(noise_out), t=i64(t), sqrt_recip_acp=ptr(recip), sqrt_recipm1_acp=ptr(recipm1), c1=ptr(c1),
+                     c2=ptr(c2), sg=None if ms else ptr(sg), hist=ptr(hist) if ms else None, k3=ptr(sg) if ms else None,
+                     sample=ptr(sample), pred_xstart=ptr(pred), mean_out=ptr(mean), seed=i64(seed), rule=0 if ms else int(rule),
+                     mean_type=int(mean_type), clip=int(bool(clip)), multistep=int(ms), B=B, T=T, H=H, W=W, C=act.shape[-1], Cx=Cx,
+                     x0=ptr(x0), obs=ptr(obs), w_in=ptr(w_in), bias_in=ptr(bias_in), h0=ptr(h0), gamma=ptr(gamma), beta=ptr(beta),
+                     gn_out=ptr(gn_out), eps=float(eps))
+    if clock is not None:
+        a.clock_table, a.model_t, a.rows_all, a.rows = (ptr(clock[k]) for k in ("table", "model_t", "rows_all", "rows"))
+        a.rows_ld, a.row_floats, a.ticket = int(clock["rows_ld"]), int(clock["row_floats"]), ptr(clock["ticket"], torch.int32)
+    return a
+
+
+def step_seam(args):
+    check(lib().lfvdm_step_seam(C.byref(args), stream()), "lfvdm_step_seam")
+
+
 def known_blend(x, known, mask, t, a, s, eps=None, seed=None, noise_out=None):
     B, T, Cx, H, W = x.shape
     if known.shape != x.shape or tuple(mask.shape) != (B, T, H, W) or (eps is not None and eps.shape != x.shape):
diff --git a/latent-flexible-video-diffusion-modeling_amd/improved_diffusion/_replay.py b/latent-flexible-video-diffusion-modeling_amd/improved_diffusion/_replay.py
--- a/latent-flexible-video-diffusion-modeling_amd/improved_diffusion/_replay.py
+++ b/latent-flexible-video-diffusion-modeling_amd/improved_diffusion/_replay.py
@@ -108,6 +108,10 @@
         self.expected_t = max(i - 1, 0)
 
 
+def seam_plan(n, seam):
+    return [(bool(seam) and k > 0, bool(seam) and k + 1 < n) for k in range(n)]
+
+
 class GraphSampler(ReplayedStep):
 
     def __init__(self, diffusion, unet, shape, clip_denoised, inject_noise=False, rule=("ancestral",)):
@@ -143,8 +147,8 @@
         self.known_eps = th.zeros(self.shape, device=dev) if fixed_noise else None
         self.known_noise = th.zeros(self.shape, device=dev) if record_noise and not fixed_noise else None
 
-    def _step_body(self):
-        self._denoise_body()
+    def _step_body(self, seam_in=False, seam_out=False):
+        self._denoise_body(seam_in, seam_out)
         if self.known is not None:
             nat.known_blend(self.plan.x_in, self.known, self.known_mask, self.t_buf, self.known_tb["a"], self.known_tb["s"],
                             eps=self.known_eps, seed=self.seed, noise_out=self.known_noise)
@@ -154,7 +158,7 @@
         tb = self.known_tb
         nat.renoise(self.plan.x_in, self.t_buf, tb["sqrt_1mbeta"], tb["sqrt_beta"], self.seed)
 
-    def _denoise_body(self):
+    def _head_mode(self):
         import os
         pl = self.plan
         recip, recipm1, c1, c2, sg, rule, mean_type = self.update
@@ -164,6 +168,33 @@
                  and pl.fuse_head_update(self.t_buf, self.tb, self.clip, self.seed, self.noise, self.pred, self.inject_noise,
                                          ddim=self.ddim, predict_xstart=self.x0_mode))
         tick_in_conv = bool(pl.time_steps) and os.environ.get("LFVDM_TICK_IN_CONV", "1") != "0"
+        return det, in_kernel, fused, tick_in_conv
+
+    def seam_ok(self):
+        if self.known is not None:
+            return False
+        _, _, fused, tick_in_conv = self._head_mode()
+        return bool(fused and tick_in_conv and self.plan.fuse_step_seam(self.ts_table))
+
+    def _warm_seam(self):
+        pl = self.plan
+        keep = [t for t in (pl.x_in, self.pred, self.t_buf, pl.tin, pl.rows)]
+        saved = [t.clone() for t in keep]
+        self.t_buf.clamp_(max=self.diffusion.num_timesteps - 1)
+        nat.step_seam(pl.seam["args"])
+        for t, s in zip(keep, saved):
+            t.copy_(s)
+        th.cuda.synchronize()
+
+    def _denoise_body(self, seam_in=False, seam_out=False):
+        pl = self.plan
+        recip, recipm1, c1, c2, sg, rule, mean_type = self.update
+        det, in_kernel, fused, tick_in_conv = self._head_mode()
+        if seam_in or seam_out:
+            assert fused and tick_in_conv
+            pl.launch(tick=None if seam_in else (self.t_buf, self.ts_table), seam_in=seam_in, seam_out=seam_out)
+            self.extra_launches = 0
+            return
         if tick_in_conv:
             pl.launch(tick=(self.t_buf, self.ts_table))
         else:
@@ -244,9 +275,13 @@
             if self.graph_k is None:
                 g = th.cuda.CUDAGraph()
                 th.cuda.synchronize()
+                seam = self.seam_ok()
+                if seam:
+                    self._warm_seam()
                 with th.no_grad(), th.cuda.graph(g, capture_error_mode="thread_local"):
-                    for _ in range(self.K):
-                        self._step_body()
+                    for seam_in, seam_out in seam_plan(self.K, seam):
+                        self._step_body(seam_in=seam_in, seam_out=seam_out)
+                self.seams_per_graph = (self.K - 1) if seam else 0
                 self.graph_k = g
             while left >= self.K:
                 self.plan.ensure_R(t, t - self.K + 1)
```

After: 1264. No clear change (-0.0%).
